# HJakeCunningham/ASVGP

Measured on AMD Instinct MI355X. Metric: Mpoints/s per ELBO+grad step, N=10M 1D Matern-3/2 M=2048, higher is better.
Workload: dtype f64

## Files before the change

### asvgp_amd/_lib.py

```python
import ctypes
import os

import torch

HERE = os.path.dirname(os.path.abspath(__file__))
LIB_PATH = os.path.join(HERE, "libasvgp_hip.so")

_c = ctypes
_P, _I, _L, _D, _Z = _c.c_void_p, _c.c_int, _c.c_int64, _c.c_double, _c.c_size_t

SIGNATURES = {
    "asvgp_version": (_I, []),
    "asvgp_last_error_string": (_c.c_char_p, []),
    "asvgp_status_name": (_c.c_char_p, [_I]),
    "asvgp_phi_workspace_bytes": (_Z, [_L, _I, _L]),
    "asvgp_create": (_I, [_c.POINTER(_P)]),
    "asvgp_destroy": (_I, [_P]),
    "asvgp_phi_accumulate_1d": (_I, [_P, _P, _P, _L, _L, _P, _L, _D, _I, _L, _P, _P, _Z, _P]),
    "asvgp_phi_weighted_workspace_bytes": (_Z, [_L, _I, _L]),
    "asvgp_phi_accumulate_1d_weighted": (_I, [_P, _P, _P, _P, _L, _L, _P, _L, _D, _I, _L, _P, _P, _P, _Z, _P]),
    "asvgp_set_weight_sums": (_I, [_P, _D, _D, _D]),
    "asvgp_phi_accumulate_kron2d_weighted": (_I, [_P, _P, _P, _L, _P, _L, _D, _L, _P, _L, _D, _L, _I, _P, _P, _P]),
    "asvgp_phi_accumulate_kron2d_sorted_weighted": (_I, [_P, _P, _P, _L, _P, _P, _L, _D, _L, _P, _L, _D, _L, _I, _P, _P, _P]),
    "asvgp_set_phi_algorithm": (_I, [_P, _I]),
    "asvgp_phi_last_algorithm": (_I, [_P]),
    "asvgp_set_phi_input_order": (_I, [_P, _I]),
    "asvgp_phi_last_input_order": (_I, [_P]),
    "asvgp_stream_probe": (_I, [_P, _P, _L, _P, _P]),
    "asvgp_debug_reload_env": (_I, []),
    "asvgp_set_deferred_forward_pass": (_I, [_P, _I]),
    "asvgp_prior_publish": (_I, [_P]),
    "asvgp_host_mantissa_bits": (_I, []),
    "asvgp_prior_interior_kuu_host": (_I, [_P, _I, _L, _I, _P, _P, _c.POINTER(_L), _c.POINTER(_L), _P]),
    "asvgp_result_mirror": (_I, [_P, _I, _c.POINTER(_P)]),
    "asvgp_result_mirror_read": (_I, [_P, _c.c_uint64, _P, _D]),
    "asvgp_elbo_grad_ahead_1d": (_I, [_P, _P, _P, _I, _L, _L, _I, _L, _P, _P, _P, _Z, _P]),
    "asvgp_elbo_publish_theta": (_I, [_P, _D, _D, _D]),
    "asvgp_elbo_grad_host_1d": (_I, [_P, _P, _P, _I, _D, _D, _D, _L, _L, _I, _L, _P, _P, _P, _Z, _P, _P, _D]),
    "asvgp_result_mirror_pending": (_c.c_uint64, [_P]),
    "asvgp_set_phi_workgroups": (_I, [_P, _I]),
    "asvgp_set_phi_deferred_reduce": (_I, [_P, _I]),
    "asvgp_phi_reduce_1d": (_I, [_P, _P]),
    "asvgp_phi_index_1d": (_I, [_P, _L, _P, _L, _D, _P, _P]),
    "asvgp_phi_evaluate_1d": (_I, [_P, _L, _P, _L, _D, _I, _I, _P, _P, _P]),
    "asvgp_matern_coeffs": (_I, [_I, _D, _D, _c.POINTER(_D), _c.POINTER(_D), _c.POINTER(_I)]),
    "asvgp_kuu_assemble": (_I, [_P, _I, _c.POINTER(_D), _c.POINTER(_D), _L, _I, _P, _P, _P]),
    "asvgp_cholesky_band": (_I, [_P, _P, _L, _I, _P, _P]),
    "asvgp_inverse_from_cholesky_band": (_I, [_P, _P, _L, _I, _P]),
    "asvgp_solve_triang_mat": (_I, [_P, _P, _P, _L, _I, _L, _I, _P]),
    "asvgp_product_band_band": (_I, [_P, _P, _P, _L, _I, _I, _I, _I, _I, _I, _P]),
    "asvgp_transpose_band": (_I, [_P, _P, _L, _I, _I, _P]),
    "asvgp_symmetrise_band": (_I, [_P, _P, _L, _I, _P]),
    "asvgp_unpack_banded_matrix_to_dense": (_I, [_P, _P, _L, _I, _I, _P]),
    "asvgp_pack_dense_matrix_to_banded": (_I, [_P, _P, _L, _I, _I, _P]),
    "asvgp_band_trace_sym": (_I, [_P, _P, _L, _I, _P, _P]),
    "asvgp_cholesky_band_vjp": (_I, [_P, _P, _P, _P, _L, _I, _P]),
    "asvgp_inverse_from_cholesky_band_vjp": (_I, [_P, _P, _P, _P, _P, _L, _I, _P]),
    "asvgp_band_outer_product": (_I, [_P, _P, _L, _L, _I, _D, _P, _P]),
    "asvgp_elbo_workspace_bytes": (_Z, [_L, _I, _L]),
    "asvgp_set_band_algorithm": (_I, [_P, _I]),
    "asvgp_prior_plan_1d": (_I, [_P, _P, _I, _L, _I, _c.POINTER(_I)]),
    "asvgp_prior_table_doubles": (_Z, [_P, _I, _L, _I]),
    "asvgp_prior_forward_host": (_I, [_P, _I, _L, _I, _P, _P, _P, _Z, _P]),
    "asvgp_set_prior_forward": (_I, [_P, _I]),
    "asvgp_prior_forward_device": (_I, [_P, _P, _P, _P, _Z, _P]),
    "asvgp_prior_forward_stamps": (_I, [_P, _P, _P, _P, _P]),
    "asvgp_prior_plan_image_host": (_I, [_P, _I, _L, _I, _P, _P, _P, _P]),
    "asvgp_elbo_grad_1d": (_I, [_P, _P, _P, _I, _D, _D, _D, _L, _L, _I, _L, _P, _P, _P, _Z, _P]),
    "asvgp_kuu_inverse_band_1d": (_I, [_P, _P, _I, _D, _D, _L, _I, _P, _P, _P, _P, _P, _P, _P, _Z, _P]),
    "asvgp_elbo_chain_sync": (_I, [_P, _I]),
    "asvgp_elbo_prior_chain_1d": (_I, [_P, _P, _I, _D, _D, _D, _L, _I, _L, _P, _P, _Z, _P]),
    "asvgp_elbo_data_chain_1d": (_I, [_P, _P, _P, _I, _D, _D, _D, _L, _L, _I, _L, _P, _P, _P, _Z, _P]),
    "asvgp_posterior_prepare_1d": (_I, [_P, _P, _P, _I, _D, _D, _D, _L, _I, _L, _P, _P, _P, _P, _Z, _P]),
    "asvgp_posterior_prepare_loo_1d": (_I, [_P, _P, _P, _I, _D, _D, _D, _L, _I, _L, _P, _P, _P, _P, _P, _Z, _P]),
    "asvgp_loo_workspace_bytes": (_Z, [_L, _I, _L]),
    "asvgp_loo_1d": (_I, [_P, _P, _P, _P, _L, _L, _P, _L, _D, _I, _L, _P, _P, _P, _D, _D, _P, _P, _P, _P, _P, _Z, _P]),
    "asvgp_predict_1d": (_I, [_P, _L, _P, _L, _D, _I, _L, _P, _P, _D, _L, _P, _P, _P]),
    "asvgp_predict_1d_h": (_I, [_P, _P, _L, _P, _L, _D, _I, _L, _P, _P, _D, _L, _P, _P, _P]),
    "asvgp_posterior_cov_workspace_bytes": (_Z, [_L, _I, _L]),
    "asvgp_posterior_cov_prepare_1d": (_I, [_P, _P, _P, _I, _D, _D, _D, _L, _I, _L, _P, _P, _P, _P, _P, _Z, _P]),
    "asvgp_predict_cov_1d": (_I, [_P, _P, _L, _P, _L, _P, _L, _D, _I, _L, _P, _I, _D, _D, _P, _L, _P]),
    "asvgp_predict_deriv_1d": (_I, [_P, _P, _L, _P, _L, _D, _I, _L, _P, _P, _I, _D, _D, _L, _P, _P, _P]),
    "asvgp_predict_cov_deriv_1d": (_I, [_P, _P, _L, _P, _L, _P, _L, _D, _I, _L, _P, _I, _D, _D, _I, _I, _P, _L, _P]),
    "asvgp_predict_grad_kron2d": (_I, [_P, _L, _P, _L, _D, _L, _P, _L, _D, _L, _I, _P, _P, _P, _P, _P, _L, _I, _L, _L, _L, _L,
                                       _I, _D, _D, _I, _D, _D, _P, _P, _P]),
    "asvgp_kron_dense_inverse": (_I, [_P, _P, _P, _L, _L, _I, _L, _L, _L, _L, _P, _P]),
    "asvgp_predict_cov_kron2d": (_I, [_P, _P, _L, _P, _L, _P, _L, _D, _L, _P, _L, _D, _L, _I, _P, _P, _P, _I, _D, _D, _I, _D, _D, _P, _L, _P]),
    "asvgp_predict_cov_additive": (_I, [_P, _P, _L, _P, _L, _I, _P, _c.POINTER(_L), _c.POINTER(_D), _c.POINTER(_L), _I,
                                         _c.POINTER(_I), _c.POINTER(_D), _c.POINTER(_D), _P, _P, _L, _P]),
    "asvgp_predict_components_additive": (_I, [_P, _P, _L, _I, _P, _c.POINTER(_L), _c.POINTER(_D), _c.POINTER(_L), _I, _c.POINTER(_I),
                                                _c.POINTER(_D), _c.POINTER(_D), _I, _P, _P, _P, _P, _P]),
    "asvgp_profile_enable": (_I, [_P, _I]),
    "asvgp_profile_read": (_I, [_P, _c.POINTER(_D), _c.POINTER(_L)]),
    "asvgp_kron_stats_doubles": (_Z, [_L, _L, _I]),
    "asvgp_phi_accumulate_kron2d": (_I, [_P, _P, _L, _P, _L, _D, _L, _P, _L, _D, _L, _I, _P, _P]),
    "asvgp_kron_evaluate_2d": (_I, [_P, _L, _P, _L, _D, _P, _L, _D, _L, _I, _P, _P, _P]),
    "asvgp_kron_assemble": (_I, [_P, _P, _P, _P, _P, _I, _L, _L, _D, _P, _P, _P]),
    "asvgp_blockband_cholesky": (_I, [_P, _L, _L, _P, _P, _P, _P]),
    "asvgp_blockband_backsolve": (_I, [_P, _L, _L, _P, _P]),
    "asvgp_predict_kron2d": (_I, [_P, _L, _P, _L, _D, _L, _P, _L, _D, _L, _I, _P, _P, _P, _P, _P, _P]),
    "asvgp_kron_cell_index": (_I, [_P, _L, _P, _L, _D, _P, _L, _D, _P, _P]),
    "asvgp_phi_accumulate_kron2d_sorted": (_I, [_P, _P, _L, _P, _P, _L, _D, _L, _P, _L, _D, _L, _I, _P, _P]),
    "asvgp_phi_accumulate_kron2d_sorted_f32": (_I, [_P, _P, _L, _P, _P, _L, _D, _L, _P, _L, _D, _L, _I, _P, _P]),
    "asvgp_blockband_to_blocks": (_I, [_P, _L, _L, _L, _P, _P, _P]),
    "asvgp_kron_grad_terms": (_I, [_P, _P, _L, _P, _P, _P, _P, _P, _P, _P, _P, _P, _P, _I, _L, _L, _P, _P]),
    "asvgp_predict_kron2d_var": (_I, [_P, _L, _P, _L, _D, _P, _L, _D, _L, _I, _P, _P, _L, _P, _P]),
    "asvgp_kron_assemble_twisted": (_I, [_P, _P, _P, _P, _P, _I, _L, _L, _D, _L, _L, _L, _L, _L, _P, _P, _P, _P]),
    "asvgp_kron_grad_terms_twisted": (_I, [_P, _P, _L, _L, _L, _L, _L, _P, _P, _P, _P, _P, _P, _P, _P, _P, _P, _I, _L, _L, _P, _P]),
    "asvgp_predict_kron2d_var_twisted": (_I, [_P, _L, _P, _L, _D, _P, _L, _D, _L, _L, _I, _P, _P, _L, _L, _L, _L, _L, _P, _P]),
    "asvgp_phi_cross_workspace_bytes": (_Z, [_L, _L]),
    "asvgp_phi_cross_2d": (_I, [_P, _P, _L, _P, _L, _D, _L, _P, _L, _D, _L, _I, _P, _P, _Z, _P]),
}


class AsvgpError(RuntimeError):
    pass


_lib = None


def get_lib():
    global _lib
    if _lib is not None:
        return _lib
    if not os.path.exists(LIB_PATH):
        raise AsvgpError("HIP extension %s is missing: run `python -m asvgp_amd.build` (hipcc, gfx950). "
                         "asvgp_amd has no CPU fallback." % LIB_PATH)
    lib = ctypes.CDLL(LIB_PATH)
    for name, (res, args) in SIGNATURES.items():
        fn = getattr(lib, name, None)
        if fn is None:
            raise AsvgpError("libasvgp_hip.so does not export %s" % name)
        fn.restype = res
        fn.argtypes = args
    _lib = lib
    return lib


def check(status, what=""):
    if status != 0:
        lib = get_lib()
        raise AsvgpError("%s failed: %s (%s)" % (what or "asvgp call", lib.asvgp_status_name(status).decode(),
                                                  lib.asvgp_last_error_string().decode()))


class Handle:
    _defaults = {"band": 0, "phi": 0, "prior_forward": 0, "phi_order": 0}
    _live = None

    def __init__(self):
        import weakref
        lib = get_lib()
        h = _P()
        check(lib.asvgp_create(ctypes.byref(h)), "asvgp_create")
        self.ptr = h
        self._lib = lib
        self.band_algorithm = 0
        if Handle._live is None:
            Handle._live = weakref.WeakSet()
        Handle._live.add(self)
        if Handle._defaults["band"]:
            self.set_band_algorithm(Handle._defaults["band"])
        if Handle._defaults["phi"]:
            self.set_phi_algorithm(Handle._defaults["phi"])
        if Handle._defaults["prior_forward"]:
            self.set_prior_forward(Handle._defaults["prior_forward"])
        if Handle._defaults["phi_order"]:
            self.set_phi_input_order(Handle._defaults["phi_order"])

    def set_prior_forward(self, mode):
        check(self._lib.asvgp_set_prior_forward(self.ptr, int(mode)), "set_prior_forward")

    def prior_forward_device(self, coef, dcoef, n_doubles):
        import numpy as np
        coef = np.ascontiguousarray(coef, dtype=np.float64)
        dcoef = np.ascontiguousarray(dcoef, dtype=np.float64)
        tab = np.zeros(int(n_doubles), dtype=np.float64)
        check(self._lib.asvgp_prior_forward_device(self.ptr, coef.ctypes.data, dcoef.ctypes.data, tab.ctypes.data, tab.size, stream_ptr()),
              "prior_forward_device")
        return tab

    def set_band_algorithm(self, algo):
        check(self._lib.asvgp_set_band_algorithm(self.ptr, int(algo)), "set_band_algorithm")
        self.band_algorithm = int(algo)

    def set_phi_algorithm(self, algo):
        check(self._lib.asvgp_set_phi_algorithm(self.ptr, int(algo)), "set_phi_algorithm")

    def set_weight_sums(self, n_pos, sum_w, sum_log_w):
        if n_pos is None:
            n_pos, sum_w, sum_log_w = -1.0, 0.0, 0.0
        check(self._lib.asvgp_set_weight_sums(self.ptr, float(n_pos), float(sum_w), float(sum_log_w)), "set_weight_sums")

    def phi_last_algorithm(self):
        return int(self._lib.asvgp_phi_last_algorithm(self.ptr))

    def set_phi_input_order(self, order):
        check(self._lib.asvgp_set_phi_input_order(self.ptr, int(order)), "set_phi_input_order")

    def phi_last_input_order(self):
        return int(self._lib.asvgp_phi_last_input_order(self.ptr))

    def result_mirror(self, enable=True):
        import numpy as np
        ptr = _P()
        check(self._lib.asvgp_result_mirror(self.ptr, int(bool(enable)), ctypes.byref(ptr)), "result_mirror")
        if not enable or not ptr.value:
            self._mirror = None
            return None
        self._mirror = np.ctypeslib.as_array(ctypes.cast(ptr, ctypes.POINTER(_D)), shape=(16,))
        return self._mirror

    def set_deferred_forward_pass(self, on):
        check(self._lib.asvgp_set_deferred_forward_pass(self.ptr, int(on)), "set_deferred_forward_pass")

    def publish_forward(self):
        self._lib.asvgp_prior_publish(self.ptr)

    def result_mirror_pending(self):
        return int(self._lib.asvgp_result_mirror_pending(self.ptr))

    def set_phi_workgroups(self, n):
        check(self._lib.asvgp_set_phi_workgroups(self.ptr, int(n)), "set_phi_workgroups")

    deferred = False

    def set_phi_deferred_reduce(self, on):
        check(self._lib.asvgp_set_phi_deferred_reduce(self.ptr, int(on)), "set_phi_deferred_reduce")
        self.deferred = bool(on)

    def chain_sync(self, on):
        check(self._lib.asvgp_elbo_chain_sync(self.ptr, int(on)), "elbo_chain_sync")

    def prior_plan(self, static_stack_host, n_terms, M, k):
        ok = _I(0)
        ptr = None if static_stack_host is None else static_stack_host.ctypes.data
        check(self._lib.asvgp_prior_plan_1d(self.ptr, ptr, int(n_terms), int(M), int(k), ctypes.byref(ok)), "prior_plan_1d")
        return bool(ok.value)

    def close(self):
        if getattr(self, "ptr", None) is not None and self.ptr:
            try:
                self._lib.asvgp_destroy(self.ptr)
            except Exception:
                pass
            self.ptr = None
            self._mirror = None

    def __del__(self):
        self.close()


def set_default_algorithms(band=None, phi=None, prior_forward=None, phi_order=None):
    if prior_forward is not None:
        Handle._defaults["prior_forward"] = int(prior_forward)
        for h in list(Handle._live or ()):
            h.set_prior_forward(prior_forward)
    if phi_order is not None:
        Handle._defaults["phi_order"] = int(phi_order)
        for h in list(Handle._live or ()):
            h.set_phi_input_order(phi_order)
    if band is not None:
        Handle._defaults["band"] = int(band)
    if phi is not None:
        Handle._defaults["phi"] = int(phi)
    for h in list(Handle._live or ()):
        if band is not None:
            h.set_band_algorithm(band)
        if phi is not None:
            h.set_phi_algorithm(phi)


_stream_override = None


def set_stream(stream=None):
    global _stream_override
    _stream_override = None if stream is None else ctypes.c_void_p(stream.cuda_stream)


def stream_ptr():
    if _stream_override is not None:
        return _stream_override
    return ctypes.c_void_p(torch.cuda.current_stream().cuda_stream)


def require_cuda(*tensors):
    for t in tensors:
        if not t.is_cuda:
            raise AsvgpError("asvgp_amd operates on ROCm device tensors only (got a %s tensor); there is no CPU path"
                             % t.device)


def f64c(t):
    if t.dtype != torch.float64:
        t = t.to(torch.float64)
    return t.contiguous()
```

### asvgp_amd/csrc/bcr_mfma.hpp

```cpp
#pragma once
#include "bcr.hpp"
#include "prior_plan.hpp"

namespace asvgp {

constexpr int BM_THREADS = 1024;
constexpr int BM_B = 4;
constexpr int BM_GAT = 0, BM_GBT = 16, BM_DINV = 32, BM_SD = 48, BM_CAT = 64, BM_CBT = 80, BM_W = 96, BM_DG = 100, BM_REC = 104;

__host__ __device__ inline size_t bcr_mfma_ws_doubles(long nb) { return (size_t)nb * BM_REC + 64; }
__host__ __device__ inline size_t bcr_mfma_lds_doubles(long nb) {
  return (size_t)((nb + 1) / 2 + 1) * 32 + (size_t)nb * 4 + 96 + (size_t)(BM_THREADS / 64) * 4 * 40 + (size_t)(nb / 8 + 2) * 52;
}

__device__ __forceinline__ double bm_mfma(double a, double b, double c) { return __builtin_amdgcn_mfma_f64_4x4x4f64(a, b, c, 0, 0, 0); }

__device__ __forceinline__ double bm_chol_linv(const double (&d)[10], int hi, int lo, double& dprod, int& badj) {
  double l00, i0, l10, l20, l30, l11, i1, l21, l31, l22, i2, l32, l33, i3;
  Num<double>::sqrt_inv(d[0], l00, i0);
  badj = !(d[0] > 0.0) ? 1 : 0;
  l10 = d[1] * i0; l20 = d[3] * i0; l30 = d[6] * i0;
  double s = fma(-l10, l10, d[2]);
  badj = (!(s > 0.0) && !badj) ? 2 : badj;
  Num<double>::sqrt_inv(s, l11, i1);
  l21 = fma(-l20, l10, d[4]) * i1;
  l31 = fma(-l30, l10, d[7]) * i1;
  s = fma(-l21, l21, fma(-l20, l20, d[5]));
  badj = (!(s > 0.0) && !badj) ? 3 : badj;
  Num<double>::sqrt_inv(s, l22, i2);
  l32 = fma(-l31, l21, fma(-l30, l20, d[8])) * i2;
  s = fma(-l32, l32, fma(-l31, l31, fma(-l30, l30, d[9])));
  badj = (!(s > 0.0) && !badj) ? 4 : badj;
  Num<double>::sqrt_inv(s, l33, i3);
  dprod = (l00 * l11) * (l22 * l33);
  const double z0 = (lo == 0) ? i0 : 0.0;
  const double z1 = fma(-l10, z0, (lo == 1) ? 1.0 : 0.0) * i1;
  const double z2 = fma(-l21, z1, fma(-l20, z0, (lo == 2) ? 1.0 : 0.0)) * i2;
  const double z3 = fma(-l32, z2, fma(-l31, z1, fma(-l30, z0, (lo == 3) ? 1.0 : 0.0))) * i3;
  return hi == 0 ? z0 : (hi == 1 ? z1 : (hi == 2 ? z2 : z3));
}

template <typename Src> __device__ __forceinline__ auto bm_src_load(const Src& A, int dd, long col, long M, int) -> decltype(A.load_dc(dd, col, M)) {
  return A.load_dc(dd, col, M);
}
template <typename Src> __device__ __forceinline__ double bm_src_load(const Src& A, int dd, long col, long M, long) {
  return A.load((long)dd * M + col, true);
}
struct BmLog {
  double m; int e;
  __device__ __forceinline__ void mul(double p) {
    m *= p;
    const int hi = __double2hiint(m);
    e += ((hi >> 20) & 0x7ff) - 1023;
    m = __hiloint2double((hi & 0x800fffff) | 0x3ff00000, __double2loint(m));
  }
};

__device__ __forceinline__ unsigned long long bm_wave_xor(unsigned long long x) {
#pragma unroll
  for (int off = 32; off > 0; off >>= 1) x ^= (unsigned long long)__shfl_xor((long long)x, off, 64);
  return x;
}
__device__ __forceinline__ void bm_msg_send(double* box, int n, double v, unsigned long long tag, int lane) {
  unsigned long long* b = reinterpret_cast<unsigned long long*>(box);
  const unsigned long long w = lane < n ? (unsigned long long)__double_as_longlong(v) : 0ull;
  const unsigned long long x = bm_wave_xor(w) ^ tag;
  if (lane < n) __hip_atomic_store(b + lane, w, __ATOMIC_RELAXED, __HIP_MEMORY_SCOPE_AGENT);
  if (lane == n) __hip_atomic_store(b + n, x, __ATOMIC_RELAXED, __HIP_MEMORY_SCOPE_AGENT);
}
__device__ __forceinline__ bool bm_msg_recv(const double* box, int n, double& v, unsigned long long tag, int lane, long spin_limit) {
  const unsigned long long* b = reinterpret_cast<const unsigned long long*>(box);
  for (long spins = 0; spins <= spin_limit; ++spins) {
    const unsigned long long w = lane <= n ? __hip_atomic_load(b + lane, __ATOMIC_RELAXED, __HIP_MEMORY_SCOPE_AGENT) : 0ull;
    const unsigned long long x = bm_wave_xor(lane < n ? w : 0ull) ^ tag;
    const unsigned long long chk = (unsigned long long)__shfl((long long)w, n, 64);
    if (x == chk) { v = __longlong_as_double((long long)w); return true; }
    __builtin_amdgcn_s_sleep(1);
  }
  return false;
}

struct BmSplit {
  int half = -1;
  double* xchg = nullptr;
  long spin_limit = 0;
  int* gave_up = nullptr;
  unsigned long long tag = 0;
};
constexpr int BM_XCHG = 96;

template <typename Src>
__device__ __attribute__((always_inline)) void bcr_mfma_solve(Src A, const double* rhs, int M, double* ws, double* lds, double* Sband, double* x,
                                                              double* logdet, int* info, int rhs_stride = 1, double* stamps = nullptr,
                                                              BmSplit sp = BmSplit{}) {
  constexpr int B = BM_B;
  const int tid = threadIdx.x;
  const int lane = tid & 63, wv = __builtin_amdgcn_readfirstlane(tid >> 6);
  const int r = lane >> 4, q = (lane >> 2) & 3, c = lane & 3;
  const int e = r * 4 + c, et = c * 4 + r;
  const int hi = r > c ? r : c, lo = r > c ? c : r;
  const int nb = (M + B - 1) / B;
  const int nslot = (nb + 1) / 2;
  double* Dl = lds;
  double* El = lds + (size_t)(nslot + 1) * 16;
  double* xs = El + (size_t)(nslot + 1) * 16;
  double* red = xs + (size_t)nb * B;
  double* slab = red + 96 + (size_t)(wv * 4 + q) * 40;
  double* Fl = red + 96 + (size_t)(BM_THREADS / 64) * 4 * 40;
  double* Sl = lds;
  int levels = 0;
  while ((1 << levels) < nb) ++levels;
  const bool split = sp.half >= 0;
  const int top = levels - 1, ht = 1 << (top > 0 ? top : 0);
  double s_other = 0.0;
  int bad_other = 0x7fffffff;
  auto level_share = [&](int l, int ne, int& m0, int& ne_h) {
    m0 = 0; ne_h = ne;
    if (!split) return;
    if (l < top) {
      const int mL = ht >> (l + 1);
      if (sp.half == 0) ne_h = ne < mL ? ne : mL;
      else { m0 = mL; ne_h = ne > mL ? ne - mL : 0; }
    } else {
      ne_h = sp.half == 0 ? ne : 0;
    }
  };
  int bad = 0;
  BmLog ld{1.0, 0};
  unsigned long long t_prev = stamps ? __builtin_amdgcn_s_memtime() : 0ull;
  int nst = 0;
  auto stamp = [&]() {
    if (stamps && tid == 0) { const unsigned long long t = __builtin_amdgcn_s_memtime(); stamps[nst++] = (double)(t - t_prev); t_prev = t; }
  };
  auto rec = [&](int node) -> double* { return ws + (size_t)node * BM_REC; };
  auto bandD = [&](int n, int rr, int cc) -> double {
    const int col = n * B + cc, row = n * B + rr;
    const bool pad = row >= M;
    const double v = bm_src_load(A, rr - cc, pad ? 0 : col, (long)M, 0);
    return pad ? ((rr == cc) ? 1.0 : 0.0) : v;
  };
  auto bandE = [&](int n, int rr, int cc) -> double {
    if (rr > cc) return 0.0;
    const int col = n * B + cc, row = (n + 1) * B + rr;
    const bool pad = row >= M;
    const double v = bm_src_load(A, B + rr - cc, pad ? 0 : col, (long)M, 0);
    return pad ? 0.0 : v;
  };
  if ((nb & 1) && tid < 16 && !(split && sp.half == 0)) {
    const int rr = tid >> 2, cc = tid & 3;
    Dl[(size_t)((nb - 1) >> 1) * 16 + tid] = bandD(nb - 1, rr > cc ? rr : cc, rr > cc ? cc : rr);
  }
  if (split && sp.half == 0 && tid < 16) Dl[(size_t)(ht >> 1) * 16 + tid] = 0.0;
  for (int row = tid; row < nb * B; row += BM_THREADS) {
    const bool sep_left = split && sp.half == 0 && row >= ht * B && row < (ht + 1) * B;
    xs[row] = (row < M && !sep_left) ? rhs[(long)row * rhs_stride] : 0.0;
  }
  __syncthreads();
  stamp();

  constexpr int RMAXR = 4;
  for (int l = 0; l < levels; ++l) {
    const int h = 1 << l;
    const int ne = (nb > h) ? (nb - h + 2 * h - 1) / (2 * h) : 0;
    int m0, ne_h;
    level_share(l, ne, m0, ne_h);
    if (split && l == top) {
      if (sp.half == 1) {
        if (wv == 0) {
          const double v = lane < 16 ? Dl[(size_t)(ht >> 1) * 16 + lane] : (lane < 20 ? xs[ht * B + lane - 16] : 0.0);
          bm_msg_send(sp.xchg, 20, v, sp.tag | 1ull, lane);
        }
        const double mine = (r == 0 && c == 0) ? (log(ld.m) + (double)ld.e * 0.6931471805599453094) : 0.0;
        const double tot = wave_sum_dpp(mine);
        int bm = bad ? bad : 0x7fffffff;
#pragma unroll
        for (int off = 32; off > 0; off >>= 1) { const int o = __shfl_xor(bm, off, 64); bm = o < bm ? o : bm; }
        int* sbad = reinterpret_cast<int*>(red + 32);
        if (lane == 0) { red[wv] = tot; sbad[wv] = bm; }
        __syncthreads();
        if (wv == 0) {
          double sv = 0.0;
          int bmin = 0x7fffffff;
          for (int w2 = 0; w2 < BM_THREADS / 64; ++w2) { sv += red[w2]; bmin = sbad[w2] < bmin ? sbad[w2] : bmin; }
          bm_msg_send(sp.xchg + 24, 2, lane == 0 ? sv : (double)bmin, sp.tag | 2ull, lane);
        }
      } else {
        if (wv == 0) {
          double v = 0.0;
          if (!bm_msg_recv(sp.xchg, 20, v, sp.tag | 1ull, lane, sp.spin_limit)) { if (lane == 0) *sp.gave_up = 1; }
          else {
            if (lane < 16) Dl[(size_t)(ht >> 1) * 16 + lane] += v;
            else if (lane < 20) xs[ht * B + lane - 16] += v;
          }
        }
        __syncthreads();
        if (*sp.gave_up) return;
      }
      stamp();
    }
    double updb[RMAXR], ybu[RMAXR];
    int qv = q, ev = e;
    asm volatile("" : "+v"(qv), "+v"(ev));
    double sl[2][3];
    auto slab_loads = [&](int rd0) __attribute__((always_inline)) {
#pragma unroll
      for (int u = 0; u < 2; ++u) {
#pragma unroll
        for (int t3 = 0; t3 < 3; ++t3) {
          sl[u][t3] = 0.0;
          int m = (rd0 + u) * 64 + wv * 4 + qv;
          m = m0 + (m < ne_h ? m : ne_h - 1);
          const int kk = ev + 16 * t3, dd = kk >> 3, col = m * 2 * B + (kk & 7);
          const bool in = kk < 40 && col + dd < M;
          const double v = bm_src_load(A, in ? dd : 0, in ? col : 0, (long)M, 0);
          sl[u][t3] = in ? v : ((dd == 0) ? 1.0 : 0.0);
        }
      }
    };
#pragma unroll
    for (int rd = 0; rd < RMAXR; ++rd) {
      __builtin_amdgcn_sched_barrier(0);
      if (l == 0 && (rd & 1) == 0) slab_loads(rd);
      updb[rd] = 0.0; ybu[rd] = 0.0;
      if (rd * 64 + wv * 4 >= ne_h) continue;
      const int ml = rd * 64 + wv * 4 + q;
      const bool act = ml < ne_h;
      const int i = h + (m0 + (act ? ml : ne_h - 1)) * 2 * h, a = i - h, b = i + h;
      const bool hasb = b < nb;
      const int bsafe = hasb ? b : a;
      double d[10];
      double ea, eb, da;
      if (l == 0) {
#pragma unroll
        for (int t3 = 0; t3 < 3; ++t3) if (e + 16 * t3 < 40) slab[e + 16 * t3] = sl[rd & 1][t3];
        int kk = 0;
#pragma unroll
        for (int rr = 0; rr < 4; ++rr)
#pragma unroll
          for (int cc = 0; cc <= rr; ++cc) d[kk++] = slab[(rr - cc) * 8 + 4 + cc];
        ea = slab[(4 + lo - hi) * 8 + hi];
        ea = (r <= c) ? ea : 0.0;
        eb = slab[(4 + lo - hi) * 8 + 4 + hi];
        eb = (hasb && c <= r) ? eb : 0.0;
        da = slab[(hi - lo) * 8 + lo];
      } else {
        const double* Di = Dl + (size_t)(i >> 1) * 16;
        int kk = 0;
#pragma unroll
        for (int rr = 0; rr < 4; ++rr)
#pragma unroll
          for (int cc = 0; cc <= rr; ++cc) d[kk++] = Di[rr * 4 + cc];
        ea = El[(size_t)(a >> 1) * 16 + e];
        eb = El[(size_t)(i >> 1) * 16 + et];
        eb = hasb ? eb : 0.0;
        da = Dl[(size_t)(a >> 1) * 16 + e];
      }
      double yv = xs[i * B + r], ya = xs[a * B + r];
      yv = (c == 0) ? yv : 0.0;
      ya = (c == 0) ? ya : 0.0;
      (void)bsafe;
      double dprod;
      int badj;
      const double t = bm_chol_linv(d, hi, lo, dprod, badj);
      if (act && badj && !bad) bad = i * B + badj;
      const double linv = (r >= c) ? t : 0.0;
      const double linvT = (c >= r) ? t : 0.0;
      if (act) ld.mul(dprod);
      const double ua = bm_mfma(linvT, ea, 0.0);
      const double ub = bm_mfma(linvT, eb, 0.0);
      const double zz = bm_mfma(linvT, yv, 0.0);
      const double nua = -ua, nub = -ub;
      const double da_new = bm_mfma(nua, ua, da);
      const double e_new = bm_mfma(nub, ua, 0.0);
      const double ya_new = bm_mfma(nua, zz, ya);
      updb[rd] = bm_mfma(ub, ub, 0.0);
      ybu[rd] = bm_mfma(ub, zz, 0.0);
      updb[rd] = act ? updb[rd] : 0.0;
      ybu[rd] = act ? ybu[rd] : 0.0;
      const double gat = bm_mfma(ua, linv, 0.0);
      const double gbt = bm_mfma(ub, linv, 0.0);
      const double dinv = bm_mfma(linv, linv, 0.0);
      const double w = bm_mfma(linv, zz, 0.0);
      if (act) {
        if (l >= 3) {
          double* R = Fl + (size_t)(i >> 3) * 52;
          R[e] = gat; R[16 + e] = gbt; R[32 + e] = dinv;
          if (c == 0) R[48 + r] = w;
        } else {
          double* R = rec(i);
          R[BM_GAT + e] = gat; R[BM_GBT + e] = gbt; R[BM_DINV + e] = dinv;
          if (c == 0) R[BM_W + r] = w;
        }
        Dl[(size_t)(a >> 1) * 16 + e] = da_new;
        El[(size_t)(a >> 1) * 16 + e] = e_new;
        if (c == 0) xs[a * B + r] = ya_new;
      }
    }
    bcr_lds_barrier();
#pragma unroll
    for (int rd = 0; rd < RMAXR; ++rd) {
      if (rd * 64 + wv * 4 >= ne_h) continue;
      const int ml = rd * 64 + wv * 4 + q;
      const int i = h + (m0 + ml) * 2 * h, b = i + h;
      if (ml < ne_h && b < nb) {
        Dl[(size_t)(b >> 1) * 16 + e] -= updb[rd];
        if (c == 0) xs[b * B + r] -= ybu[rd];
      }
    }
    bcr_lds_barrier();
    stamp();
  }
  if (wv == 0 && !(split && sp.half == 1)) {
    const bool act = q == 0;
    double d[10];
    int kk = 0;
#pragma unroll
    for (int rr = 0; rr < 4; ++rr)
#pragma unroll
      for (int cc = 0; cc <= rr; ++cc) { const double v = Dl[rr * 4 + cc]; d[kk++] = act ? v : ((rr == cc) ? 1.0 : 0.0); }
    const double yv = (act && c == 0) ? xs[r] : 0.0;
    double dprod;
    int badj;
    const double t = bm_chol_linv(d, hi, lo, dprod, badj);
    if (act && badj && !bad) bad = badj;
    const double linv = (r >= c) ? t : 0.0, linvT = (c >= r) ? t : 0.0;
    if (act) ld.mul(dprod);
    const double s00 = bm_mfma(linv, linv, 0.0);
    const double zz = bm_mfma(linvT, yv, 0.0);
    const double x0 = bm_mfma(linv, zz, 0.0);
    if (act) {
      rec(0)[BM_SD + e] = s00;
      Sl[e] = s00;
      if (r >= c && r < M) Sband[(long)(r - c) * M + c] = s00;
      if (c == 0) xs[r] = x0;
    }
  }
  __syncthreads();
  stamp();
  unsigned long long lw = 0ull;
  for (int l = levels - 1; l >= 0; --l) {
    const int h = 1 << l;
    const int ne = (nb > h) ? (nb - h + 2 * h - 1) / (2 * h) : 0;
    int m0, ne_h;
    level_share(l, ne, m0, ne_h);
    if (split && sp.half == 0 && wv == BM_THREADS / 64 - 1) {
      if (l == top - 1 && lane <= 2)
        lw = __hip_atomic_load(reinterpret_cast<const unsigned long long*>(sp.xchg + 24) + lane, __ATOMIC_RELAXED, __HIP_MEMORY_SCOPE_AGENT);
      if (l == 2) {
        const unsigned long long x = bm_wave_xor(lane < 2 ? lw : 0ull) ^ (sp.tag | 2ull);
        const unsigned long long chk = (unsigned long long)__shfl((long long)lw, 2, 64);
        double v = __longlong_as_double((long long)lw);
        bool ok = x == chk;
        if (!ok) ok = bm_msg_recv(sp.xchg + 24, 2, v, sp.tag | 2ull, lane, sp.spin_limit);
        if (!ok) { if (lane == 0) *sp.gave_up = 1; }
        else if (lane < 2) red[48 + lane] = v;
      }
    }
#pragma unroll
    for (int rd = 0; rd < RMAXR; ++rd) {
      __builtin_amdgcn_sched_barrier(0);
      if (rd * 64 + wv * 4 >= ne_h) continue;
      const int ml = rd * 64 + wv * 4 + q;
      const bool act = ml < ne_h;
      const int i = h + (m0 + (act ? ml : ne_h - 1)) * 2 * h, a = i - h, b = i + h;
      const bool hasb = b < nb;
      const int bs = hasb ? b : a;
      const bool e_is_a = ((a / (2 * h)) & 1) != 0;
      double gat, gbt, dinv, w, saa, sbb, sba, sab;
      if (l >= 3) {
        const double* R = Fl + (size_t)(i >> 3) * 52;
        gat = R[e]; gbt = R[16 + e]; dinv = R[32 + e]; w = R[48 + r];
      } else {
        const double* R = rec(i);
        gat = R[BM_GAT + e]; gbt = R[BM_GBT + e]; dinv = R[BM_DINV + e]; w = R[BM_W + r];
      }
      if (l >= 1) {
        const double* Ra = Sl + (size_t)(a >> 2) * 48;
        const double* Rb = Sl + (size_t)(bs >> 2) * 48;
        saa = Ra[e];
        sbb = Rb[e];
        sba = e_is_a ? Ra[32 + e] : Rb[16 + et];
        sab = e_is_a ? Ra[32 + et] : Rb[16 + e];
      } else {
        const double* Ra = rec(a);
        const double* Rb = rec(bs);
        saa = Ra[BM_SD + e];
        sbb = Rb[BM_SD + e];
        sba = e_is_a ? Ra[BM_CBT + e] : Rb[BM_CAT + et];
        sab = e_is_a ? Ra[BM_CBT + et] : Rb[BM_CAT + e];
      }
      sbb = hasb ? sbb : 0.0; sba = hasb ? sba : 0.0; sab = hasb ? sab : 0.0;
      double xa = xs[a * B + r], xb = xs[bs * B + r];
      xa = (c == 0) ? xa : 0.0;
      xb = (hasb && c == 0) ? xb : 0.0;
      w = (c == 0) ? w : 0.0;
      double ncat = bm_mfma(saa, gat, 0.0);
      ncat = bm_mfma(sba, gbt, ncat);
      double ncbt = bm_mfma(sab, gat, 0.0);
      ncbt = bm_mfma(sbb, gbt, ncbt);
      double sii = bm_mfma(ncat, gat, dinv);
      sii = bm_mfma(ncbt, gbt, sii);
      double gx = bm_mfma(gat, xa, 0.0);
      gx = bm_mfma(gbt, xb, gx);
      if (act) {
        if (c == 0) xs[i * B + r] = w - gx;
        if (l >= 2) {
          double* Rw = Sl + (size_t)(i >> 2) * 48;
          Rw[e] = sii; Rw[16 + e] = -ncat; Rw[32 + e] = -ncbt;
        }
        if (l > 0) {
          double* Rw = rec(i);
          Rw[BM_SD + e] = sii; Rw[BM_CAT + e] = -ncat; Rw[BM_CBT + e] = -ncbt;
        }
        if (r >= c && i * B + r < M) Sband[(long)(r - c) * M + i * B + c] = sii;
        if (l == 0) {
          if (c <= r && i * B + c < M) Sband[(long)(B + c - r) * M + a * B + r] = -ncat;
          if (hasb && r <= c && b * B + r < M) Sband[(long)(B + r - c) * M + i * B + c] = -ncbt;
        }
      }
    }
    if (l == 1) __syncthreads(); else bcr_lds_barrier();
    if (split && l == top) {
      double* Rs = Sl + (size_t)(ht >> 2) * 48;
      if (sp.half == 0) {
        if (wv == 0) bm_msg_send(sp.xchg + 32, 52, lane < 48 ? Rs[lane < 48 ? lane : 0] : (lane < 52 ? xs[ht * B + lane - 48] : 0.0), sp.tag | 3ull, lane);
      } else {
        if (wv == 0) {
          double v = 0.0;
          if (!bm_msg_recv(sp.xchg + 32, 52, v, sp.tag | 3ull, lane, sp.spin_limit)) { if (lane == 0) *sp.gave_up = 1; }
          else if (lane < 48) {
            Rs[lane] = v;
            rec(ht)[BM_SD + lane] = v;
            if (lane < 16) {
              const int rr = lane >> 2, cc = lane & 3;
              if (rr >= cc && ht * B + rr < M) Sband[(long)(rr - cc) * M + ht * B + cc] = v;
            }
          } else if (lane < 52) {
            xs[ht * B + lane - 48] = v;
          }
        }
        __syncthreads();
        if (*sp.gave_up) return;
      }
    }
    stamp();
  }
  if (!(split && sp.half == 0))
    for (int col = M - B + tid; col < M; col += BM_THREADS)
      if (col >= 0)
#pragma unroll
        for (int dd = 1; dd <= B; ++dd)
          if (col + dd >= M) Sband[(long)dd * M + col] = 0.0;
  {
    const int row0 = (split && sp.half == 1) ? (ht + 1) * B : 0, row1 = (split && sp.half == 0) ? (ht + 1) * B : M;
    for (int row = row0 + tid; row < row1 && row < M; row += BM_THREADS) x[(long)row * rhs_stride] = xs[row];
  }
  if (!(split && sp.half == 1)) {
    const double mine = (r == 0 && c == 0) ? (log(ld.m) + (double)ld.e * 0.6931471805599453094) : 0.0;
    const double tot = wave_sum_dpp(mine);
    int bm = bad ? bad : 0x7fffffff;
#pragma unroll
    for (int off = 32; off > 0; off >>= 1) { const int o = __shfl_xor(bm, off, 64); bm = o < bm ? o : bm; }
    int* sbad = reinterpret_cast<int*>(red + 32);
    if (lane == 0) { red[wv] = tot; sbad[wv] = bm; }
    __syncthreads();
    if (split && tid == 0) { s_other = red[48]; bad_other = (int)red[49]; }
    if (tid == 0) {
      double s = 0.0;
      int bmin = 0x7fffffff;
      for (int w2 = 0; w2 < BM_THREADS / 64; ++w2) { s += red[w2]; bmin = sbad[w2] < bmin ? sbad[w2] : bmin; }
      s += s_other;
      bmin = bad_other < bmin ? bad_other : bmin;
      __hip_atomic_store(logdet + 0, 2.0 * s, __ATOMIC_RELAXED, __HIP_MEMORY_SCOPE_AGENT);
      __hip_atomic_store(logdet + 1, 0.0, __ATOMIC_RELAXED, __HIP_MEMORY_SCOPE_AGENT);
      __hip_atomic_store(info, (bmin == 0x7fffffff) ? 0 : bmin, __ATOMIC_RELAXED, __HIP_MEMORY_SCOPE_AGENT);
    }
  }
  stamp();
}


__host__ __device__ inline size_t bcr_mfma_pre_ws_doubles(long nb) { return (size_t)nb * 96 + 64; }
__host__ __device__ inline size_t bcr_mfma_pre_lds_doubles(long nb, int n_rec) {
  return PRIOR_TAB_HEADER + (size_t)2 * n_rec * prior_rec_fields(BM_B) + (size_t)(nb / 4 + 2) * 96 + (size_t)(nb + 1) / 2 + 64;
}

struct BmDual { double v, d; };
__device__ __forceinline__ BmDual bm_dmfma(BmDual x, BmDual y, BmDual c) {
  BmDual r;
  r.v = bm_mfma(x.v, y.v, c.v);
  r.d = bm_mfma(x.d, y.v, c.d);
  r.d = bm_mfma(x.v, y.d, r.d);
  return r;
}

__device__ __attribute__((always_inline)) void bcr_mfma_backward_pre(const double* __restrict__ tab, int n_rec, const int* __restrict__ node_rec, int M,
                                                                      double* ws, double* lds, double* Sv, double* Sd, double* logdet, int* info,
                                                                      unsigned long long* done_flag, unsigned long long seq,
                                                                      const unsigned long long* ready_flag = nullptr, long spin_limit = 0, int* gave_up = nullptr) {
  constexpr int B = BM_B, W = prior_rec_fields(B);
  const int tid = threadIdx.x;
  if (ready_flag) {
    if (tid == 0) {
      long spins = 0;
      while (__hip_atomic_load(ready_flag, __ATOMIC_RELAXED, __HIP_MEMORY_SCOPE_SYSTEM) < seq) {
        __builtin_amdgcn_s_sleep(8);
        if (++spins > spin_limit) { *gave_up = 1; break; }
      }
    }
    __syncthreads();
    if (*gave_up) return;
    __builtin_amdgcn_fence(__ATOMIC_ACQUIRE, "");
  }
  const int lane = tid & 63, wv = __builtin_amdgcn_readfirstlane(tid >> 6);
  const int r = lane >> 4, q = (lane >> 2) & 3, c = lane & 3;
  const int e = r * 4 + c, et = c * 4 + r;
  const int nb = (M + B - 1) / B;
  const int n_tab = PRIOR_TAB_HEADER + 2 * n_rec * W;
  double* tl = lds;
  double* Sl = lds + n_tab;
  int* nrl = reinterpret_cast<int*>(Sl + (size_t)(nb / 4 + 2) * 96);
  {
    const double2* src = reinterpret_cast<const double2*>(tab);
    double2* dst = reinterpret_cast<double2*>(tl);
// ... 96 lines not shown
```

### asvgp_amd/csrc/elbo.hip

```cpp
#include <stdlib.h>
#include <time.h>
#include <string.h>

#include "bcr_pre.hpp"
#include "bcr_mfma.hpp"
#include "handle.hpp"

namespace asvgp {


struct Ws {
  double *Kuu, *dK, *P, *LK, *dLK, *LP, *SK, *dSK, *SP, *c, *alpha, *logdets, *fin, *bcrK, *bcrP;
};
static size_t bcr_ws_chain(int planes, int k, bool big) {
  long ns = 1024;
  while ((long)planes * 2 * k * k * ns * 8 + 2 * ns * k * 8 + 1024 > 150 * 1024) ns >>= 1;
  if (big) ns *= 2;
  return (size_t)planes * (7 * k * k + k) * 2 * ns + (big ? (size_t)planes * k * k * ns : 0);
}
static size_t bcr_ws_K(int k, long M) {
  size_t a = bcr_ws_chain(2, k, false), b = bcr_ws_chain(2, k, true), c = bcr_pre_ws_doubles(k, (M + k - 1) / k);
  a = a > b ? a : b;
  return (a > c ? a : c) + 64;
}
// ... 157 lines not shown
template <int K, bool BIG>
__global__ __launch_bounds__(BCR_THREADS) void elbo_bcr_data_kernel(const double* Kuu, const double* A, const double* b, int M,
                                                                    double* wsP, double* SP, double* x, double* logdets,
                                                                    int* info, int do_stamps, double s, int D, int lds_doubles) {
  extern __shared__ double lds[];
  double* st = do_stamps ? logdets + 8 : nullptr;
  bcr_solve<double, K, 1, BandSumP, BIG>(BandSumP{A, Kuu, 1.0 / s}, b, M, wsP, lds, BandOut<double>{SP, nullptr}, x, logdets + 2, info + 1,
                                         st ? st + 24 : nullptr, D);
  more_columns<K, BIG>(b, x, D, M, wsP, lds, lds_doubles);
}

template <int KT>
__device__ __forceinline__ double quad_col(const double* S, long M, long j, const double* x, long D, long d) {
  double xj = x[j * D + d];
  double a = S[j] * xj * xj;
#pragma unroll
  for (int r = 1; r <= KT; ++r) {
    long jr = (j + r < M) ? j + r : M - 1;
    double sv = (j + r < M) ? S[(long)r * M + j] : 0.0;
    a = fma(2.0 * sv * xj, x[jr * D + d], a);
  }
  return a;
}

struct ElboScalars { double v, l, s, N, Nw, cw; };

template <int KT>
__device__ __forceinline__ void elbo_finalize_body(
    int bid, int nblk, double* part_lds, const double* __restrict__ stats, const double* __restrict__ Kuu, const double* __restrict__ dK,
    const double* __restrict__ LK, const double* __restrict__ LP, const double* __restrict__ SK,
    const double* __restrict__ dSK, const double* __restrict__ SP, const double* __restrict__ c,
    const double* __restrict__ alpha, const double* __restrict__ logdets, long M, long D, ElboScalars th,
    double alpha_scale, double* __restrict__ gacc, unsigned* __restrict__ ticket, unsigned* __restrict__ rearm, double* __restrict__ out) {
  constexpr int k = KT;
  const double* A = stats;
  const double* b = stats + (long)(k + 1) * M;
  const double yy = stats[(long)(k + 1) * M + M * D];
  enum { LOGK, LOGP, TRKA, DTRKA, SKDK, SPDK, SKK, SPK, SPA, CC, AKA, ADKA, AAA, BA, NACC };
  double acc[NACC];
#pragma unroll
  for (int i = 0; i < NACC; ++i) acc[i] = 0.0;
  const long chunk = (M + nblk - 1) / nblk;
  const long j_end = ((long)(bid + 1) * chunk < M) ? (long)(bid + 1) * chunk : M;
  for (long j = (long)bid * chunk + threadIdx.x; j < j_end; j += blockDim.x) {
    if (!logdets) {
      double lk = LK[j], lp = LP[j];
      acc[LOGK] += log(lk * lk);
      acc[LOGP] += log(lp * lp);
    }
#pragma unroll
    for (int r = 0; r <= k; ++r) {
      long o = (long)r * M + j;
      double w = (r == 0) ? 1.0 : 2.0;
      double sk = SK[o], sp = SP[o], a = A[o], kk = Kuu[o], dk = dK[o];
      acc[TRKA] = fma(w * sk, a, acc[TRKA]);
      acc[DTRKA] = fma(w * dSK[o], a, acc[DTRKA]);
      acc[SKDK] = fma(w * sk, dk, acc[SKDK]);
      acc[SPDK] = fma(w * sp, dk, acc[SPDK]);
      acc[SKK] = fma(w * sk, kk, acc[SKK]);
      acc[SPK] = fma(w * sp, kk, acc[SPK]);
      acc[SPA] = fma(w * sp, a, acc[SPA]);
    }
    for (long d = 0; d < D; ++d) {
      if (!logdets) {
        double cv = c[j * D + d];
        acc[CC] = fma(cv, cv, acc[CC]);
      }
      acc[AKA] += quad_col<KT>(Kuu, M, j, alpha, D, d);
      acc[ADKA] += quad_col<KT>(dK, M, j, alpha, D, d);
      acc[AAA] += quad_col<KT>(A, M, j, alpha, D, d);
      acc[BA] = fma(b[j * D + d], alpha[j * D + d], acc[BA]);
    }
  }
  double (*part)[NACC] = reinterpret_cast<double (*)[NACC]>(part_lds);
  const int lane = threadIdx.x & 63, wv = threadIdx.x >> 6, nw = blockDim.x >> 6;
#pragma unroll
  for (int i = 0; i < NACC; ++i) {
    double v = wave_sum_dpp(acc[i]);
    if (lane == 0) part[wv][i] = v;
  }
  __syncthreads();
  double tot[NACC];
  if (threadIdx.x < 64) {
#pragma unroll
    for (int i = 0; i < NACC; ++i) tot[i] = wave_sum_dpp(lane < nw ? part[lane][i] : 0.0);
  }
  int* is_last_p = reinterpret_cast<int*>(part_lds + 16 * NACC);
#define is_last (*is_last_p)
  if (threadIdx.x == 0) {
#pragma unroll
    for (int i = 0; i < NACC; ++i)
      if (tot[i] != 0.0) __hip_atomic_fetch_add(gacc + i, tot[i], __ATOMIC_RELAXED, __HIP_MEMORY_SCOPE_AGENT);
    asm volatile("s_waitcnt vmcnt(0)" ::: "memory");
    unsigned t = __hip_atomic_fetch_add(ticket, 1u, __ATOMIC_RELAXED, __HIP_MEMORY_SCOPE_AGENT);
    is_last = (t == (unsigned)nblk - 1);
  }
  __syncthreads();
  if (!is_last) return;
  if (threadIdx.x == 0) {
#pragma unroll
    for (int i = 0; i < NACC; ++i) tot[i] = __hip_atomic_load(gacc + i, __ATOMIC_RELAXED, __HIP_MEMORY_SCOPE_AGENT);
#pragma unroll
    for (int i = 0; i < NACC; ++i) __hip_atomic_store(gacc + i, 0.0, __ATOMIC_RELAXED, __HIP_MEMORY_SCOPE_AGENT);
    __hip_atomic_store(ticket, 0u, __ATOMIC_RELAXED, __HIP_MEMORY_SCOPE_AGENT);
    if (rearm) __hip_atomic_store(rearm, 0u, __ATOMIC_RELAXED, __HIP_MEMORY_SCOPE_AGENT);
    const double v = th.v, s = th.s, N = th.N, Nw = th.Nw, Dd = (double)D;
    tot[AKA] *= alpha_scale * alpha_scale; tot[ADKA] *= alpha_scale * alpha_scale; tot[AAA] *= alpha_scale * alpha_scale;
    tot[BA] *= alpha_scale;
    if (logdets) {
      tot[LOGK] = logdets[0];
      tot[LOGP] = logdets[2];
      tot[CC] = tot[BA] / s;
    }
    const double two_pi = 6.283185307179586476925286766559;
    double elbo = -0.5 * N * Dd * log(two_pi * s);
    elbo -= 0.5 * Dd * tot[LOGP];
    elbo += 0.5 * Dd * tot[LOGK];
    elbo -= 0.5 * yy / s;
    elbo += 0.5 * tot[CC];
    elbo -= 0.5 * Nw * v / s;
    elbo += 0.5 * tot[TRKA] / s;
    if (th.cw != 0.0) elbo += th.cw;
    double d_l = 0.5 * (Dd * tot[SKDK] - Dd * tot[SPDK] - tot[ADKA] + tot[DTRKA] / s);
    double d_v = 0.5 * (-Dd * tot[SKK] / v + Dd * tot[SPK] / v + tot[AKA] / v + tot[TRKA] / (v * s)) - 0.5 * Nw / s;
    double s2 = s * s;
    double d_s = -0.5 * N * Dd / s + 0.5 * Dd * tot[SPA] / s2 + 0.5 * yy / s2 + 0.5 * tot[AAA] / s2 - tot[BA] / s2 +
                 0.5 * Nw * v / s2 - 0.5 * tot[TRKA] / s2;
    out[0] = elbo; out[1] = d_v; out[2] = d_l; out[3] = d_s;
    out[4] = tot[LOGK]; out[5] = tot[LOGP]; out[6] = tot[TRKA]; out[7] = tot[CC];
  }
#undef is_last
}

constexpr int FIN_LDS_DOUBLES = 16 * 14 + 2;

template <int KT>
__global__ __launch_bounds__(256) void elbo_finalize_kernel(
    const double* __restrict__ stats, const double* __restrict__ Kuu, const double* __restrict__ dK,
    const double* __restrict__ LK, const double* __restrict__ LP, const double* __restrict__ SK,
    const double* __restrict__ dSK, const double* __restrict__ SP, const double* __restrict__ c,
    const double* __restrict__ alpha, const double* __restrict__ logdets, long M, int k_rt, long D, ElboScalars th,
    double alpha_scale, double* __restrict__ gacc, unsigned* __restrict__ ticket, double* __restrict__ out) {
  __shared__ double part[FIN_LDS_DOUBLES];
  (void)k_rt;
  elbo_finalize_body<KT>((int)blockIdx.x, (int)gridDim.x, part, stats, Kuu, dK, LK, LP, SK, dSK, SP, c, alpha, logdets, M, D, th, alpha_scale,
                         gacc, ticket, nullptr, out);
}

struct FusedFin {
  const double* stats; ElboScalars th; double alpha_scale; double* gacc; unsigned* ticket; unsigned* arrived; unsigned* assembled; double* out;
  long D; int n_helpers; int finalize; int debug_no_assembly; int debug_stamps;
  double* mirror; unsigned long long mirror_seq;
  int split; double* xchg;
};
constexpr int FIN_GACC_PR = 21;
__device__ __forceinline__ void assemble_band_slice(const double* __restrict__ S, const double* __restrict__ coef, const double* __restrict__ dcoef, int n_terms,
                                                    long E, long e, double* __restrict__ Kuu, double* __restrict__ dK) {
#pragma clang fp contract(off)
  double sv[ASVGP_MAX_KUU_TERMS];
#pragma unroll
  for (int t = 0; t < ASVGP_MAX_KUU_TERMS; ++t) sv[t] = (t < n_terms) ? S[(long)t * E + e] : 0.0;
  double acc = coef[0] * sv[0], dacc = dcoef[0] * sv[0];
#pragma unroll
  for (int t = 1; t < ASVGP_MAX_KUU_TERMS; ++t)
    if (t < n_terms) { acc = acc + coef[t] * sv[t]; dacc = dacc + dcoef[t] * sv[t]; }
  Kuu[e] = acc;
  if (dK) dK[e] = dacc;
}
template <int K, bool BIG>
__global__ __launch_bounds__(BCR_THREADS) void elbo_chains_kernel(const double* S_static, KuuCoefs2 cf, double* Kuu, double* dK, const double* A, const double* b, int M,
                                                                  double* wsP, double* SP, double* x, double* logdets, int* info,
                                                                  double s, const double* tab, int n_rec, const int* node_rec,
                                                                  double* wsK, double* SK, double* dSK,
                                                                  unsigned long long* done_flag, unsigned long long seq, int D, int lds_doubles, FusedFin fin) {
  extern __shared__ double lds[];
  const long E = (long)(K + 1) * M;
  __shared__ int gave_up;
  if (threadIdx.x == 0) gave_up = 0;
  __syncthreads();
  if (blockIdx.x == 0) {
    if (threadIdx.x == 0) {
      long spins = 0;
      while (__hip_atomic_load(fin.assembled, __ATOMIC_RELAXED, __HIP_MEMORY_SCOPE_AGENT) < (unsigned)fin.n_helpers) {
        __builtin_amdgcn_s_sleep(2);
        if (++spins > (1L << 25)) { gave_up = 1; break; }
      }
      if (!gave_up) __hip_atomic_store(fin.assembled, 0u, __ATOMIC_RELAXED, __HIP_MEMORY_SCOPE_AGENT);
    }
    __syncthreads();
    if (gave_up) { if (threadIdx.x == 0) atomicExch(info + 1, -1); return; }
    __builtin_amdgcn_fence(__ATOMIC_ACQUIRE, "agent");
    bcr_solve<double, K, 1, BandSumP, BIG>(BandSumP{A, Kuu, 1.0 / s}, b, M, wsP, lds, BandOut<double>{SP, nullptr}, x, logdets + 2, info + 1, nullptr, D);
    more_columns<K, BIG>(b, x, D, M, wsP, lds, lds_doubles);
  } else if (blockIdx.x == 1) {
    bcr_backward_pre<K>(tab, n_rec, node_rec, M, wsK, lds, BandOut<Dual>{SK, dSK}, logdets, info, done_flag, seq);
  } else {
    for (long e = (long)(blockIdx.x - 2) * blockDim.x + threadIdx.x; e < E; e += (long)fin.n_helpers * blockDim.x)
      assemble_band_slice(S_static, cf.c, cf.dc, cf.n, E, e, Kuu, dK);
    __syncthreads();
    if (threadIdx.x == 0) {
      __threadfence();
      __hip_atomic_fetch_add(fin.assembled, 1u, __ATOMIC_RELEASE, __HIP_MEMORY_SCOPE_AGENT);
    }
  }
  if (!fin.finalize) return;
  if (blockIdx.x < 2) {
    __syncthreads();
    if (threadIdx.x == 0) {
      __threadfence();
      __hip_atomic_fetch_add(fin.arrived, 1u, __ATOMIC_RELEASE, __HIP_MEMORY_SCOPE_AGENT);
    }
    return;
  }
  if (threadIdx.x == 0) {
    long spins = 0;
    while (__hip_atomic_load(fin.arrived, __ATOMIC_RELAXED, __HIP_MEMORY_SCOPE_AGENT) < 2u) {
      __builtin_amdgcn_s_sleep(8);
      if (++spins > (1L << 25)) { gave_up = 1; break; }
    }
  }
  __syncthreads();
  if (gave_up) { if (threadIdx.x == 0) atomicExch(info + 1, -1); return; }
  __builtin_amdgcn_fence(__ATOMIC_ACQUIRE, "agent");
  elbo_finalize_body<K>((int)blockIdx.x - 2, fin.n_helpers, lds, fin.stats, Kuu, dK, nullptr, nullptr, SK, dSK, SP, nullptr, x, logdets, (long)M, fin.D,
                        fin.th, fin.alpha_scale, fin.gacc, fin.ticket, fin.arrived, fin.out);
}

template <int K>
__global__ __launch_bounds__(BM_THREADS) void elbo_chains_mfma_kernel(KuuInterior ki, const double* S_static, KuuCoefs2 cf, double* Kuu, double* dK, const double* A, const double* b, int M,
                                                                      double* wsP, double* SP, double* x, double* logdets, int* info,
                                                                      double s, const double* tab, int n_rec, const int* node_rec,
                                                                      double* wsK, double* SK, double* dSK,
                                                                      unsigned long long* done_flag, unsigned long long seq,
                                                                      const unsigned long long* ready_flag, long spin_limit, FusedFin fin, const ThetaBox* box) {
  extern __shared__ double lds[];
  static_assert(K == BM_B, "matrix-core chains: bandwidth 4");
  const long E = (long)(K + 1) * M;
  const unsigned long long t_start = fin.debug_stamps ? __builtin_amdgcn_s_memrealtime() : 0ull;
  auto rstamp = [&](int slot) {
    if (fin.debug_stamps && threadIdx.x == 0 && blockIdx.x <= 2)
      logdets[(slot < 4 ? 8 + 4 * (int)blockIdx.x : 24) + slot] = (slot == 0) ? (double)(t_start & 0xffffffffull) : (double)((__builtin_amdgcn_s_memrealtime() - t_start) & 0xffffffffull);
  };
  rstamp(0);
  __shared__ int gave_up, kuu_ok;
  __shared__ double kuu_pref[4];
  if (threadIdx.x == 0) { gave_up = 0; kuu_ok = 0; }
  __syncthreads();
  double s_v = s, asc_v = fin.alpha_scale;
  ElboScalars th_v = fin.th;
  if (box) {
    if (threadIdx.x == 0) {
      long spins = 0;
      for (;;) {
        const unsigned long long got = __hip_atomic_load(&box->seq, __ATOMIC_RELAXED, __HIP_MEMORY_SCOPE_SYSTEM);
        if (got == seq) break;
        if (got == ~0ull || ++spins > spin_limit) { gave_up = 1; break; }
        __builtin_amdgcn_s_sleep(2);
      }
    }
    __syncthreads();
    if (gave_up) { if (threadIdx.x == 0) atomicExch(info + 1, -1); return; }
    s_v = box->s; asc_v = box->alpha_scale;
    th_v.v = box->v; th_v.l = box->l; th_v.s = box->s; th_v.N = box->N; th_v.Nw = box->Nw; th_v.cw = box->cw;
  }
  const double* stats = fin.stats;
  enum { LOGK, LOGP, TRKA, DTRKA, SKDK, SPDK, SKK, SPK, SPA, CC, AKA, ADKA, AAA, BA, NACC };
  double acc[NACC];
#pragma unroll
  for (int i = 0; i < NACC; ++i) acc[i] = 0.0;
  const bool isP = blockIdx.x == 0 || (fin.split && blockIdx.x == 2);
  const bool isPR = fin.split && blockIdx.x == 2;
  __shared__ double kdl[16];
  __shared__ double bnd[2 * PRIOR_BND_DIAGS * PRIOR_BND], dkb[2 * 5 * KI_DKB];
  {
    if (isP) rstamp(1);
    if (threadIdx.x == 0) {
      if (box) {
#pragma unroll
        for (int i = 0; i < 5; ++i) { kdl[i] = box->k[i]; kdl[8 + i] = box->dk[i]; }
      } else {
        kdl[0] = ki.k[0]; kdl[1] = ki.k[1]; kdl[2] = ki.k[2]; kdl[3] = ki.k[3]; kdl[4] = ki.k[4];
        kdl[8] = ki.dk[0]; kdl[9] = ki.dk[1]; kdl[10] = ki.dk[2]; kdl[11] = ki.dk[3]; kdl[12] = ki.dk[4];
      }
    }
    {
      const double* bnd_g = box ? box->bnd : reinterpret_cast<const double*>((const char*)__builtin_amdgcn_kernarg_segment_ptr() + offsetof(KuuInterior, bnd));
      const double* dkb_g = box ? box->dkb : reinterpret_cast<const double*>((const char*)__builtin_amdgcn_kernarg_segment_ptr() + offsetof(KuuInterior, dkb));
      if (threadIdx.x < 2 * PRIOR_BND_DIAGS * PRIOR_BND) bnd[threadIdx.x] = bnd_g[threadIdx.x];
      else if (threadIdx.x < 2 * PRIOR_BND_DIAGS * PRIOR_BND + 2 * 5 * KI_DKB) dkb[threadIdx.x - 2 * PRIOR_BND_DIAGS * PRIOR_BND] = dkb_g[threadIdx.x - 2 * PRIOR_BND_DIAGS * PRIOR_BND];
    }
    __syncthreads();
  }
  if (isP) {
    BmSplit bsp;
    if (fin.split) { bsp.half = isPR ? 1 : 0; bsp.xchg = fin.xchg; bsp.spin_limit = spin_limit; bsp.gave_up = &gave_up; bsp.tag = seq << 8; }
    bcr_mfma_solve<BandSumToep>(BandSumToep{A, 1.0 / s_v, (lds_cdouble_ptr)kdl, (lds_cdouble_ptr)bnd, ki.lo, ki.hi}, b, M, wsP, lds, SP, x, logdets + 2, info + 1, 1,
                                fin.debug_stamps ? (isPR ? fin.xchg + 128 : logdets + 32) : (double*)nullptr, bsp);
    rstamp(3);
    __syncthreads();
    if (gave_up) { if (threadIdx.x == 0) atomicExch(info + 1, -1); return; }
    rstamp(4);
    if (fin.finalize) {
      const double* xs_l = lds + (size_t)2 * ((((M + K - 1) / K) + 1) / 2 + 1) * 16;
      static_assert(BM_THREADS == 1024, "two columns per thread");
      int nbl = (M + K - 1) / K, lv = 0;
      while ((1 << lv) < nbl) ++lv;
      const long jsep = (long)(1 << (lv > 0 ? lv - 1 : 0)) * K;
      const long j0 = isPR ? jsep : 0, j1 = (fin.split && !isPR) ? jsep : (long)M;
      unsigned long long kw = 0ull;
      const bool kuu_reader = !isPR && (threadIdx.x >> 6) == 1;
      if (kuu_reader && (threadIdx.x & 63) <= 4)
        kw = __hip_atomic_load(reinterpret_cast<const unsigned long long*>(fin.gacc + 8) + (threadIdx.x & 63), __ATOMIC_RELAXED, __HIP_MEMORY_SCOPE_AGENT);
      double sp[2][K + 1], av[2][K + 1], bj[2];
#pragma unroll
      for (int cI = 0; cI < 2; ++cI) {
        const long j = j0 + threadIdx.x + cI * BM_THREADS, jc = j < j1 ? j : j1 - 1;
#pragma unroll
        for (int r = 0; r <= K; ++r) { sp[cI][r] = SP[(long)r * M + jc]; av[cI][r] = stats[(long)r * M + jc]; }
        bj[cI] = stats[(long)(K + 1) * M + jc];
      }
#pragma unroll
      for (int cI = 0; cI < 2; ++cI) {
        const long j = j0 + threadIdx.x + cI * BM_THREADS;
        if (j >= j1) continue;
        const bool left = j < ki.lo, right = j >= ki.hi;
        const double xj = xs_l[j];
#pragma unroll
        for (int r = 0; r <= K; ++r) {
          const long o = (long)r * M + j;
          const double w2 = (r == 0) ? 1.0 : 2.0;
          double kv = kdl[r], dkv = kdl[8 + r];
          if (left || right) {
            kv = bnd[left ? (long)r * PRIOR_BND + j : (long)(PRIOR_BND_DIAGS + r) * PRIOR_BND + (j - ki.hi)];
            if (ki.dk_tab) {
              dkv = dkb[left ? (long)r * KI_DKB + j : (long)(5 + r) * KI_DKB + (j - ki.hi)];
            } else {
              dkv = 0.0;
              for (int t = 0; t < cf.n; ++t) dkv = fma(box ? box->dc[t] : cf.dc[t], S_static[(long)t * E + o], dkv);
            }
          }
          const double xx = (j + r < M) ? w2 * xj * xs_l[j + r] : 0.0;
          acc[SPDK] = fma(w2 * sp[cI][r], dkv, acc[SPDK]);
          acc[SPK] = fma(w2 * sp[cI][r], kv, acc[SPK]);
          acc[SPA] = fma(w2 * sp[cI][r], av[cI][r], acc[SPA]);
          acc[AKA] = fma(kv, xx, acc[AKA]);
          acc[ADKA] = fma(dkv, xx, acc[ADKA]);
          acc[AAA] = fma(av[cI][r], xx, acc[AAA]);
        }
        acc[BA] = fma(bj[cI], xj, acc[BA]);
      }
      if (kuu_reader) {
        const int ln = threadIdx.x & 63;
        const unsigned long long x = bm_wave_xor(ln < 4 ? kw : 0ull) ^ ((seq << 8) | 4ull);
        const unsigned long long chk = (unsigned long long)__shfl((long long)kw, 4, 64);
        if (x == chk) { if (ln < 4) kuu_pref[ln] = __longlong_as_double((long long)kw); if (ln == 0) kuu_ok = 1; }
      }
    }
  } else {
    if (fin.debug_no_assembly) {
      if (threadIdx.x == 0) { for (long sp_ = 0; sp_ < spin_limit; ++sp_) __builtin_amdgcn_s_sleep(8); atomicExch(info + 1, -1); }
      return;
    }
    bcr_mfma_backward_pre(tab, n_rec, node_rec, M, wsK, lds, SK, dSK, logdets, info, done_flag, seq, ready_flag,
                          spin_limit < (1L << 20) ? spin_limit : (1L << 20), &gave_up);
    if (gave_up) { if (threadIdx.x == 0) atomicExch(info + 1, -1); return; }
    rstamp(1);
    if (fin.finalize) {
      __syncthreads();
      double sk[2][K + 1], dsk[2][K + 1], av[2][K + 1];
#pragma unroll
      for (int cI = 0; cI < 2; ++cI) {
        const long j = (long)threadIdx.x + cI * BM_THREADS, jc = j < M ? j : M - 1;
#pragma unroll
        for (int r = 0; r <= K; ++r) { sk[cI][r] = SK[(long)r * M + jc]; dsk[cI][r] = dSK[(long)r * M + jc]; av[cI][r] = stats[(long)r * M + jc]; }
      }
#pragma unroll
      for (int cI = 0; cI < 2; ++cI) {
        const long j = (long)threadIdx.x + cI * BM_THREADS;
        if (j >= M) continue;
        const bool left = j < ki.lo, right = j >= ki.hi;
#pragma unroll
        for (int r = 0; r <= K; ++r) {
          const long o = (long)r * M + j;
          const double w2 = (r == 0) ? 1.0 : 2.0;
          double kv = kdl[r], dkv = kdl[8 + r];
          if (left || right) {
            kv = bnd[left ? (long)r * PRIOR_BND + j : (long)(PRIOR_BND_DIAGS + r) * PRIOR_BND + (j - ki.hi)];
            if (ki.dk_tab) {
              dkv = dkb[left ? (long)r * KI_DKB + j : (long)(5 + r) * KI_DKB + (j - ki.hi)];
            } else {
              dkv = 0.0;
              for (int t = 0; t < cf.n; ++t) dkv = fma(box ? box->dc[t] : cf.dc[t], S_static[(long)t * E + o], dkv);
            }
          }
          acc[TRKA] = fma(w2 * sk[cI][r], av[cI][r], acc[TRKA]);
          acc[DTRKA] = fma(w2 * dsk[cI][r], av[cI][r], acc[DTRKA]);
          acc[SKDK] = fma(w2 * sk[cI][r], dkv, acc[SKDK]);
          acc[SKK] = fma(w2 * sk[cI][r], kv, acc[SKK]);
        }
      }
    }
  }
  if (!fin.finalize) { rstamp(2); return; }
  if (isP) rstamp(5);
  double* part0 = lds;
  const int lane = threadIdx.x & 63;
  double mine[8];
  mine[0] = isP ? acc[SPDK] : acc[TRKA];
  mine[1] = isP ? acc[SPK] : acc[DTRKA];
  mine[2] = isP ? acc[SPA] : acc[SKDK];
  mine[3] = isP ? acc[AKA] : acc[SKK];
  mine[4] = acc[ADKA]; mine[5] = acc[AAA]; mine[6] = acc[BA]; mine[7] = 0.0;
  const int nmine = isP ? 7 : 4;
  __syncthreads();
  const bool b0 = (lane & 1) != 0, b1 = (lane & 2) != 0, b2 = (lane & 4) != 0;
  double s4[4], s2[2];
#pragma unroll
  for (int i = 0; i < 4; ++i) { const double keep = b0 ? mine[4 + i] : mine[i], send = b0 ? mine[i] : mine[4 + i]; s4[i] = keep + dpp_move_f64<0xB1>(send); }
#pragma unroll
  for (int i = 0; i < 2; ++i) { const double keep = b1 ? s4[2 + i] : s4[i], send = b1 ? s4[i] : s4[2 + i]; s2[i] = keep + dpp_move_f64<0x4E>(send); }
  double s1 = (b2 ? s2[1] : s2[0]) + dpp_xor4_f64(b2 ? s2[0] : s2[1], b2);
  s1 += dpp_move_f64<0x128>(s1); s1 += __shfl_xor(s1, 16, 64); s1 += __shfl_xor(s1, 32, 64);
  const int wv = threadIdx.x >> 6;
  if (lane < 8) part0[wv * 8 + lane] = s1;
  __syncthreads();
  if (threadIdx.x >= 64) return;
  double t2 = part0[(2 * (lane >> 3)) * 8 + (lane & 7)] + part0[(2 * (lane >> 3) + 1) * 8 + (lane & 7)];
  t2 += __shfl_xor(t2, 8, 64); t2 += __shfl_xor(t2, 16, 64); t2 += __shfl_xor(t2, 32, 64);
  double red[7];
  red[0] = __shfl(t2, 0, 64); red[1] = __shfl(t2, 4, 64); red[2] = __shfl(t2, 2, 64); red[3] = __shfl(t2, 6, 64);
  red[4] = __shfl(t2, 1, 64); red[5] = __shfl(t2, 5, 64); red[6] = __shfl(t2, 3, 64);
  (void)nmine;
  double tot[NACC];
#pragma unroll
  for (int i = 0; i < NACC; ++i) tot[i] = 0.0;
  if (isP && threadIdx.x == 0) rstamp(6);
  const unsigned long long mtag = seq << 8;
  double* box_kuu = fin.gacc + 8;
  double* box_pr = fin.gacc + FIN_GACC_PR;
  if (!isP || isPR) {
    double v = red[0];
#pragma unroll
    for (int i = 1; i < 7; ++i) v = (lane == i) ? red[i] : v;
    bm_msg_send(isPR ? box_pr : box_kuu, nmine, v, mtag | (isPR ? 5ull : 4ull), lane);
    if (threadIdx.x == 0) rstamp(2);
    return;
  }
  double kuu_v = 0.0, pr_v = 0.0;
// ... 5 lines not shown
    if (!ok) { if (lane == 0) atomicExch(info + 1, -1); return; }
  }
  {
    const int pidx[7] = {SPDK, SPK, SPA, AKA, ADKA, AAA, BA};
#pragma unroll
    for (int i = 0; i < 7; ++i) tot[pidx[i]] = red[i] + (fin.split ? __shfl(pr_v, i, 64) : 0.0);
  }
  tot[TRKA] = __shfl(kuu_v, 0, 64); tot[DTRKA] = __shfl(kuu_v, 1, 64); tot[SKDK] = __shfl(kuu_v, 2, 64); tot[SKK] = __shfl(kuu_v, 3, 64);
  if (threadIdx.x != 0) return;
#pragma unroll
  for (int i = 0; i < 14; ++i) __hip_atomic_store(fin.gacc + i, 0.0, __ATOMIC_RELAXED, __HIP_MEMORY_SCOPE_AGENT);
  {
    const double v = th_v.v, sn = th_v.s, N = th_v.N, Nw = th_v.Nw;
    const double yy = stats[(long)(K + 1) * M + M];
    const double asc = asc_v;
    tot[AKA] *= asc * asc; tot[ADKA] *= asc * asc; tot[AAA] *= asc * asc; tot[BA] *= asc;
    tot[LOGK] = __hip_atomic_load(logdets + 0, __ATOMIC_RELAXED, __HIP_MEMORY_SCOPE_AGENT);
    tot[LOGP] = __hip_atomic_load(logdets + 2, __ATOMIC_RELAXED, __HIP_MEMORY_SCOPE_AGENT);
    tot[CC] = tot[BA] / sn;
    const double two_pi = 6.283185307179586476925286766559;
    double elbo = -0.5 * N * log(two_pi * sn);
    elbo -= 0.5 * tot[LOGP];
    elbo += 0.5 * tot[LOGK];
    elbo -= 0.5 * yy / sn;
    elbo += 0.5 * tot[CC];
    elbo -= 0.5 * Nw * v / sn;
    elbo += 0.5 * tot[TRKA] / sn;
    if (th_v.cw != 0.0) elbo += th_v.cw;
    const double d_l = 0.5 * (tot[SKDK] - tot[SPDK] - tot[ADKA] + tot[DTRKA] / sn);
    const double d_v = 0.5 * (-tot[SKK] / v + tot[SPK] / v + tot[AKA] / v + tot[TRKA] / (v * sn)) - 0.5 * Nw / sn;
    const double s2 = sn * sn;
    const double d_s = -0.5 * N / sn + 0.5 * tot[SPA] / s2 + 0.5 * yy / s2 + 0.5 * tot[AAA] / s2 - tot[BA] / s2 + 0.5 * Nw * v / s2 - 0.5 * tot[TRKA] / s2;
    double* out = fin.out;
    out[0] = elbo; out[1] = d_v; out[2] = d_l; out[3] = d_s;
    out[4] = tot[LOGK]; out[5] = tot[LOGP]; out[6] = tot[TRKA]; out[7] = tot[CC];
    if (fin.mirror) {
      double* m = fin.mirror;
      const double mv[10] = {elbo, d_v, d_l, d_s, tot[LOGK], tot[LOGP], tot[TRKA], tot[CC],
                             (double)__hip_atomic_load(info, __ATOMIC_RELAXED, __HIP_MEMORY_SCOPE_AGENT),
                             (double)__hip_atomic_load(info + 1, __ATOMIC_RELAXED, __HIP_MEMORY_SCOPE_AGENT)};
      double sum = (double)fin.mirror_seq;
#pragma unroll
      for (int i = 0; i < 10; ++i) { __hip_atomic_store(m + i, mv[i], __ATOMIC_RELAXED, __HIP_MEMORY_SCOPE_SYSTEM); sum += mv[i]; }
      __hip_atomic_store(m + 11, sum, __ATOMIC_RELAXED, __HIP_MEMORY_SCOPE_SYSTEM);
      __hip_atomic_store(m + 10, (double)fin.mirror_seq, __ATOMIC_RELAXED, __HIP_MEMORY_SCOPE_SYSTEM);
    }
  }
  rstamp(2);
}

static __global__ void scale_sub_kernel(const double* __restrict__ a, const double* __restrict__ b, double* __restrict__ o,
                                 long n) {
  long i = (long)blockIdx.x * blockDim.x + threadIdx.x;
  if (i < n) o[i] = a[i] - b[i];
}
static __global__ void scale_kernel(double* __restrict__ x, double f, long n) {
  long i = (long)blockIdx.x * blockDim.x + threadIdx.x;
  if (i < n) x[i] = x[i] * f;
}

template <int K, bool TANGENT>
static int run_chains(Handle* h, const double* stats, const double* S, int kind, double v, double l, double s, long M, long D,
                      Ws w, int* info, hipStream_t st, bool& use_bcr, int part = 0, bool scale_alpha = true, FusedFin* fin = nullptr) {
  double t_enter = 0.0;
  if (debug_env().host_times) { timespec ts; clock_gettime(CLOCK_MONOTONIC, &ts); t_enter = ts.tv_sec * 1e6 + ts.tv_nsec * 1e-3; }
  KuuCoefs2 cf;
  for (int t = 0; t < ASVGP_MAX_KUU_TERMS; ++t) cf.c[t] = cf.dc[t] = 0.0;
  int rc = asvgp_matern_coeffs(kind, v, l, cf.c, cf.dc, &cf.n);
  if (rc) return rc;
  const long E = (long)(K + 1) * M;
  const double* A = stats;
  const double* b = stats ? stats + E : nullptr;
  const long nb = (M + K - 1) / K;
  const int algo = h->band_algo;
  const bool have_plan = h->plan && prior_plan_M(h->plan) == M && prior_plan_k(h->plan) == K && prior_plan_terms(h->plan) == cf.n;
  if ((algo == 3 || algo == 4) && !have_plan) { set_error("band algorithms 3 and 4 need asvgp_prior_plan_1d for this (M, k, kernel)"); return ASVGP_ERR_BAD_ARG; }
  size_t ldsK = sizeof(double) * (TANGENT ? bcr_lds_doubles<Dual, K, 0>(nb) : bcr_lds_doubles<double, K, 0>(nb));
  size_t ldsP = sizeof(double) * bcr_lds_doubles<double, K, 1>(nb);
  bool planned = have_plan && (algo == 0 || algo == 3 || algo == 4);
  size_t lds_bytes = planned ? ldsP : (ldsK > ldsP ? ldsK : ldsP);
  bool fits = lds_bytes <= 160 * 1024 - 256;
  bool big = false;
  constexpr bool HAS_BIG = (K <= 5);
  if (HAS_BIG && !fits) {
    size_t bK = sizeof(double) * (TANGENT ? bcr_lds_doubles<Dual, K, 0, true>(nb) : bcr_lds_doubles<double, K, 0, true>(nb));
    size_t bP = sizeof(double) * bcr_lds_doubles<double, K, 1, true>(nb);
    size_t bb = planned ? bP : (bK > bP ? bK : bP);
    if (bb <= 160 * 1024 - 256) { big = true; fits = true; lds_bytes = bb; }
  }
  use_bcr = (algo == 2 || algo == 3 || algo == 4 || (algo == 0 && fits));
  planned = planned && use_bcr;
  if (part != 0 && (!use_bcr || planned)) {
    if (part == 1) return ASVGP_OK;
    part = 0;
  }
  if (planned) {
    const int n_rec = prior_plan_nrec(h->plan);
    bool use_mfma = false;
    KuuInterior ki;
    if constexpr (K == BM_B) {
      use_mfma = (algo == 0 || algo == 4) && D == 1 && nb <= 512 && TANGENT && fin != nullptr &&
                 sizeof(double) * bcr_mfma_lds_doubles(nb) <= 160 * 1024 && sizeof(double) * bcr_mfma_pre_lds_doubles(nb, n_rec) <= 160 * 1024;
      if (use_mfma) {
        prior_plan_interior_kuu(h->plan, cf.c, ki.k, &ki.lo, &ki.hi, ki.bnd);
        use_mfma = ki.hi > ki.lo;
        if (use_mfma) {
          double bnd2[2 * PRIOR_BND_DIAGS * PRIOR_BND];
          long lo2 = 0, hi2 = 0;
          prior_plan_interior_kuu(h->plan, cf.dc, ki.dk, &lo2, &hi2, bnd2);
          ki.dk_tab = (ki.lo <= KI_DKB && M - ki.hi <= KI_DKB) ? 1 : 0;
          for (int sd = 0; sd < 2; ++sd)
            for (int d = 0; d <= K; ++d)
              for (int cI = 0; cI < KI_DKB; ++cI)
                ki.dkb[(sd * 5 + d) * KI_DKB + cI] = bnd2[(size_t)(sd * PRIOR_BND_DIAGS + d) * PRIOR_BND + cI];
        }
      }
    }
    if (algo == 4 && !use_mfma) {
      set_error("band algorithm 4 (matrix-core chains) needs k = 4, D = 1, M <= 2048, Toeplitz static bands and the ELBO + gradient entry point");
      return ASVGP_ERR_UNSUPPORTED;
    }
    if (h->ahead_req && !use_mfma) { set_error("launch-ahead exists for the matrix-core launch only (k = 4, D = 1, M <= 2048, planned prior chain)"); return ASVGP_ERR_UNSUPPORTED; }
    if (!use_mfma && !fits) { set_error("BCR needs %zu B of LDS", lds_bytes); return ASVGP_ERR_LDS_CAPACITY; }
    unsigned long long seq = 0;
    int slot = 0;
    double t_acq0 = 0.0, t_acq1 = 0.0;
    if (debug_env().host_times) { timespec ts; clock_gettime(CLOCK_MONOTONIC, &ts); t_acq0 = ts.tv_sec * 1e6 + ts.tv_nsec * 1e-3; }
    double* tab = handle_table_acquire(h, &seq, &slot);
    if (debug_env().host_times) { timespec ts; clock_gettime(CLOCK_MONOTONIC, &ts); t_acq1 = ts.tv_sec * 1e6 + ts.tv_nsec * 1e-3; }
    const bool gpu_fwd = h->prior_forward_gpu;
    const double* tab_k = h->tab_dev + (size_t)slot * h->slot_doubles;
    const unsigned long long* dd_ready = nullptr;
    if (gpu_fwd) {
      double* t = nullptr;
      rc = handle_prior_dd_forward(h, cf.c, cf.dc, slot, st, &t, nullptr, use_mfma ? seq : 0ull, use_mfma ? &dd_ready : nullptr);
      if (rc) return rc;
      tab_k = t;
    }
    size_t lds_pre = sizeof(double) * bcr_pre_lds_doubles(K, n_rec);
    if (lds_pre > lds_bytes) lds_bytes = lds_pre;
    FusedFin ff{};
    if (fin) { ff = *fin; ff.finalize = 1; fin->finalize = -1; }
    ff.n_helpers = (int)((M + 255) / 256 < 6 ? (M + 255) / 256 : 6);
    ff.split = 0; ff.xchg = nullptr;
    ff.assembled = reinterpret_cast<unsigned*>(w.fin + 20);
    ff.debug_no_assembly = debug_env().no_assembly;
    ff.debug_stamps = debug_env().chain_stamps;
    const long spin_limit = debug_env().spin_limit;
    if constexpr (K == BM_B) {
      if (use_mfma) {
        size_t lb = sizeof(double) * bcr_mfma_lds_doubles(nb), lk = sizeof(double) * bcr_mfma_pre_lds_doubles(nb, n_rec);
        if (lk > lb) lb = lk;
        if (sizeof(double) * FIN_LDS_DOUBLES > lb) lb = sizeof(double) * FIN_LDS_DOUBLES;
        auto kern = elbo_chains_mfma_kernel<K>;
        static size_t lds_granted[16] = {0};
        size_t& granted = lds_granted[h->device & 15];
        if (lb > granted) {
          hipError_t e = hipFuncSetAttribute(reinterpret_cast<const void*>(kern), hipFuncAttributeMaxDynamicSharedMemorySize, (int)lb);
          if (e != hipSuccess) { set_error("hipFuncSetAttribute: %s", hipGetErrorString(e)); return ASVGP_ERR_LDS_CAPACITY; }
          granted = lb;
        }
        if (h->mirror_dev) { ff.mirror = h->mirror_dev; ff.mirror_seq = ++h->mirror_seq; h->mirror_pending = ff.mirror_seq; }
        if (nb >= 128 && !debug_env().no_split) {
          ff.split = 1;
          ff.xchg = w.LP;
        }
        ff.n_helpers = 0;
        const bool plan_first = debug_env().plan_first != 0;
        const bool host_times = debug_env().host_times != 0;
        auto now_us = []() { timespec ts; clock_gettime(CLOCK_MONOTONIC, &ts); return ts.tv_sec * 1e6 + ts.tv_nsec * 1e-3; };
        const double t0 = host_times ? now_us() : 0.0;
        if (plan_first && !gpu_fwd) (void)prior_plan_eval(h->plan, cf.c, cf.dc, tab);
        const ThetaBox* box_k = nullptr;
        if (h->ahead_req) {
          if (gpu_fwd || plan_first) { set_error("launch-ahead needs the host forward pass (asvgp_set_prior_forward(h, 0))"); return ASVGP_ERR_UNSUPPORTED; }
          static_assert(sizeof(ThetaBox) <= BOX_BYTES, "theta box");
          if (!h->box_host) {
            if (hipHostMalloc(&h->box_host, BOX_BYTES * TAB_SLOTS, hipHostMallocMapped | hipHostMallocPortable | hipHostMallocCoherent) != hipSuccess ||
                hipHostGetDevicePointer(&h->box_dev, h->box_host, 0) != hipSuccess) {
              if (h->box_host) { (void)hipHostFree(h->box_host); h->box_host = nullptr; }
              set_error("launch-ahead: pinned allocation failed: %s", hipGetErrorString(hipGetLastError()));
              return ASVGP_ERR_HIP;
            }
            memset(h->box_host, 0, BOX_BYTES * TAB_SLOTS);
          }
          ThetaBox* bh = reinterpret_cast<ThetaBox*>(static_cast<char*>(h->box_host) + (size_t)slot * BOX_BYTES);
          __atomic_store_n(&bh->seq, 0ull, __ATOMIC_RELEASE);
          box_k = reinterpret_cast<const ThetaBox*>(static_cast<const char*>(h->box_dev) + (size_t)slot * BOX_BYTES);
        }
        const bool to_worker = !plan_first && !gpu_fwd && h->fwd_worker && !h->ahead_req;
        if (to_worker) {
          for (int t = 0; t < ASVGP_MAX_KUU_TERMS; ++t) { h->fwd.coef[t] = cf.c[t]; h->fwd.dcoef[t] = cf.dc[t]; }
          h->fwd.tab = tab; h->fwd.slot = slot; h->fwd.seq = seq;
          handle_post_forward(h);
        }
        hipLaunchKernelGGL(kern, dim3(2 + ff.split + ff.n_helpers), dim3(BM_THREADS), lb, st, ki, S, cf, w.Kuu, w.dK, A, b, (int)M, w.bcrP, w.SP, w.alpha, w.logdets, info, s,
                           tab_k, n_rec, h->node_rec_dev, w.bcrK, w.SK, w.dSK, h->done_dev + slot, seq,
                           gpu_fwd ? dd_ready : (plan_first ? (const unsigned long long*)nullptr : h->ready_dev + slot), spin_limit, ff, box_k);
        if (h->ahead_req) {
          h->ahead = Handle::PendingAhead{true, slot, seq, tab, kind, ff.th.N, ff.th.Nw, ff.th.cw};
          return check_launch("elbo chains (matrix cores, launched ahead of theta)");
        }
        if (gpu_fwd) return check_launch("elbo chains (matrix cores, forward pass on the GPU)");
        if (to_worker) return check_launch("elbo chains (matrix cores, forward pass on the worker thread)");
        const double t1 = host_times ? now_us() : 0.0;
        if (!plan_first && h->defer_forward) {
          h->fwd.valid = true;
          for (int t = 0; t < ASVGP_MAX_KUU_TERMS; ++t) { h->fwd.coef[t] = cf.c[t]; h->fwd.dcoef[t] = cf.dc[t]; }
          h->fwd.tab = tab; h->fwd.slot = slot; h->fwd.seq = seq;
          return check_launch("elbo chains (matrix cores, forward pass deferred)");
        }
        if (!plan_first) (void)prior_plan_eval(h->plan, cf.c, cf.dc, tab);
        if (host_times) {
          static double acc_launch = 0.0, acc_plan = 0.0, acc_pre = 0.0, acc_acq = 0.0, acc_a = 0.0;
          acc_acq += t_acq1 - t_acq0; acc_a += t_acq0 - t_enter;
          static long calls = 0;
          const double t2 = now_us();
          acc_pre += t0 - t_enter; acc_launch += t1 - t0; acc_plan += t2 - t1;
          if (++calls % 200 == 0) {
            fprintf(stderr, "[entry -> acquire %.1f us, table acquire %.1f us] ", acc_a / 200, acc_acq / 200);
            acc_a = acc_acq = 0.0;
            fprintf(stderr, "[asvgp host times, mean of 200 calls] entry -> launch call %.1f us | launch call (%s) %.1f us | %s %.1f us\n", acc_pre / 200,
                    plan_first ? "forward pass + hipLaunchKernel" : "hipLaunchKernel", acc_launch / 200, plan_first ? "-" : "forward pass", acc_plan / 200);
            acc_launch = acc_plan = acc_pre = 0.0;
          }
        }
        __atomic_store_n(h->ready_host + slot, seq, __ATOMIC_RELEASE);
      }
    }
    if (!use_mfma) {
    if (!gpu_fwd) {
      (void)prior_plan_eval(h->plan, cf.c, cf.dc, tab);
      __atomic_store_n(h->ready_host + slot, seq, __ATOMIC_RELEASE);
    }
    auto kern = big ? elbo_chains_kernel<K, HAS_BIG> : elbo_chains_kernel<K, false>;
    hipError_t e = hipFuncSetAttribute(reinterpret_cast<const void*>(kern), hipFuncAttributeMaxDynamicSharedMemorySize, (int)lds_bytes);
    if (e != hipSuccess) { set_error("hipFuncSetAttribute: %s", hipGetErrorString(e)); return ASVGP_ERR_LDS_CAPACITY; }
    hipLaunchKernelGGL(kern, dim3(2 + ff.n_helpers), dim3(BCR_THREADS), lds_bytes, st, S, cf, w.Kuu, TANGENT ? w.dK : (double*)nullptr, A, b,
                       (int)M, w.bcrP, w.SP, w.alpha, w.logdets, info, s,
                       tab_k, n_rec, h->node_rec_dev, w.bcrK, w.SK, w.dSK,
                       h->done_dev + slot, seq, (int)D, (int)(lds_bytes / sizeof(double)), ff);
    }
    if (scale_alpha) {
      long n = M * D;
      hipLaunchKernelGGL(scale_kernel, dim3((unsigned)((n + 255) / 256)), dim3(256), 0, st, w.alpha, 1.0 / s, n);
    }
    return check_launch("elbo chains (planned prior)");
  }
  const bool pfly = (part == 2) && use_bcr;
  if (!pfly)
    hipLaunchKernelGGL(elbo_prepare_kernel, dim3((unsigned)((E + 255) / 256)), dim3(256), 0, st, S, cf, E, A, s,
                       part == 2 ? w.LK : w.Kuu, part == 2 ? (double*)nullptr : w.dK, part == 1 ? (double*)nullptr : w.P);
  if (h->sync_on && part == 1) (void)hipEventRecord(h->evK, st);
  if (h->sync_on && part == 2) (void)hipStreamWaitEvent(st, h->evK, 0);
  if (use_bcr) {
    if (!fits) { set_error("BCR forced but needs %zu B of LDS", lds_bytes); return ASVGP_ERR_LDS_CAPACITY; }
    hipError_t e = hipFuncSetAttribute(big ? reinterpret_cast<const void*>(elbo_bcr_kernel<K, TANGENT, HAS_BIG>) : reinterpret_cast<const void*>(elbo_bcr_kernel<K, TANGENT, false>), hipFuncAttributeMaxDynamicSharedMemorySize, (int)lds_bytes);
    if (e != hipSuccess) { set_error("hipFuncSetAttribute: %s", hipGetErrorString(e)); return ASVGP_ERR_LDS_CAPACITY; }
    if (part == 1 && TANGENT) {
      if constexpr (TANGENT) {
        auto kern = big ? elbo_bcr_prior_kernel<K, HAS_BIG> : elbo_bcr_prior_kernel<K, false>;
        e = hipFuncSetAttribute(reinterpret_cast<const void*>(kern), hipFuncAttributeMaxDynamicSharedMemorySize, (int)lds_bytes);
        if (e != hipSuccess) { set_error("hipFuncSetAttribute: %s", hipGetErrorString(e)); return ASVGP_ERR_LDS_CAPACITY; }
        hipLaunchKernelGGL(kern, dim3(1), dim3(BCR_THREADS), lds_bytes, st, w.Kuu, w.dK, (int)M, w.bcrK, w.SK, w.dSK, w.logdets, info,
                           debug_env().bcr_stamps);
      }
    } else if (pfly) {
      auto kern = big ? elbo_bcr_data_kernel<K, HAS_BIG> : elbo_bcr_data_kernel<K, false>;
      e = hipFuncSetAttribute(reinterpret_cast<const void*>(kern), hipFuncAttributeMaxDynamicSharedMemorySize, (int)lds_bytes);
      if (e != hipSuccess) { set_error("hipFuncSetAttribute: %s", hipGetErrorString(e)); return ASVGP_ERR_LDS_CAPACITY; }
      hipLaunchKernelGGL(kern, dim3(1), dim3(BCR_THREADS), lds_bytes, st, w.Kuu, A, b, (int)M, w.bcrP, w.SP, w.alpha, w.logdets, info,
                         debug_env().bcr_stamps, s, (int)D, (int)(lds_bytes / sizeof(double)));
    } else {
      auto kern = big ? elbo_bcr_kernel<K, TANGENT, HAS_BIG> : elbo_bcr_kernel<K, TANGENT, false>;
      hipLaunchKernelGGL(kern, dim3(part == 0 ? 2 : 1), dim3(BCR_THREADS), lds_bytes, st, w.Kuu, w.dK,
                         w.P, b, (int)M, w.bcrK, w.bcrP, w.SK, w.dSK, w.SP, w.alpha, w.logdets, info,
                         debug_env().bcr_stamps, part == 2 ? 1 : 0, (int)D, (int)(lds_bytes / sizeof(double)));
    }
    if (part == 1) {
      if (h->sync_on) (void)hipEventRecord(h->evP, st);
      return check_launch("elbo prior chain");
    }
  } else if (D == 1) {
    hipLaunchKernelGGL((elbo_factor_kernel<K, TANGENT, true>), dim3(2), dim3(64), 0, st, w.Kuu, w.dK, w.P, w.LK, w.dLK,
                       w.LP, b, w.c, (int)M, info);
    hipLaunchKernelGGL((elbo_inverse_kernel<K, TANGENT, true>), dim3(2), dim3(64), 0, st, w.LK, w.dLK, w.LP, w.SK,
                       w.dSK, w.SP, w.c, w.alpha, (int)M);
  } else {
    hipLaunchKernelGGL((elbo_factor_kernel<K, TANGENT, false>), dim3(2), dim3(64), 0, st, w.Kuu, w.dK, w.P, w.LK,
                       w.dLK, w.LP, b, w.c, (int)M, info);
    hipLaunchKernelGGL(elbo_trsv_kernel<K>, dim3((unsigned)D), dim3(64), 0, st, w.LP, (int)M, b, w.c, D, 0, 1.0);
    hipLaunchKernelGGL((elbo_inverse_kernel<K, TANGENT, false>), dim3(2), dim3(64), 0, st, w.LK, w.dLK, w.LP, w.SK,
                       w.dSK, w.SP, w.c, w.alpha, (int)M);
    hipLaunchKernelGGL(elbo_trsv_kernel<K>, dim3((unsigned)D), dim3(64), 0, st, w.LP, (int)M, w.c, w.alpha, D, 1, 1.0);
  }
  long n = M * D;
  if (!use_bcr) hipLaunchKernelGGL(scale_kernel, dim3((unsigned)((n + 255) / 256)), dim3(256), 0, st, w.c, 1.0 / s, n);
  if (!use_bcr || scale_alpha)
    hipLaunchKernelGGL(scale_kernel, dim3((unsigned)((n + 255) / 256)), dim3(256), 0, st, w.alpha, 1.0 / s, n);
  return check_launch("elbo chains");
}

template <int K>
int ElboLauncher<K>::run(Handle* h, const double* stats, const double* S, int kind, double v, double l, double s, long N, long M, long D,
                         double* out, int* info, void* ws, hipStream_t st, int part) {
  {
    Ws w = carve(ws, M, K, D);
    bool bcr = false;
    h->mirror_pending = 0;
    ElboScalars th{v, l, s, (double)N, (double)N, 0.0};
    if (h->w_set) { th.N = h->w_npos; th.Nw = h->w_sum; th.cw = 0.5 * (double)D * h->w_sumlog; }
    const int fin_blocks = (int)((M + 255) / 256 < 64 ? (M + 255) / 256 : 64);
    static_assert(BCR_THREADS == 256, "the fused finalize shares the chain kernel's workgroup size");
    FusedFin ff{stats, th, 1.0 / s, w.fin, reinterpret_cast<unsigned*>(w.fin + 16), reinterpret_cast<unsigned*>(w.fin + 18), nullptr, out, D, 0, 0};
    int rc = run_chains<K, true>(h, stats, S, kind, v, l, s, M, D, w, info, st, bcr, part, false, part == 1 ? nullptr : &ff);
    if (rc || (part == 1)) return rc;
    if (ff.finalize < 0) return check_launch("elbo_grad_1d (fused)");
    if (h->sync_on && part == 2 && bcr && h->evP) (void)hipStreamWaitEvent(st, h->evP, 0);
    hipLaunchKernelGGL(elbo_finalize_kernel<K>, dim3(fin_blocks), dim3(256), 0, st, stats, w.Kuu, w.dK, w.LK, w.LP, w.SK,
                       w.dSK, w.SP, w.c, w.alpha, bcr ? w.logdets : (const double*)nullptr, M, K, D, th,
                       bcr ? 1.0 / s : 1.0, w.fin, reinterpret_cast<unsigned*>(w.fin + 16), out);
    return check_launch("elbo_grad_1d");
  }
}
template <int K>
int PostLauncher<K>::run(Handle* h, const double* stats, const double* S, int kind, double v, double l, double s, long M, long D,
                         double* alpha, double* W, int* info, void* ws, hipStream_t st, double* Pinv) {
  {
    Ws w = carve(ws, M, K, D);
    bool bcr = false;
    int rc = run_chains<K, false>(h, stats, S, kind, v, l, s, M, D, w, info, st, bcr);
    if (rc) return rc;
    long E = (long)(K + 1) * M;
    hipLaunchKernelGGL(scale_sub_kernel, dim3((unsigned)((E + 255) / 256)), dim3(256), 0, st, w.SP, w.SK, W, E);
    hipError_t e = hipMemcpyAsync(alpha, w.alpha, sizeof(double) * M * D, hipMemcpyDeviceToDevice, st);
    if (e == hipSuccess && Pinv) e = hipMemcpyAsync(Pinv, w.SP, sizeof(double) * E, hipMemcpyDeviceToDevice, st);
    if (e != hipSuccess) { set_error("hipMemcpyAsync: %s", hipGetErrorString(e)); return ASVGP_ERR_HIP; }
    return check_launch(Pinv ? "posterior_prepare_loo_1d" : "posterior_prepare_1d");
  }
}

#if !defined(ASVGP_ELBO_PART) || ASVGP_ELBO_PART == 2
static __global__ void cov_recip_kernel(const double* __restrict__ LK, const double* __restrict__ LP, long M, double* __restrict__ rK,
                                        double* __restrict__ rP, const int* __restrict__ finfo, int* __restrict__ info) {
  const long j = (long)blockIdx.x * blockDim.x + threadIdx.x;
  if (j < M) { rK[j] = 1.0 / LK[j]; rP[j] = 1.0 / LP[j]; }
  if (j < 2 && info[j] == 0 && finfo[j] != 0) info[j] = finfo[j];
}

// ... 73 lines not shown
template <int K>
int PostCovLauncher<K>::run(Handle* h, const double* stats, const double* S, int kind, double v, double l, double s, long M, long D,
                            double* alpha, double* W, double* Wd, int* info, void* ws, hipStream_t st) {
  int rc = PostLauncher<K>::run(h, stats, S, kind, v, l, s, M, D, alpha, W, info, ws, st);
  if (rc) return rc;
  const Ws w = carve(ws, M, K, D);
  const long E = (long)(K + 1) * M;
  double* c = static_cast<double*>(ws) + ws_doubles(M, K, D);
  double *Kb = c, *Pb = c + E, *LKb = c + 2 * E, *LPb = c + 3 * E, *rK = c + 4 * E, *rP = rK + M;
  int* finfo = reinterpret_cast<int*>(rP + M);
  KuuCoefs2 cf;
  for (int t = 0; t < ASVGP_MAX_KUU_TERMS; ++t) cf.c[t] = cf.dc[t] = 0.0;
  rc = asvgp_matern_coeffs(kind, v, l, cf.c, cf.dc, &cf.n);
  if (rc) return rc;
  hipLaunchKernelGGL(elbo_prepare_kernel, dim3((unsigned)((E + 255) / 256)), dim3(256), 0, st, S, cf, E, stats, s, Kb, (double*)nullptr, Pb);
  rc = asvgp_cholesky_band(Kb, LKb, M, K, finfo, st);
  if (rc) return rc;
  rc = asvgp_cholesky_band(Pb, LPb, M, K, finfo + 1, st);
  if (rc) return rc;
  hipLaunchKernelGGL(cov_recip_kernel, dim3((unsigned)((M + 255) / 256)), dim3(256), 0, st, LKb, LPb, M, rK, rP, finfo, info);
  hipLaunchKernelGGL(cov_rows_kernel<K>, dim3((unsigned)((M + COV_CH - 1) / COV_CH)), dim3(COV_CH), 0, st, LKb, LPb, rK, rP, w.SK, w.SP, W,
                     (int)M, Wd);
  const unsigned nt = (unsigned)((M + 63) / 64);
  hipLaunchKernelGGL(cov_mirror_kernel, dim3(nt, nt), dim3(256), 0, st, Wd, (int)M);
  return check_launch("posterior_cov_prepare_1d");
}
#endif


template <int K>
__global__ __launch_bounds__(BCR_THREADS) void kuu_inverse_pre_kernel(const double* tab, int n_rec, const int* node_rec, int M, double* wsK,
                                                                      double* SK, double* dSK, double* logdet2, int* info,
                                                                      unsigned long long* done_flag, unsigned long long seq) {
  extern __shared__ double lds[];
  bcr_backward_pre<K>(tab, n_rec, node_rec, M, wsK, lds, BandOut<Dual>{SK, dSK}, logdet2, info, done_flag, seq);
}
template <int K>
__global__ __launch_bounds__(64) void kuu_inverse_sweep_kernel(const double* Kuu, const double* dK, double* LK, double* dLK, double* SK,
                                                               double* dSK, int M, int* info) {
  cholesky_sweep<Dual, K, false>(BandPtr<Dual>{Kuu, dK}, BandOut<Dual>{LK, dLK}, M, nullptr, nullptr, info);
  __syncthreads();
  takahashi_sweep<Dual, K, false>(BandPtr<Dual>{LK, dLK}, BandOut<Dual>{SK, dSK}, M, nullptr, nullptr);
}
static __global__ void kuu_logdet_kernel(const double* __restrict__ LK, const double* __restrict__ dLK, long M, double* __restrict__ out) {
  __shared__ double scratch[32];
  double a = 0.0, b = 0.0;
  for (long j = threadIdx.x; j < M; j += blockDim.x) { const double l = LK[j]; a += log(l * l); b += 2.0 * dLK[j] / l; }
  a = block_sum(a, scratch);
  b = block_sum(b, scratch + 16);
  if (threadIdx.x == 0) { out[0] = a; out[1] = b; }
}

template <int K>
int KuuInvLauncher<K>::run(Handle* h, const double* S, int kind, double v, double l, long M, double* Kuu, double* dK, double* SK,
                           double* dSK, double* logdet2, int* info, void* ws, hipStream_t st) {
  KuuCoefs2 cf;
  for (int t = 0; t < ASVGP_MAX_KUU_TERMS; ++t) cf.c[t] = cf.dc[t] = 0.0;
  int rc = asvgp_matern_coeffs(kind, v, l, cf.c, cf.dc, &cf.n);
  if (rc) return rc;
  Ws w = carve(ws, M, K, 1);
  const long E = (long)(K + 1) * M, nb = (M + K - 1) / K;
  hipLaunchKernelGGL(elbo_prepare_kernel, dim3((unsigned)((E + 255) / 256)), dim3(256), 0, st, S, cf, E, (const double*)nullptr, 1.0, Kuu, dK,
                     (double*)nullptr);
  const bool have_plan = h->plan && prior_plan_M(h->plan) == M && prior_plan_k(h->plan) == K && prior_plan_terms(h->plan) == cf.n;
  if (have_plan && h->band_algo != 1 && h->band_algo != 2) {
    unsigned long long seq = 0;
    int slot = 0;
    double* tab = handle_table_acquire(h, &seq, &slot);
    const double* tab_k = h->tab_dev + (size_t)slot * h->slot_doubles;
    if (h->prior_forward_gpu) {
      double* t = nullptr;
      rc = handle_prior_dd_forward(h, cf.c, cf.dc, slot, st, &t);
      if (rc) return rc;
      tab_k = t;
    } else {
      (void)prior_plan_eval(h->plan, cf.c, cf.dc, tab);
    }
    const int n_rec = prior_plan_nrec(h->plan);
    const size_t lds_bytes = sizeof(double) * bcr_pre_lds_doubles(K, n_rec);
    hipError_t e = hipFuncSetAttribute(reinterpret_cast<const void*>(kuu_inverse_pre_kernel<K>), hipFuncAttributeMaxDynamicSharedMemorySize, (int)lds_bytes);
    if (e != hipSuccess) { set_error("hipFuncSetAttribute: %s", hipGetErrorString(e)); return ASVGP_ERR_LDS_CAPACITY; }
    hipLaunchKernelGGL(kuu_inverse_pre_kernel<K>, dim3(1), dim3(BCR_THREADS), lds_bytes, st, tab_k, n_rec,
                       h->node_rec_dev, (int)M, w.bcrK, SK, dSK, logdet2, info, h->done_dev + slot, seq);
    return check_launch("kuu_inverse_band_1d (planned)");
  }
  const size_t ldsK = sizeof(double) * bcr_lds_doubles<Dual, K, 0>(nb);
  if (ldsK <= 160 * 1024 - 256 && h->band_algo != 1) {
    auto kern = elbo_bcr_prior_kernel<K, false>;
    hipError_t e = hipFuncSetAttribute(reinterpret_cast<const void*>(kern), hipFuncAttributeMaxDynamicSharedMemorySize, (int)ldsK);
    if (e != hipSuccess) { set_error("hipFuncSetAttribute: %s", hipGetErrorString(e)); return ASVGP_ERR_LDS_CAPACITY; }
    hipLaunchKernelGGL(kern, dim3(1), dim3(BCR_THREADS), ldsK, st, Kuu, dK, (int)M, w.bcrK, SK, dSK, logdet2, info, 0);
    return check_launch("kuu_inverse_band_1d (BCR)");
  }
  hipLaunchKernelGGL(kuu_inverse_sweep_kernel<K>, dim3(1), dim3(64), 0, st, Kuu, dK, w.LK, w.dLK, SK, dSK, (int)M, info);
  hipLaunchKernelGGL(kuu_logdet_kernel, dim3(1), dim3(256), 0, st, w.LK, w.dLK, M, logdet2);
  return check_launch("kuu_inverse_band_1d (sweeps)");
}

#if ASVGP_ELBO_ONLY_K == 4 && (!defined(ASVGP_ELBO_PART) || ASVGP_ELBO_PART == 1)
int elbo_publish_theta(Handle* h, double v, double l, double s, bool withdraw) {
  if (!h->ahead.valid) { set_error("publish_theta: no launch is waiting for its theta"); return ASVGP_ERR_BAD_ARG; }
  const Handle::PendingAhead a = h->ahead;
  h->ahead.valid = false;
  ThetaBox* bh = reinterpret_cast<ThetaBox*>(static_cast<char*>(h->box_host) + (size_t)a.slot * BOX_BYTES);
  if (withdraw || !h->plan) {
    __atomic_store_n(&bh->seq, ~0ull, __ATOMIC_RELEASE);
    __atomic_store_n(h->ready_host + a.slot, a.seq, __ATOMIC_RELEASE);
    return ASVGP_OK;
  }
  KuuCoefs2 cf;
  for (int t = 0; t < ASVGP_MAX_KUU_TERMS; ++t) cf.c[t] = cf.dc[t] = 0.0;
  const int rc = asvgp_matern_coeffs(a.kind, v, l, cf.c, cf.dc, &cf.n);
  if (rc) { __atomic_store_n(&bh->seq, ~0ull, __ATOMIC_RELEASE); return rc; }
  constexpr int K = 4;
  long lo = 0, hi = 0, lo2 = 0, hi2 = 0;
  double bnd2[2 * PRIOR_BND_DIAGS * PRIOR_BND];
  for (int i = 0; i < 8; ++i) { bh->k[i] = 0.0; bh->dk[i] = 0.0; }
  prior_plan_interior_kuu(h->plan, cf.c, bh->k, &lo, &hi, bh->bnd);
  prior_plan_interior_kuu(h->plan, cf.dc, bh->dk, &lo2, &hi2, bnd2);
  for (int sd = 0; sd < 2; ++sd)
    for (int d = 0; d <= K; ++d)
      for (int cI = 0; cI < KI_DKB; ++cI)
        bh->dkb[(sd * 5 + d) * KI_DKB + cI] = bnd2[(size_t)(sd * PRIOR_BND_DIAGS + d) * PRIOR_BND + cI];
  for (int t = 0; t < ASVGP_MAX_KUU_TERMS; ++t) bh->dc[t] = cf.dc[t];
  bh->s = s; bh->alpha_scale = 1.0 / s; bh->v = v; bh->l = l; bh->N = a.N; bh->Nw = a.Nw; bh->cw = a.cw;
  __atomic_store_n(&bh->seq, a.seq, __ATOMIC_RELEASE);
  if (h->defer_forward) {
    h->fwd.valid = true;
    for (int t = 0; t < ASVGP_MAX_KUU_TERMS; ++t) { h->fwd.coef[t] = cf.c[t]; h->fwd.dcoef[t] = cf.dc[t]; }
    h->fwd.tab = a.tab; h->fwd.slot = a.slot; h->fwd.seq = a.seq;
    return ASVGP_OK;
  }
  (void)prior_plan_eval(h->plan, cf.c, cf.dc, a.tab);
  __atomic_store_n(h->ready_host + a.slot, a.seq, __ATOMIC_RELEASE);
  return ASVGP_OK;
}
#endif

#if !defined(ASVGP_ELBO_PART) || ASVGP_ELBO_PART == 1
template struct ElboLauncher<ASVGP_ELBO_ONLY_K>;
template struct KuuInvLauncher<ASVGP_ELBO_ONLY_K>;
#endif
#if !defined(ASVGP_ELBO_PART) || ASVGP_ELBO_PART == 2
template struct PostLauncher<ASVGP_ELBO_ONLY_K>;
template struct PostCovLauncher<ASVGP_ELBO_ONLY_K>;
#endif
#endif

}

#ifndef ASVGP_ELBO_ONLY_K
using namespace asvgp;

extern "C" size_t asvgp_elbo_workspace_bytes(int64_t M, int k, int64_t D) {
  if (M < 1 || k < 1 || D < 1) return 0;
  return sizeof(double) * ws_doubles(M, k, D);
}

static int elbo_args_ok(const void* stats, const void* S, const void* out, int64_t M, int k, int64_t D, double v,
                        double l, double s, void* ws, size_t wsb, int* info, const char* who) {
  if (!stats || !S || !out || !info || M < 1 || D < 1 || D > 65535 || !(v > 0.0) || !(l > 0.0) || !(s > 0.0)) {
    set_error("%s: bad argument", who);
    return ASVGP_ERR_BAD_ARG;
  }
  if (k < 1 || k > ASVGP_MAX_ORDER) { set_error("%s: bandwidth %d outside 1..%d", who, k, (int)ASVGP_MAX_ORDER); return ASVGP_ERR_UNSUPPORTED; }
  if (M > 0x3fffffff) { set_error("%s: M too large", who); return ASVGP_ERR_UNSUPPORTED; }
  if (!ws || wsb < asvgp_elbo_workspace_bytes(M, k, D)) { set_error("%s: workspace too small", who); return ASVGP_ERR_WORKSPACE; }
  return ASVGP_OK;
}

extern "C" int asvgp_elbo_grad_1d(asvgp_handle_t handle, const double* stats, const double* static_bands, int kind, double variance,
                                  double lengthscale, double noise_variance, int64_t N, int64_t M, int k, int64_t D,
                                  double* out, int* info, void* workspace, size_t workspace_bytes, asvgp_stream_t stream);
extern "C" int asvgp_result_mirror_read(asvgp_handle_t handle, uint64_t token, double* result10, double timeout_seconds) {
  Handle* h = as_handle(handle);
  if (!result10) { set_error("result_mirror_read: bad argument"); return ASVGP_ERR_BAD_ARG; }
  handle_publish_forward(h);
  if (token == 0 || !h->mirror_host) return 1;
  volatile const double* m = h->mirror_host;
  const double want = (double)token;
  struct timespec t0;
  clock_gettime(CLOCK_MONOTONIC, &t0);
  for (unsigned long spins = 0;; ++spins) {
    if (m[10] == want) {
      double r[12];
      for (int i = 0; i < 12; ++i) r[i] = m[i];
      double sum = want;
      for (int i = 0; i < 10; ++i) sum += r[i];
      if (r[10] == want && (sum == r[11] || r[11] != r[11])) {
        for (int i = 0; i < 10; ++i) result10[i] = r[i];
        return ASVGP_OK;
      }
    }
    __builtin_ia32_pause();
    if ((spins & 1023) == 1023) {
      struct timespec t1;
      clock_gettime(CLOCK_MONOTONIC, &t1);
      if ((double)(t1.tv_sec - t0.tv_sec) + 1e-9 * (double)(t1.tv_nsec - t0.tv_nsec) > timeout_seconds) return 1;
    }
  }
}
extern "C" int asvgp_elbo_grad_ahead_1d(asvgp_handle_t handle, const double* stats, const double* static_bands, int kind, int64_t N, int64_t M,
                                        int k, int64_t D, double* out, int* info, void* workspace, size_t workspace_bytes, asvgp_stream_t stream) {
  Handle* h = as_handle(handle);
  if (h->ahead.valid) { set_error("elbo_grad_ahead_1d: the previous launch still waits for its theta (asvgp_elbo_publish_theta)"); return ASVGP_ERR_BAD_ARG; }
  if (!h->mirror_host) { const double* p = nullptr; const int rcm = asvgp_result_mirror(handle, 1, &p); if (rcm) return rcm; }
  h->ahead_req = true;
  const int rc = asvgp_elbo_grad_1d(handle, stats, static_bands, kind, 1.0, 1.0, 1.0, N, M, k, D, out, info, workspace, workspace_bytes, stream);
  h->ahead_req = false;
  return rc;
}
extern "C" int asvgp_elbo_publish_theta(asvgp_handle_t handle, double variance, double lengthscale, double noise_variance) {
  if (!(variance > 0.0) || !(lengthscale > 0.0) || !(noise_variance > 0.0)) { set_error("elbo_publish_theta: bad argument"); return ASVGP_ERR_BAD_ARG; }
  return elbo_publish_theta(as_handle(handle), variance, lengthscale, noise_variance, false);
}
extern "C" int asvgp_elbo_grad_host_1d(asvgp_handle_t handle, const double* stats, const double* static_bands, int kind, double variance,
                                       double lengthscale, double noise_variance, int64_t N, int64_t M, int k, int64_t D,
                                       double* out, int* info, void* workspace, size_t workspace_bytes, asvgp_stream_t stream,
                                       double* result10, double timeout_seconds) {
  Handle* h = as_handle(handle);
  if (!h->mirror_host) { const double* p = nullptr; const int rcm = asvgp_result_mirror(handle, 1, &p); if (rcm) return rcm; }
  const int rc = asvgp_elbo_grad_1d(handle, stats, static_bands, kind, variance, lengthscale, noise_variance, N, M, k, D, out, info, workspace,
                                    workspace_bytes, stream);
  if (rc) return rc;
  return asvgp_result_mirror_read(handle, h->mirror_pending, result10, timeout_seconds);
}

extern "C" int asvgp_elbo_grad_1d(asvgp_handle_t handle, const double* stats, const double* static_bands, int kind, double variance,
                                  double lengthscale, double noise_variance, int64_t N, int64_t M, int k, int64_t D,
                                  double* out, int* info, void* workspace, size_t workspace_bytes,
                                  asvgp_stream_t stream) {
  int rc = elbo_args_ok(stats, static_bands, out, M, k, D, variance, lengthscale, noise_variance, workspace,
                        workspace_bytes, info, "elbo_grad_1d");
  if (rc) return rc;
  Handle* h = as_handle(handle);
  { const int rcf = handle_flush_phi_reduce(h, stats, as_stream(stream)); if (rcf) return rcf; }
  hipStream_t st = as_stream(stream);
#define ELBO_CASE(KK) case KK: return ElboLauncher<KK>::run(h, stats, static_bands, kind, variance, lengthscale, noise_variance, (long)N, (long)M, (long)D, out, info, workspace, st, 0);
  switch (k) { ELBO_CASE(1) ELBO_CASE(2) ELBO_CASE(3) ELBO_CASE(4) ELBO_CASE(5) ELBO_CASE(6) }
#undef ELBO_CASE
  return ASVGP_ERR_UNSUPPORTED;
}

extern "C" int asvgp_elbo_prior_chain_1d(asvgp_handle_t handle, const double* static_bands, int kind, double variance, double lengthscale,
                                         double noise_variance, int64_t M, int k, int64_t D, int* info, void* workspace,
                                         size_t workspace_bytes, asvgp_stream_t stream) {
  int rc = elbo_args_ok(static_bands, static_bands, static_bands, M, k, D, variance, lengthscale, noise_variance, workspace,
                        workspace_bytes, info, "elbo_prior_chain_1d");
  if (rc) return rc;
  Handle* h = as_handle(handle);
  hipStream_t st = as_stream(stream);
#define ELBO_CASE(KK) case KK: return ElboLauncher<KK>::run(h, nullptr, static_bands, kind, variance, lengthscale, noise_variance, 0, (long)M, (long)D, nullptr, info, workspace, st, 1);
  switch (k) { ELBO_CASE(1) ELBO_CASE(2) ELBO_CASE(3) ELBO_CASE(4) ELBO_CASE(5) ELBO_CASE(6) }
#undef ELBO_CASE
  return ASVGP_ERR_UNSUPPORTED;
}

extern "C" int asvgp_elbo_data_chain_1d(asvgp_handle_t handle, const double* stats, const double* static_bands, int kind, double variance,
                                        double lengthscale, double noise_variance, int64_t N, int64_t M, int k, int64_t D,
                                        double* out, int* info, void* workspace, size_t workspace_bytes,
                                        asvgp_stream_t stream) {
  int rc = elbo_args_ok(stats, static_bands, out, M, k, D, variance, lengthscale, noise_variance, workspace,
                        workspace_bytes, info, "elbo_data_chain_1d");
  if (rc) return rc;
  Handle* h = as_handle(handle);
  { const int rcf = handle_flush_phi_reduce(h, stats, as_stream(stream)); if (rcf) return rcf; }
  hipStream_t st = as_stream(stream);
#define ELBO_CASE(KK) case KK: return ElboLauncher<KK>::run(h, stats, static_bands, kind, variance, lengthscale, noise_variance, (long)N, (long)M, (long)D, out, info, workspace, st, 2);
  switch (k) { ELBO_CASE(1) ELBO_CASE(2) ELBO_CASE(3) ELBO_CASE(4) ELBO_CASE(5) ELBO_CASE(6) }
#undef ELBO_CASE
  return ASVGP_ERR_UNSUPPORTED;
}

extern "C" int asvgp_kuu_inverse_band_1d(asvgp_handle_t handle, const double* static_bands, int kind, double variance, double lengthscale,
                                         int64_t M, int k, double* Kuu, double* dKuu_dl, double* S, double* dS_dl, double* logdet2, int* info,
                                         void* workspace, size_t workspace_bytes, asvgp_stream_t stream) {
  if (!static_bands || !Kuu || !dKuu_dl || !S || !dS_dl || !logdet2 || !info || M < 1 || !(variance > 0.0) || !(lengthscale > 0.0)) {
    set_error("kuu_inverse_band_1d: bad argument");
    return ASVGP_ERR_BAD_ARG;
  }
  if (k < 1 || k > ASVGP_MAX_ORDER) { set_error("kuu_inverse_band_1d: bandwidth %d outside 1..%d", k, (int)ASVGP_MAX_ORDER); return ASVGP_ERR_UNSUPPORTED; }
  if (!workspace || workspace_bytes < asvgp_elbo_workspace_bytes(M, k, 1)) { set_error("kuu_inverse_band_1d: workspace too small"); return ASVGP_ERR_WORKSPACE; }
  Handle* h = as_handle(handle);
  hipStream_t st = as_stream(stream);
#define KINV_CASE(KK) case KK: return KuuInvLauncher<KK>::run(h, static_bands, kind, variance, lengthscale, (long)M, Kuu, dKuu_dl, S, dS_dl, logdet2, info, workspace, st);
  switch (k) { KINV_CASE(1) KINV_CASE(2) KINV_CASE(3) KINV_CASE(4) KINV_CASE(5) KINV_CASE(6) }
#undef KINV_CASE
  return ASVGP_ERR_UNSUPPORTED;
}

extern "C" int asvgp_posterior_prepare_1d(asvgp_handle_t handle, const double* stats, const double* static_bands, int kind, double variance,
                                          double lengthscale, double noise_variance, int64_t M, int k, int64_t D,
                                          double* alpha, double* W, int* info, void* workspace, size_t workspace_bytes,
                                          asvgp_stream_t stream) {
  int rc = elbo_args_ok(stats, static_bands, alpha, M, k, D, variance, lengthscale, noise_variance, workspace,
                        workspace_bytes, info, "posterior_prepare_1d");
  if (rc) return rc;
  if (!W) { set_error("posterior_prepare_1d: bad argument"); return ASVGP_ERR_BAD_ARG; }
  Handle* h = as_handle(handle);
  { const int rcf = handle_flush_phi_reduce(h, stats, as_stream(stream)); if (rcf) return rcf; }
  hipStream_t st = as_stream(stream);
#define POST_CASE(KK) case KK: return PostLauncher<KK>::run(h, stats, static_bands, kind, variance, lengthscale, noise_variance, (long)M, (long)D, alpha, W, info, workspace, st);
  switch (k) { POST_CASE(1) POST_CASE(2) POST_CASE(3) POST_CASE(4) POST_CASE(5) POST_CASE(6) }
#undef POST_CASE
  return ASVGP_ERR_UNSUPPORTED;
}
// ... 46 lines not shown
```

### asvgp_amd/csrc/handle.hip

```cpp
#include <sched.h>
#include <stdlib.h>
#include <string.h>
#include <time.h>

#include <condition_variable>
#include <mutex>
#include <thread>
#include <vector>

#include "handle.hpp"

namespace asvgp {

static DebugEnv g_dbg;
static std::once_flag g_dbg_once;
static void debug_env_load() {
  g_dbg.no_assembly = getenv("ASVGP_DEBUG_NO_ASSEMBLY") ? 1 : 0;
  g_dbg.chain_stamps = getenv("ASVGP_CHAIN_STAMPS") ? 1 : 0;
  g_dbg.spin_limit = getenv("ASVGP_SPIN_LIMIT") ? atol(getenv("ASVGP_SPIN_LIMIT")) : (1L << 25);
  g_dbg.host_times = getenv("ASVGP_HOST_TIMES") ? 1 : 0;
  g_dbg.plan_first = getenv("ASVGP_PLAN_FIRST") ? 1 : 0;
  g_dbg.bcr_stamps = getenv("ASVGP_BCR_STAMPS") ? atoi(getenv("ASVGP_BCR_STAMPS")) : 0;
  g_dbg.no_split = getenv("ASVGP_NO_SPLIT") ? atoi(getenv("ASVGP_NO_SPLIT")) : 0;
}
const DebugEnv& debug_env() {
  std::call_once(g_dbg_once, debug_env_load);
  return g_dbg;
}

static Handle* g_default = nullptr;
static std::mutex g_default_mu;

Handle* as_handle(asvgp_handle_t h) {
  if (h) return reinterpret_cast<Handle*>(h);
  std::lock_guard<std::mutex> lk(g_default_mu);
  if (!g_default) {
    g_default = new Handle;
    (void)hipGetDevice(&g_default->device);
  }
  return g_default;
}

static void handle_quiesce(Handle* h) {
  if (h->ahead.valid) (void)elbo_publish_theta(h, 1.0, 1.0, 1.0, true);
  handle_publish_forward(h);
  bool need_sync = false;
  struct timespec t0;
  clock_gettime(CLOCK_MONOTONIC, &t0);
  auto expired = [&]() { struct timespec t1; clock_gettime(CLOCK_MONOTONIC, &t1); return (t1.tv_sec - t0.tv_sec) > 2; };
  if (h->done_host && h->seq > 0) {
    volatile unsigned long long* flag = h->done_host + (h->seq % TAB_SLOTS);
    while (*flag < h->seq) { sched_yield(); if (expired()) { need_sync = true; break; } }
  }
  if (!need_sync && h->mirror_host && h->mirror_pending) {
    volatile double* m = h->mirror_host + 10;
    while (*m != (double)h->mirror_pending) { sched_yield(); if (expired()) { need_sync = true; break; } }
  }
  if (need_sync) (void)hipDeviceSynchronize();
}

static void plan_release(Handle* h) {
  handle_quiesce(h);
  if (h->plan) { prior_plan_destroy(h->plan); h->plan = nullptr; }
  handle_prior_dd_release(h);
  if (h->node_rec_dev) { (void)hipFree(h->node_rec_dev); h->node_rec_dev = nullptr; }
  if (h->tab_host) { (void)hipHostFree(h->tab_host); h->tab_host = nullptr; h->tab_dev = nullptr; }
  if (h->done_host) { (void)hipHostFree(h->done_host); h->done_host = nullptr; h->done_dev = nullptr; }
  if (h->ready_host) { (void)hipHostFree(h->ready_host); h->ready_host = nullptr; h->ready_dev = nullptr; }
  h->slot_doubles = 0;
}

static void worker_wait_idle(Handle* h) {
  while (__atomic_load_n(&h->wstate, __ATOMIC_ACQUIRE) == 1) sched_yield();
}
struct WorkerPark {
  std::mutex mu;
  std::condition_variable cv;
  int parked = 0;
};
static WorkerPark* park_of(Handle* h) { return static_cast<WorkerPark*>(h->worker_park); }
static void worker_main(Handle* h) {
  long idle = 0;
  WorkerPark* pk = park_of(h);
  for (;;) {
    const int st = __atomic_load_n(&h->wstate, __ATOMIC_ACQUIRE);
    if (st == 2) return;
    if (st == 1) {
      if (h->plan) (void)prior_plan_eval(h->plan, h->fwd.coef, h->fwd.dcoef, h->fwd.tab);
      __atomic_store_n(h->ready_host + h->fwd.slot, h->fwd.seq, __ATOMIC_RELEASE);
      __atomic_store_n(&h->wstate, 0, __ATOMIC_RELEASE);
      idle = 0;
    } else if (++idle > 200000) {
      std::unique_lock<std::mutex> lk(pk->mu);
      pk->parked = 1;
      pk->cv.wait(lk, [&] { return __atomic_load_n(&h->wstate, __ATOMIC_ACQUIRE) != 0; });
      pk->parked = 0;
      idle = 0;
    } else {
      __builtin_ia32_pause();
    }
  }
}
static void worker_signal(Handle* h, int state) {
  WorkerPark* pk = park_of(h);
  __atomic_store_n(&h->wstate, state, __ATOMIC_SEQ_CST);
  bool wake;
  { std::lock_guard<std::mutex> lk(pk->mu); wake = pk->parked != 0; }
  if (wake) pk->cv.notify_one();
}
void handle_post_forward(Handle* h) {
  if (!h->worker) {
    h->worker_park = new WorkerPark;
    h->worker = new std::thread(worker_main, h);
  }
  worker_signal(h, 1);
}
static void worker_stop(Handle* h) {
  if (!h->worker) return;
  worker_wait_idle(h);
  worker_signal(h, 2);
  std::thread* t = static_cast<std::thread*>(h->worker);
  t->join();
  delete t;
  delete park_of(h);
  h->worker_park = nullptr;
  h->worker = nullptr;
  h->wstate = 0;
}

void handle_publish_forward(Handle* h) {
  if (h->worker) worker_wait_idle(h);
  if (!h->fwd.valid) return;
  h->fwd.valid = false;
  if (h->plan) (void)prior_plan_eval(h->plan, h->fwd.coef, h->fwd.dcoef, h->fwd.tab);
  __atomic_store_n(h->ready_host + h->fwd.slot, h->fwd.seq, __ATOMIC_RELEASE);
}

double* handle_table_acquire(Handle* h, unsigned long long* seq_out, int* slot_out) {
  handle_publish_forward(h);
  const unsigned long long seq = ++h->seq;
  const int slot = (int)(seq % TAB_SLOTS);
  if (seq > TAB_SLOTS) {
    const unsigned long long need = seq - TAB_SLOTS;
    volatile unsigned long long* flag = h->done_host + slot;
    struct timespec t0;
    clock_gettime(CLOCK_MONOTONIC, &t0);
    while (*flag < need) {
      sched_yield();
      struct timespec t1;
      clock_gettime(CLOCK_MONOTONIC, &t1);
      if ((t1.tv_sec - t0.tv_sec) > 2) { (void)hipDeviceSynchronize(); break; }
    }
  }
  *seq_out = seq;
  *slot_out = slot;
  return h->tab_host + (size_t)slot * h->slot_doubles;
}

bool handle_mesh_is_linspace(Handle* h, const double* mesh_dev, long n_mesh, hipStream_t st, double* step_out, double* first_out, double* last_out) {
  for (int i = 0; i < h->n_mesh_seen; ++i)
    if (h->mesh_seen[i].ptr == mesh_dev && h->mesh_seen[i].n == n_mesh) {
      *step_out = h->mesh_seen[i].step;
      if (first_out) *first_out = h->mesh_seen[i].first;
      if (last_out) *last_out = h->mesh_seen[i].last;
      return h->mesh_seen[i].regular != 0;
    }
  std::vector<double> m((size_t)n_mesh);
  bool regular = false;
  double step = 0.0, first = 0.0, last = 0.0;
  if (n_mesh >= 2 && hipMemcpyAsync(m.data(), mesh_dev, sizeof(double) * (size_t)n_mesh, hipMemcpyDeviceToHost, st) == hipSuccess &&
      hipStreamSynchronize(st) == hipSuccess) {
    const double m0 = m[0];
    first = m0; last = m[n_mesh - 1];
    step = (m[n_mesh - 1] - m0) / (double)(n_mesh - 1);
    regular = step > 0.0 && step == step;
    for (long i = 0; i < n_mesh - 1 && regular; ++i) {
      volatile double t = (double)i * step;
      regular = (m[i] == t + m0);
    }
  }
  if (h->n_mesh_seen < 8) h->mesh_seen[h->n_mesh_seen++] = Handle::MeshSeen{mesh_dev, n_mesh, regular ? 1 : 0, step, first, last};
  *step_out = step;
  if (first_out) *first_out = first;
  if (last_out) *last_out = last;
  return regular;
}

}

using namespace asvgp;

extern "C" int asvgp_prior_interior_kuu_host(const double* static_bands_host, int n_terms, int64_t M, int k, const double* coef_host,
                                             double* kuu_diag8, int64_t* lo, int64_t* hi, double* bnd256) {
  if (!coef_host || !kuu_diag8 || !lo || !hi || !bnd256) { set_error("prior_interior_kuu_host: bad argument"); return ASVGP_ERR_BAD_ARG; }
  char err[256] = "";
  PriorPlan* p = prior_plan_create(static_bands_host, n_terms, (long)M, k, err, sizeof(err));
  if (!p) { set_error("%s", err); return strstr(err, "bad argument") ? ASVGP_ERR_BAD_ARG : ASVGP_ERR_UNSUPPORTED; }
  long l = 0, h = 0;
  for (int i = 0; i < 8; ++i) kuu_diag8[i] = 0.0;
  for (int i = 0; i < 2 * PRIOR_BND_DIAGS * PRIOR_BND; ++i) bnd256[i] = 0.0;
  prior_plan_interior_kuu(p, coef_host, kuu_diag8, &l, &h, bnd256);
  *lo = l; *hi = h;
  prior_plan_destroy(p);
  return ASVGP_OK;
}

extern "C" int asvgp_host_mantissa_bits(void) { return prior_plan_mantissa_bits(); }

extern "C" int asvgp_debug_reload_env(void) {
  asvgp::debug_env_load();
  return ASVGP_OK;
}

extern "C" int asvgp_create(asvgp_handle_t* out) {
  if (!out) { set_error("asvgp_create: bad argument"); return ASVGP_ERR_BAD_ARG; }
  Handle* h = new Handle;
  if (hipGetDevice(&h->device) != hipSuccess) { delete h; set_error("asvgp_create: no HIP device"); return ASVGP_ERR_HIP; }
  *out = reinterpret_cast<asvgp_handle_t>(h);
  return ASVGP_OK;
}

extern "C" int asvgp_destroy(asvgp_handle_t handle) {
  if (!handle) return ASVGP_OK;
  Handle* h = reinterpret_cast<Handle*>(handle);
  if (h->magic != 0x41535647u) { set_error("asvgp_destroy: not a handle"); return ASVGP_ERR_BAD_ARG; }
  worker_stop(h);
  plan_release(h);
  if (h->mirror_host) (void)hipHostFree(h->mirror_host);
  if (h->evK) (void)hipEventDestroy(h->evK);
  if (h->evP) (void)hipEventDestroy(h->evP);
  if (h->prof_made)
    for (int i = 0; i < PROF_RING; ++i) { (void)hipEventDestroy(h->prof_ev[i][0]); (void)hipEventDestroy(h->prof_ev[i][1]); }
  if (h->order_dev) { (void)hipFree(h->order_dev); h->order_dev = nullptr; }
  if (h->box_host) { (void)hipHostFree(h->box_host); h->box_host = nullptr; h->box_dev = nullptr; }
  h->magic = 0;
  delete h;
  return ASVGP_OK;
}

extern "C" int asvgp_set_phi_algorithm(asvgp_handle_t handle, int algo) {
  if (algo != 0 && algo != 1 && algo != 3 && algo != 5 && algo != 6) {
    set_error("set_phi_algorithm: 0 auto (6 where it applies, else 5, else 3), 1 fp64 LDS-atomic band scatter, 3 fixed-point band scatter, 5 fixed-point centred-moment scatter, 6 tile sort + register moments");
    return ASVGP_ERR_BAD_ARG;
  }
  as_handle(handle)->phi_algo = algo;
  return ASVGP_OK;
}

extern "C" int asvgp_set_phi_input_order(asvgp_handle_t handle, int order) {
  if (order < 0 || order > 2) { set_error("set_phi_input_order: 0 probe once per (x, N), 1 unsorted, 2 time series"); return ASVGP_ERR_BAD_ARG; }
  Handle* h = as_handle(handle);
  h->phi_order = order;
  h->n_order_seen = 0;
  return ASVGP_OK;
}

extern "C" int asvgp_phi_last_input_order(asvgp_handle_t handle) { return as_handle(handle)->phi_last_series ? 2 : 1; }

extern "C" int asvgp_set_phi_workgroups(asvgp_handle_t handle, int n) {
  if (n < 0 || n > 256) { set_error("set_phi_workgroups: 0 (default, one per CU) .. 256"); return ASVGP_ERR_BAD_ARG; }
  as_handle(handle)->phi_blocks = n;
  return ASVGP_OK;
}

extern "C" int asvgp_set_weight_sums(asvgp_handle_t handle, double n_pos, double sum_w, double sum_log_w) {
  Handle* h = as_handle(handle);
  if (n_pos < 0.0) { h->w_set = false; h->w_npos = h->w_sum = h->w_sumlog = 0.0; return ASVGP_OK; }
  if (!(n_pos == n_pos) || n_pos != (double)(long long)n_pos || n_pos > 9.0e15 || !(sum_w >= 0.0) || !(sum_w < 1e300) || !(fabs(sum_log_w) < 1e300)) {
    set_error("set_weight_sums: n_pos must be a whole number of rows (negative: unweighted), sum_w >= 0 and sum_log_w finite");
    return ASVGP_ERR_BAD_ARG;
  }
  h->w_set = true; h->w_npos = n_pos; h->w_sum = sum_w; h->w_sumlog = sum_log_w;
  return ASVGP_OK;
}

extern "C" int asvgp_set_phi_deferred_reduce(asvgp_handle_t handle, int on) {
  Handle* h = as_handle(handle);
  h->phi_defer = on != 0;
  if (!h->phi_defer) h->pend.valid = false;
  return ASVGP_OK;
}

extern "C" int asvgp_set_band_algorithm(asvgp_handle_t handle, int algo) {
  if (algo < 0 || algo > 4) {
    set_error("set_band_algorithm: 0 auto, 1 sequential sweeps, 2 block cyclic reduction on the GPU, 3 block cyclic reduction with the planned (host, long double) prior forward pass, 4 the planned chains on the matrix cores");
    return ASVGP_ERR_BAD_ARG;
  }
  as_handle(handle)->band_algo = algo;
  return ASVGP_OK;
}

extern "C" int asvgp_set_deferred_forward_pass(asvgp_handle_t handle, int on) {
  Handle* h = as_handle(handle);
  if (on < 0 || on > 2) { set_error("set_deferred_forward_pass: 0 inline, 1 the caller publishes (asvgp_prior_publish), 2 the handle's worker thread"); return ASVGP_ERR_BAD_ARG; }
  handle_publish_forward(h);
  if (on != 2) worker_stop(h);
  h->defer_forward = on == 1;
  h->fwd_worker = on == 2;
  return ASVGP_OK;
}

extern "C" int asvgp_prior_publish(asvgp_handle_t handle) {
  handle_publish_forward(as_handle(handle));
  return ASVGP_OK;
}

extern "C" int asvgp_result_mirror(asvgp_handle_t handle, int enable, const double** host_ptr) {
  Handle* h = as_handle(handle);
  if (enable && !h->mirror_host) {
    if (hipHostMalloc(reinterpret_cast<void**>(&h->mirror_host), sizeof(double) * 16, hipHostMallocMapped | hipHostMallocPortable | hipHostMallocCoherent) != hipSuccess ||
        hipHostGetDevicePointer(reinterpret_cast<void**>(&h->mirror_dev), h->mirror_host, 0) != hipSuccess) {
      if (h->mirror_host) { (void)hipHostFree(h->mirror_host); h->mirror_host = nullptr; }
      h->mirror_dev = nullptr;
      set_error("result_mirror: pinned allocation failed: %s", hipGetErrorString(hipGetLastError()));
      return ASVGP_ERR_HIP;
    }
    memset(h->mirror_host, 0, sizeof(double) * 16);
  }
  if (!enable && h->mirror_host) {
    handle_quiesce(h);
    (void)hipHostFree(h->mirror_host);
    h->mirror_host = nullptr; h->mirror_dev = nullptr; h->mirror_pending = 0;
  }
  if (host_ptr) *host_ptr = h->mirror_host;
  return ASVGP_OK;
}

extern "C" uint64_t asvgp_result_mirror_pending(asvgp_handle_t handle) { return as_handle(handle)->mirror_pending; }

extern "C" int asvgp_elbo_chain_sync(asvgp_handle_t handle, int enable) {
  Handle* h = as_handle(handle);
  if (enable && !h->evK) {
    if (hipEventCreateWithFlags(&h->evK, hipEventDisableTiming | hipEventReleaseToDevice) != hipSuccess ||
        hipEventCreateWithFlags(&h->evP, hipEventDisableTiming | hipEventReleaseToDevice) != hipSuccess) {
      set_error("elbo_chain_sync: hipEventCreate failed");
      return ASVGP_ERR_HIP;
    }
  }
  h->sync_on = enable != 0;
  return ASVGP_OK;
}

extern "C" int asvgp_profile_enable(asvgp_handle_t handle, int on) {
  Handle* h = as_handle(handle);
  if (on && !h->prof_made) {
    for (int i = 0; i < PROF_RING; ++i)
      for (int j = 0; j < 2; ++j)
        if (hipEventCreateWithFlags(&h->prof_ev[i][j], hipEventReleaseToDevice) != hipSuccess) { set_error("hipEventCreate failed"); return ASVGP_ERR_HIP; }
    h->prof_made = true;
  }
  h->prof_on = on != 0;
  h->prof_every = on > 1 ? on : 1;
  h->prof_calls = 0;
  h->prof_n = 0;
  return ASVGP_OK;
}

extern "C" int asvgp_profile_read(asvgp_handle_t handle, double* phi_kernel_ms_sum, int64_t* launches) {
  Handle* h = as_handle(handle);
  if (!phi_kernel_ms_sum || !launches) { set_error("profile_read: bad argument"); return ASVGP_ERR_BAD_ARG; }
  double tot = 0.0;
  for (long i = 0; i < h->prof_n; ++i) {
    if (hipEventSynchronize(h->prof_ev[i][1]) != hipSuccess) { set_error("hipEventSynchronize failed"); return ASVGP_ERR_HIP; }
    float ms = 0.f;
    (void)hipEventElapsedTime(&ms, h->prof_ev[i][0], h->prof_ev[i][1]);
    tot += ms;
  }
  *phi_kernel_ms_sum = tot;
  *launches = h->prof_n;
  h->prof_n = 0;
  return ASVGP_OK;
}

extern "C" int asvgp_prior_plan_1d(asvgp_handle_t handle, const double* static_bands_host, int n_terms, int64_t M, int k,
                                   int* planned) {
  Handle* h = as_handle(handle);
  if (planned) *planned = 0;
  plan_release(h);
  if (!static_bands_host) return ASVGP_OK;
  char err[256] = "";
  PriorPlan* p = prior_plan_create(static_bands_host, n_terms, (long)M, k, err, sizeof(err));
  if (!p) {
    if (strstr(err, "bad argument")) { set_error("%s", err); return ASVGP_ERR_BAD_ARG; }
    return ASVGP_OK;
  }
  const int nb = prior_plan_nb(p);
  h->slot_doubles = (prior_plan_table_doubles(p) + 63) / 64 * 64;
  bool ok = hipMalloc(reinterpret_cast<void**>(&h->node_rec_dev), sizeof(int) * (size_t)nb) == hipSuccess &&
            hipMemcpy(h->node_rec_dev, prior_plan_node_rec(p), sizeof(int) * (size_t)nb, hipMemcpyHostToDevice) == hipSuccess &&
            hipHostMalloc(reinterpret_cast<void**>(&h->tab_host), sizeof(double) * h->slot_doubles * TAB_SLOTS, hipHostMallocMapped | hipHostMallocPortable | hipHostMallocCoherent) == hipSuccess &&
            hipHostGetDevicePointer(reinterpret_cast<void**>(&h->tab_dev), h->tab_host, 0) == hipSuccess &&
            hipHostMalloc(reinterpret_cast<void**>(&h->done_host), sizeof(unsigned long long) * TAB_SLOTS, hipHostMallocMapped | hipHostMallocPortable | hipHostMallocCoherent) == hipSuccess &&
            hipHostGetDevicePointer(reinterpret_cast<void**>(&h->done_dev), h->done_host, 0) == hipSuccess &&
            hipHostMalloc(reinterpret_cast<void**>(&h->ready_host), sizeof(unsigned long long) * TAB_SLOTS, hipHostMallocMapped | hipHostMallocPortable | hipHostMallocCoherent) == hipSuccess &&
            hipHostGetDevicePointer(reinterpret_cast<void**>(&h->ready_dev), h->ready_host, 0) == hipSuccess;
  if (!ok) {
    prior_plan_destroy(p);
    plan_release(h);
    set_error("prior_plan_1d: device / pinned allocation failed: %s", hipGetErrorString(hipGetLastError()));
    return ASVGP_ERR_HIP;
  }
  for (int i = 0; i < TAB_SLOTS; ++i) { h->done_host[i] = h->seq; h->ready_host[i] = h->seq; }
  h->plan = p;
  h->plan_terms = n_terms;
  if (planned) *planned = 1;
  return ASVGP_OK;
}

extern "C" size_t asvgp_prior_table_doubles(const double* static_bands_host, int n_terms, int64_t M, int k) {
  char err[256];
  PriorPlan* p = prior_plan_create(static_bands_host, n_terms, (long)M, k, err, sizeof(err));
  if (!p) return 0;
  const size_t n = prior_plan_table_doubles(p);
  prior_plan_destroy(p);
  return n;
}

extern "C" int asvgp_prior_forward_host(const double* static_bands_host, int n_terms, int64_t M, int k, const double* coef_host,
                                        const double* dcoef_dl_host, double* table_host, size_t table_doubles, int* node_rec_host) {
  if (!coef_host || !dcoef_dl_host || !table_host || !node_rec_host) { set_error("prior_forward_host: bad argument"); return ASVGP_ERR_BAD_ARG; }
  char err[256] = "";
  PriorPlan* p = prior_plan_create(static_bands_host, n_terms, (long)M, k, err, sizeof(err));
  if (!p) { set_error("%s", err); return strstr(err, "bad argument") ? ASVGP_ERR_BAD_ARG : ASVGP_ERR_UNSUPPORTED; }
  if (table_doubles < prior_plan_table_doubles(p)) { prior_plan_destroy(p); set_error("prior_forward_host: table too small"); return ASVGP_ERR_WORKSPACE; }
  (void)prior_plan_eval(p, coef_host, dcoef_dl_host, table_host);
  memcpy(node_rec_host, prior_plan_node_rec(p), sizeof(int) * (size_t)prior_plan_nb(p));
  prior_plan_destroy(p);
  return ASVGP_OK;
}

extern "C" int asvgp_prior_plan_image_host(const double* static_bands_host, int n_terms, int64_t M, int k, int* ints, size_t* n_ints,
                                           double* doubles, size_t* n_doubles) {
  if (!n_ints || !n_doubles) { set_error("prior_plan_image_host: bad argument"); return ASVGP_ERR_BAD_ARG; }
  char err[256] = "";
  PriorPlan* p = prior_plan_create(static_bands_host, n_terms, (long)M, k, err, sizeof(err));
  if (!p) { set_error("%s", err); return strstr(err, "bad argument") ? ASVGP_ERR_BAD_ARG : ASVGP_ERR_UNSUPPORTED; }
  const size_t ni = prior_plan_image_ints(p), nd = prior_plan_image_doubles(p);
  int rc = ASVGP_OK;
  if (ints && doubles) {
    if (*n_ints < ni || *n_doubles < nd) { set_error("prior_plan_image_host: buffers too small"); rc = ASVGP_ERR_WORKSPACE; }
    else prior_plan_image(p, ints, doubles);
  }
// ... 5 lines not shown
```

### asvgp_amd/csrc/handle.hpp

```cpp
#pragma once
#include "asvgp_common.hpp"
#include "prior_plan.hpp"

namespace asvgp {

constexpr int PROF_RING = 1024;
constexpr int TAB_SLOTS = 16;

struct Handle {
  unsigned magic = 0x41535647u;
  int device = 0;
  int phi_algo = 0, phi_blocks = 0;
  int phi_last = 0;
  bool phi_defer = false;
  struct PendingReduce { const double* partials; int G, M, K; double* stats; bool valid; const int* ranges; } pend = {nullptr, 0, 0, 0, nullptr, false, nullptr};
  int band_algo = 0;
  bool sync_on = false;
  hipEvent_t evK = nullptr, evP = nullptr;
  bool prof_on = false, prof_made = false;
  int prof_every = 1;
  long prof_calls = 0, prof_n = 0;
  hipEvent_t prof_ev[PROF_RING][2];
  PriorPlan* plan = nullptr;
  int* node_rec_dev = nullptr;
  double* tab_host = nullptr;
  double* tab_dev = nullptr;
  unsigned long long* done_host = nullptr;
  unsigned long long* done_dev = nullptr;
  unsigned long long* ready_host = nullptr;
  unsigned long long* ready_dev = nullptr;
  size_t slot_doubles = 0;
  unsigned long long seq = 0;
  int plan_terms = 0;
  bool defer_forward = false;
  bool fwd_worker = false;
  void* worker = nullptr;
  void* worker_park = nullptr;
  int wstate = 0;
  struct PendingForward { bool valid; double coef[ASVGP_MAX_KUU_TERMS], dcoef[ASVGP_MAX_KUU_TERMS]; double* tab; int slot; unsigned long long seq; } fwd = {false, {0}, {0}, nullptr, 0, 0};
  bool prior_forward_gpu = false;
  int* dd_img_i = nullptr;
  int dd_n_img = 0;
  double* dd_img_d = nullptr;
  double* dd_tab = nullptr;
  hipStream_t dd_stream = nullptr;
  unsigned long long* dd_ready = nullptr;
  double* mirror_host = nullptr;
  double* mirror_dev = nullptr;
  unsigned long long mirror_seq = 0;
  unsigned long long mirror_pending = 0;
  struct MeshSeen { const double* ptr; long n; int regular; double step, first, last; };
  MeshSeen mesh_seen[8];
  int n_mesh_seen = 0;
  int phi_order = 0;
  struct OrderSeen { const double* ptr; long n; int series; };
  OrderSeen order_seen[8];
  int n_order_seen = 0;
  int* order_dev = nullptr;
  int phi_last_series = 0;
  bool ahead_req = false;
  void* box_host = nullptr;
  void* box_dev = nullptr;
  struct PendingAhead { bool valid; int slot; unsigned long long seq; double* tab; int kind; double N, Nw, cw; } ahead = {false, 0, 0, nullptr, 0, 0.0, 0.0, 0.0};
  bool w_set = false;
  double w_npos = 0.0, w_sum = 0.0, w_sumlog = 0.0;
};
constexpr size_t BOX_BYTES = 4096;

struct DebugEnv { int no_assembly; int chain_stamps; long spin_limit; int host_times; int plan_first; int bcr_stamps; int no_split; };
const DebugEnv& debug_env();

Handle* as_handle(asvgp_handle_t h);

bool handle_mesh_is_linspace(Handle* h, const double* mesh_dev, long n_mesh, hipStream_t st, double* step_out, double* first_out, double* last_out);

int handle_flush_phi_reduce(Handle* h, const double* stats, hipStream_t st);

void handle_publish_forward(Handle* h);
void handle_post_forward(Handle* h);

int handle_prior_dd_prepare(Handle* h);
void handle_prior_dd_release(Handle* h);
int handle_prior_dd_forward(Handle* h, const double* coef, const double* dcoef, int slot, hipStream_t st, double** tab_out, unsigned long long* stamps = nullptr,
                            unsigned long long seq = 0, const unsigned long long** ready_out = nullptr);

int elbo_publish_theta(Handle* h, double v, double l, double s, bool withdraw);

double* handle_table_acquire(Handle* h, unsigned long long* seq_out, int* slot_out);

}
```

### include/asvgp_hip.h

```cpp
#ifndef ASVGP_HIP_H
#define ASVGP_HIP_H

#include <stddef.h>
#include <stdint.h>

#ifdef __cplusplus
extern "C" {
#endif

typedef void* asvgp_stream_t;
typedef struct asvgp_handle_s* asvgp_handle_t;

typedef enum {
  ASVGP_OK = 0,
  ASVGP_ERR_BAD_ARG = -1,
  ASVGP_ERR_UNSUPPORTED = -2,
  ASVGP_ERR_LDS_CAPACITY = -3,
  ASVGP_ERR_WORKSPACE = -4,
  ASVGP_ERR_HIP = -5
} asvgp_status;

enum { ASVGP_MATERN12 = 0, ASVGP_MATERN32 = 1, ASVGP_MATERN52 = 2 };
enum { ASVGP_MAX_ORDER = 6, ASVGP_MAX_BANDWIDTH = 8, ASVGP_MAX_KUU_TERMS = 9 };

int asvgp_version(void);
const char* asvgp_last_error_string(void);
const char* asvgp_status_name(int status);

int asvgp_create(asvgp_handle_t* handle_out);
int asvgp_destroy(asvgp_handle_t handle);

size_t asvgp_phi_workspace_bytes(int64_t M, int order, int64_t D);
int asvgp_phi_accumulate_1d(asvgp_handle_t handle, const double* x, const double* y, int64_t N, int64_t D,
                            const double* mesh, int64_t n_mesh, double delta, int order, int64_t M,
                            double* stats, void* workspace, size_t workspace_bytes, asvgp_stream_t stream);

int asvgp_set_phi_algorithm(asvgp_handle_t handle, int algo);
int asvgp_prior_interior_kuu_host(const double* static_bands_host, int n_terms, int64_t M, int k, const double* coef_host,
                                  double* kuu_diag8, int64_t* lo, int64_t* hi, double* bnd256);
int asvgp_host_mantissa_bits(void);
int asvgp_debug_reload_env(void);
int asvgp_set_deferred_forward_pass(asvgp_handle_t handle, int on);
int asvgp_prior_publish(asvgp_handle_t handle);
int asvgp_result_mirror(asvgp_handle_t handle, int enable, const double** host_ptr);
uint64_t asvgp_result_mirror_pending(asvgp_handle_t handle);
int asvgp_result_mirror_read(asvgp_handle_t handle, uint64_t token, double* result10, double timeout_seconds);
int asvgp_elbo_grad_ahead_1d(asvgp_handle_t handle, const double* stats, const double* static_bands, int kind, int64_t N, int64_t M, int k,
                             int64_t D, double* out, int* info, void* workspace, size_t workspace_bytes, asvgp_stream_t stream);
int asvgp_elbo_publish_theta(asvgp_handle_t handle, double variance, double lengthscale, double noise_variance);
int asvgp_elbo_grad_host_1d(asvgp_handle_t handle, const double* stats, const double* static_bands, int kind, double variance,
                            double lengthscale, double noise_variance, int64_t N, int64_t M, int k, int64_t D,
                            double* out, int* info, void* workspace, size_t workspace_bytes, asvgp_stream_t stream,
                            double* result10, double timeout_seconds);
int asvgp_phi_last_algorithm(asvgp_handle_t handle);
int asvgp_set_phi_input_order(asvgp_handle_t handle, int order);
int asvgp_phi_last_input_order(asvgp_handle_t handle);
int asvgp_stream_probe(const double* x, const double* y, int64_t N, double* sink, asvgp_stream_t stream);
int asvgp_set_phi_workgroups(asvgp_handle_t handle, int n);
int asvgp_set_phi_deferred_reduce(asvgp_handle_t handle, int on);
int asvgp_phi_reduce_1d(asvgp_handle_t handle, asvgp_stream_t stream);

size_t asvgp_phi_weighted_workspace_bytes(int64_t M, int order, int64_t D);
int asvgp_phi_accumulate_1d_weighted(asvgp_handle_t handle, const double* x, const double* y, const double* w, int64_t N, int64_t D,
                                     const double* mesh, int64_t n_mesh, double delta, int order, int64_t M, double* stats,
                                     double* wstats, void* workspace, size_t workspace_bytes, asvgp_stream_t stream);
int asvgp_set_weight_sums(asvgp_handle_t handle, double n_pos, double sum_w, double sum_log_w);

int asvgp_phi_index_1d(const double* x, int64_t N, const double* mesh, int64_t n_mesh, double delta,
                       int64_t* idx, asvgp_stream_t stream);

int asvgp_phi_evaluate_1d(const double* x, int64_t N, const double* mesh, int64_t n_mesh, double delta,
                          int order, int deriv, int64_t* rows, double* data, asvgp_stream_t stream);

int asvgp_matern_coeffs(int kind, double variance, double lengthscale, double* coef_host, double* dcoef_dl_host,
                        int* n_terms_host);
int asvgp_kuu_assemble(const double* static_bands, int n_terms, const double* coef_host,
                       const double* dcoef_dl_host, int64_t M, int k, double* Kuu, double* dKuu_dl,
                       asvgp_stream_t stream);

int asvgp_cholesky_band(const double* K, double* L, int64_t M, int k, int* info, asvgp_stream_t stream);
int asvgp_inverse_from_cholesky_band(const double* L, double* S, int64_t M, int k, asvgp_stream_t stream);
int asvgp_solve_triang_mat(const double* L, const double* B, double* X, int64_t M, int k, int64_t D,
                           int transpose_left, asvgp_stream_t stream);
int asvgp_product_band_band(const double* left, const double* right, double* out, int64_t M,
                            int left_lower, int left_upper, int right_lower, int right_upper,
                            int result_lower, int result_upper, asvgp_stream_t stream);
int asvgp_transpose_band(const double* in, double* out, int64_t M, int lower, int upper, asvgp_stream_t stream);
int asvgp_symmetrise_band(const double* in, double* out, int64_t M, int lower, asvgp_stream_t stream);
int asvgp_unpack_banded_matrix_to_dense(const double* band, double* dense, int64_t M, int lower, int upper,
                                        asvgp_stream_t stream);
int asvgp_pack_dense_matrix_to_banded(const double* dense, double* band, int64_t M, int lower, int upper,
                                      asvgp_stream_t stream);
int asvgp_band_trace_sym(const double* S, const double* A, int64_t M, int k, double* out, asvgp_stream_t stream);

int asvgp_cholesky_band_vjp(const double* L, const double* Lbar, double* Kbar, double* work, int64_t M, int k, asvgp_stream_t stream);
int asvgp_inverse_from_cholesky_band_vjp(const double* L, const double* S, const double* Sbar, double* Lbar, double* work, int64_t M,
                                         int k, asvgp_stream_t stream);
int asvgp_band_outer_product(const double* U, const double* V, int64_t M, int64_t D, int k, double sign, double* out, asvgp_stream_t stream);

size_t asvgp_elbo_workspace_bytes(int64_t M, int k, int64_t D);
int asvgp_set_band_algorithm(asvgp_handle_t handle, int algo);
int asvgp_prior_plan_1d(asvgp_handle_t handle, const double* static_bands_host, int n_terms, int64_t M, int k, int* planned);
size_t asvgp_prior_table_doubles(const double* static_bands_host, int n_terms, int64_t M, int k);
int asvgp_prior_forward_host(const double* static_bands_host, int n_terms, int64_t M, int k, const double* coef_host,
                             const double* dcoef_dl_host, double* table_host, size_t table_doubles, int* node_rec_host);
int asvgp_set_prior_forward(asvgp_handle_t handle, int mode);
int asvgp_prior_forward_device(asvgp_handle_t handle, const double* coef_host, const double* dcoef_dl_host, double* table_host,
                               size_t table_doubles, void* stream);
int asvgp_prior_plan_image_host(const double* static_bands_host, int n_terms, int64_t M, int k, int* ints, size_t* n_ints,
                                double* doubles, size_t* n_doubles);
int asvgp_prior_forward_stamps(asvgp_handle_t handle, const double* coef_host, const double* dcoef_dl_host, uint64_t* out64, void* stream);
int asvgp_elbo_grad_1d(asvgp_handle_t handle, const double* stats, const double* static_bands, int kind, double variance,
                       double lengthscale, double noise_variance, int64_t N, int64_t M, int k, int64_t D,
                       double* out, int* info, void* workspace, size_t workspace_bytes, asvgp_stream_t stream);

int asvgp_kuu_inverse_band_1d(asvgp_handle_t handle, const double* static_bands, int kind, double variance, double lengthscale,
                              int64_t M, int k, double* Kuu, double* dKuu_dl, double* S, double* dS_dl, double* logdet2, int* info,
                              void* workspace, size_t workspace_bytes, asvgp_stream_t stream);

int asvgp_elbo_chain_sync(asvgp_handle_t handle, int enable);
int asvgp_elbo_prior_chain_1d(asvgp_handle_t handle, const double* static_bands, int kind, double variance, double lengthscale,
                              double noise_variance, int64_t M, int k, int64_t D, int* info, void* workspace,
                              size_t workspace_bytes, asvgp_stream_t stream);
int asvgp_elbo_data_chain_1d(asvgp_handle_t handle, const double* stats, const double* static_bands, int kind, double variance,
                             double lengthscale, double noise_variance, int64_t N, int64_t M, int k, int64_t D,
                             double* out, int* info, void* workspace, size_t workspace_bytes, asvgp_stream_t stream);

int asvgp_posterior_prepare_1d(asvgp_handle_t handle, const double* stats, const double* static_bands, int kind, double variance,
                               double lengthscale, double noise_variance, int64_t M, int k, int64_t D,
                               double* alpha, double* W, int* info, void* workspace, size_t workspace_bytes,
                               asvgp_stream_t stream);
int asvgp_predict_1d(const double* xnew, int64_t n, const double* mesh, int64_t n_mesh, double delta, int order,
                     int64_t M, const double* alpha, const double* W, double variance, int64_t D, double* mean,
                     double* var, asvgp_stream_t stream);
int asvgp_predict_1d_h(asvgp_handle_t handle, const double* xnew, int64_t n, const double* mesh, int64_t n_mesh, double delta, int order,
                       int64_t M, const double* alpha, const double* W, double variance, int64_t D, double* mean,
                       double* var, asvgp_stream_t stream);

size_t asvgp_posterior_cov_workspace_bytes(int64_t M, int k, int64_t D);
int asvgp_posterior_cov_prepare_1d(asvgp_handle_t handle, const double* stats, const double* static_bands, int kind, double variance,
                                   double lengthscale, double noise_variance, int64_t M, int k, int64_t D,
                                   double* alpha, double* W, double* W_dense, int* info, void* workspace, size_t workspace_bytes,
                                   asvgp_stream_t stream);
int asvgp_predict_cov_1d(asvgp_handle_t handle, const double* x1, int64_t n1, const double* x2, int64_t n2, const double* mesh,
                         int64_t n_mesh, double delta, int order, int64_t M, const double* W_dense, int kind, double variance,
                         double lengthscale, double* cov, int64_t ldc, asvgp_stream_t stream);

int asvgp_predict_deriv_1d(asvgp_handle_t handle, const double* xnew, int64_t n, const double* mesh, int64_t n_mesh, double delta,
                           int order, int64_t M, const double* alpha, const double* W, int kind, double variance, double lengthscale,
                           int64_t D, double* mean, double* var, asvgp_stream_t stream);
int asvgp_predict_cov_deriv_1d(asvgp_handle_t handle, const double* x1, int64_t n1, const double* x2, int64_t n2, const double* mesh,
                               int64_t n_mesh, double delta, int order, int64_t M, const double* W_dense, int kind, double variance,
                               double lengthscale, int p, int q, double* cov, int64_t ldc, asvgp_stream_t stream);

int asvgp_posterior_prepare_loo_1d(asvgp_handle_t handle, const double* stats, const double* static_bands, int kind, double variance,
                                   double lengthscale, double noise_variance, int64_t M, int k, int64_t D,
                                   double* alpha, double* W, double* Pinv_band, int* info, void* workspace, size_t workspace_bytes,
                                   asvgp_stream_t stream);
size_t asvgp_loo_workspace_bytes(int64_t M, int order, int64_t D);
int asvgp_loo_1d(asvgp_handle_t handle, const double* x, const double* y, const double* w, int64_t N, int64_t D, const double* mesh,
                 int64_t n_mesh, double delta, int order, int64_t M, const double* alpha, const double* W, const double* Pinv_band,
                 double variance, double noise_variance, double* mean, double* var, double* logdens, double* scores,
                 void* workspace, size_t workspace_bytes, asvgp_stream_t stream);

size_t asvgp_kron_stats_doubles(int64_t m1, int64_t m2, int k);
int asvgp_phi_accumulate_kron2d(const double* X, const double* y, int64_t N, const double* mesh1, int64_t n_mesh1,
                                double delta1, int64_t m1, const double* mesh2, int64_t n_mesh2, double delta2,
                                int64_t m2, int order, double* stats, asvgp_stream_t stream);
int asvgp_kron_evaluate_2d(const double* X, int64_t N, const double* mesh1, int64_t n_mesh1, double delta1,
                           const double* mesh2, int64_t n_mesh2, double delta2, int64_t m2, int order, int64_t* rows,
                           double* data, asvgp_stream_t stream);
int asvgp_kron_assemble(const double* K1, const double* K2, const double* S1, const double* S2, const double* Ablk, int k,
                        int64_t m1, int64_t m2, double noise_variance, double* Pb, double* trace_out,
                        asvgp_stream_t stream);
int asvgp_blockband_cholesky(double* Pb, int64_t M, int64_t bw, double* rhs, double* logdet, int* info,
                             asvgp_stream_t stream);
int asvgp_blockband_backsolve(const double* Lb, int64_t M, int64_t bw, double* x, asvgp_stream_t stream);
int asvgp_predict_kron2d(const double* Xnew, int64_t n, const double* mesh1, int64_t n_mesh1, double delta1, int64_t m1,
                         const double* mesh2, int64_t n_mesh2, double delta2, int64_t m2, int order, const double* alpha,
                         const double* S1, const double* S2, double* mean, double* qk, asvgp_stream_t stream);

int asvgp_kron_cell_index(const double* X, int64_t N, const double* mesh1, int64_t n_mesh1, double delta1,
                          const double* mesh2, int64_t n_mesh2, double delta2, int* cell, asvgp_stream_t stream);
int asvgp_phi_accumulate_kron2d_sorted(const double* Xs, const double* ys, int64_t N, const int64_t* cell_start,
                                       const double* mesh1, int64_t n_mesh1, double delta1, int64_t m1,
                                       const double* mesh2, int64_t n_mesh2, double delta2, int64_t m2, int order,
                                       double* stats, asvgp_stream_t stream);
int asvgp_phi_accumulate_kron2d_sorted_f32(const float* Xs, const float* ys, int64_t N, const int64_t* cell_start,
                                           const double* mesh1, int64_t n_mesh1, double delta1, int64_t m1,
                                           const double* mesh2, int64_t n_mesh2, double delta2, int64_t m2, int order,
                                           double* stats, asvgp_stream_t stream);
int asvgp_phi_accumulate_kron2d_weighted(const double* X, const double* y, const double* w, int64_t N, const double* mesh1, int64_t n_mesh1,
                                         double delta1, int64_t m1, const double* mesh2, int64_t n_mesh2, double delta2,
                                         int64_t m2, int order, double* stats, double* wstats, asvgp_stream_t stream);
// ... 64 lines not shown
```

Baseline: 118,400.

## Offload level-0 block cyclic reduction of P solve to helper workgroups

Adds extra helper workgroups to the fused ELBO kernel. They compute the first block-cyclic-reduction level of the P band solve in parallel shares and post the results to a global staging area as tagged messages. The main solver waits a bounded time to import these results and falls back to computing level 0 itself if they do not arrive. This spreads the level-0 elimination across more compute units. In exchange it costs extra workgroups, a staging buffer, spin-wait polling and a miss counter.

After: 106,400. 10.1% lower.

```diff
diff --git a/asvgp_amd/_lib.py b/asvgp_amd/_lib.py
--- a/asvgp_amd/_lib.py
+++ b/asvgp_amd/_lib.py
@@ -63,6 +63,9 @@
     "asvgp_prior_table_doubles": (_Z, [_P, _I, _L, _I]),
     "asvgp_prior_forward_host": (_I, [_P, _I, _L, _I, _P, _P, _P, _Z, _P]),
     "asvgp_set_prior_forward": (_I, [_P, _I]),
+    "asvgp_set_p_helpers": (_I, [_P, _I]),
+    "asvgp_p_helper_misses": (_c.c_int64, [_P]),
+    "asvgp_p_helper_shares": (_I, [_L, _I, _c.POINTER(_I), _I]),
     "asvgp_prior_forward_device": (_I, [_P, _P, _P, _P, _Z, _P]),
     "asvgp_prior_forward_stamps": (_I, [_P, _P, _P, _P, _P]),
     "asvgp_prior_plan_image_host": (_I, [_P, _I, _L, _I, _P, _P, _P, _P]),
@@ -181,6 +184,12 @@
               "prior_forward_device")
         return tab
 
+    def set_p_helpers(self, n):
+        check(self._lib.asvgp_set_p_helpers(self.ptr, int(n)), "set_p_helpers")
+
+    def p_helper_misses(self):
+        return int(self._lib.asvgp_p_helper_misses(self.ptr))
+
     def set_band_algorithm(self, algo):
         check(self._lib.asvgp_set_band_algorithm(self.ptr, int(algo)), "set_band_algorithm")
         self.band_algorithm = int(algo)
@@ -250,6 +259,13 @@
 
     def __del__(self):
         self.close()
+
+
+def p_helper_shares(nb, n_helpers):
+    lib = get_lib()
+    buf = (_I * (4 * 64))()
+    n = lib.asvgp_p_helper_shares(int(nb), int(n_helpers), buf, 64)
+    return [tuple(buf[4 * s: 4 * s + 4]) for s in range(min(n, 64))]
 
 
 def set_default_algorithms(band=None, phi=None, prior_forward=None, phi_order=None):
diff --git a/asvgp_amd/csrc/bcr_mfma.hpp b/asvgp_amd/csrc/bcr_mfma.hpp
--- a/asvgp_amd/csrc/bcr_mfma.hpp
+++ b/asvgp_amd/csrc/bcr_mfma.hpp
@@ -86,8 +86,246 @@
   long spin_limit = 0;
   int* gave_up = nullptr;
   unsigned long long tag = 0;
+  int help = 0;
+  double* stage = nullptr;
+  long help_wait = 0;
+  unsigned long long t0 = 0;
+  int* miss = nullptr;
+  unsigned long long* miss_ctr = nullptr;
 };
 constexpr int BM_XCHG = 96;
+
+struct BmShare { int half, m_lo, m_hi, halo; };
+constexpr int BM_SHARE_MAX = 128;
+constexpr int BM_STAGE_BOX = 40;
+__host__ __device__ inline int bm_sep_node(int nb) {
+  int levels = 0;
+  while ((1 << levels) < nb) ++levels;
+  return 1 << (levels > 1 ? levels - 1 : 0);
+}
+__host__ __device__ inline int bm_half_shares(int n, int want) {
+  if (n <= 0) return 0;
+  int k = want < 1 ? 1 : (want > n ? n : want);
+  while (!(k == 1 ? n <= BM_SHARE_MAX : (n + k - 1) / k + 1 <= BM_SHARE_MAX)) ++k;
+  return k;
+}
+__host__ __device__ inline int bm_helper_share(int nb, int H, int s, BmShare* out) {
+  const int ht = bm_sep_node(nb), ne0 = nb / 2;
+  const int nL = ne0 < ht / 2 ? ne0 : ht / 2, nR = ne0 - nL;
+  if (H < 1 || ne0 < 1) return 0;
+  int hL = H, hR = 0;
+  if (nR > 0) {
+    hL = H < 2 ? 1 : (H * nL + ne0 / 2) / ne0;
+    hL = hL < 1 ? 1 : (hL > H - 1 && H >= 2 ? H - 1 : hL);
+    hR = H < 2 ? 1 : H - hL;
+    if (hR > nR) { hR = nR; hL = H - hR; }
+  }
+  const int sL = bm_half_shares(nL, hL), sR = bm_half_shares(nR, hR);
+  if (s >= 0 && s < sL + sR && out) {
+    const int half = s < sL ? 0 : 1, idx = half ? s - sL : s, k = half ? sR : sL, base = half ? nL : 0, n = half ? nR : nL;
+    out->half = half;
+    out->m_lo = base + (int)((long)idx * n / k);
+    out->m_hi = base + (int)((long)(idx + 1) * n / k);
+    out->halo = idx > 0 ? 1 : 0;
+  }
+  return sL + sR;
+}
+__host__ __device__ inline size_t bcr_mfma_stage_doubles(long nb) { return (size_t)((nb + 1) / 2 + 2) * BM_STAGE_BOX; }
+__host__ __device__ inline size_t bcr_mfma_helper_lds_doubles(long nb) {
+  const long rows = ((nb + 1) / 2 < BM_SHARE_MAX ? (nb + 1) / 2 : BM_SHARE_MAX) + 2;
+  return (size_t)(BM_THREADS / 64) * 4 * 40 + (size_t)rows * 60;
+}
+
+struct BmL0Out {
+  double* stage = nullptr;
+  double* upd = nullptr;
+  int halo = 0;
+  const double* rhs = nullptr;
+  int rhs_stride = 1;
+};
+
+template <bool HELPER, typename Src>
+__device__ __attribute__((always_inline)) void bm_level0(const Src& A, int M, int nb, int m0, int ne_h, double* ws, double* Dl, double* El, double* xs,
+                                                         double* slab_base, int& bad, BmLog& ld, BmL0Out ho) {
+  constexpr int B = BM_B;
+  constexpr int NR = HELPER ? BM_SHARE_MAX / 64 : 4;
+  const int tid = threadIdx.x;
+  const int lane = tid & 63, wv = __builtin_amdgcn_readfirstlane(tid >> 6);
+  const int r = lane >> 4, q = (lane >> 2) & 3, c = lane & 3;
+  const int e = r * 4 + c;
+  const int hi = r > c ? r : c, lo = r > c ? c : r;
+  double* slab = slab_base + (size_t)(wv * 4 + q) * 40;
+  double updb[NR], ybu[NR];
+  int qv = q, ev = e;
+  asm volatile("" : "+v"(qv), "+v"(ev));
+  double sl[2][3], yg[2][2];
+  auto slab_loads = [&](int rd0) __attribute__((always_inline)) {
+#pragma unroll
+    for (int u = 0; u < 2; ++u) {
+      int m = (rd0 + u) * 64 + wv * 4 + qv;
+      m = m0 + (m < ne_h ? m : ne_h - 1);
+#pragma unroll
+      for (int t3 = 0; t3 < 3; ++t3) {
+        sl[u][t3] = 0.0;
+        const int kk = ev + 16 * t3, dd = kk >> 3, col = m * 2 * B + (kk & 7);
+        const bool in = kk < 40 && col + dd < M;
+        const double v = bm_src_load(A, in ? dd : 0, in ? col : 0, (long)M, 0);
+        sl[u][t3] = in ? v : ((dd == 0) ? 1.0 : 0.0);
+      }
+      if (HELPER) {
+#pragma unroll
+        for (int t2 = 0; t2 < 2; ++t2) {
+          const int row = (2 * m + t2) * B + (ev >> 2);
+          const double v = ho.rhs[(long)(row < M ? row : M - 1) * ho.rhs_stride];
+          yg[u][t2] = row < M ? v : 0.0;
+        }
+      }
+    }
+  };
+  if (ne_h > 0) {
+#pragma unroll
+    for (int rd = 0; rd < NR; ++rd) {
+      __builtin_amdgcn_sched_barrier(0);
+      if ((rd & 1) == 0 && rd * 64 < ne_h) slab_loads(rd);
+      updb[rd] = 0.0; ybu[rd] = 0.0;
+      if (rd * 64 + wv * 4 >= ne_h) continue;
+      const int ml = rd * 64 + wv * 4 + q;
+      const bool act = ml < ne_h;
+      const int i = 1 + (m0 + (act ? ml : ne_h - 1)) * 2, a = i - 1, b = i + 1;
+      const bool hasb = b < nb;
+      double d[10];
+#pragma unroll
+      for (int t3 = 0; t3 < 3; ++t3) if (e + 16 * t3 < 40) slab[e + 16 * t3] = sl[rd & 1][t3];
+      int kk = 0;
+#pragma unroll
+      for (int rr = 0; rr < 4; ++rr)
+#pragma unroll
+        for (int cc = 0; cc <= rr; ++cc) d[kk++] = slab[(rr - cc) * 8 + 4 + cc];
+      double ea = slab[(4 + lo - hi) * 8 + hi];
+      ea = (r <= c) ? ea : 0.0;
+      double eb = slab[(4 + lo - hi) * 8 + 4 + hi];
+      eb = (hasb && c <= r) ? eb : 0.0;
+      const double da = slab[(hi - lo) * 8 + lo];
+      double yv, ya;
+      if (HELPER) { yv = yg[rd & 1][1]; ya = yg[rd & 1][0]; }
+      else { yv = xs[i * B + r]; ya = xs[a * B + r]; }
+      yv = (c == 0) ? yv : 0.0;
+      ya = (c == 0) ? ya : 0.0;
+      double dprod;
+      int badj;
+      const double t = bm_chol_linv(d, hi, lo, dprod, badj);
+      if (!HELPER && act && badj && !bad) bad = i * B + badj;
+      const double linv = (r >= c) ? t : 0.0;
+      const double linvT = (c >= r) ? t : 0.0;
+      if (!HELPER && act) ld.mul(dprod);
+      const double ua = bm_mfma(linvT, ea, 0.0);
+      const double ub = bm_mfma(linvT, eb, 0.0);
+      const double zz = bm_mfma(linvT, yv, 0.0);
+      const double nua = -ua, nub = -ub;
+      const double da_new = bm_mfma(nua, ua, da);
+      const double e_new = bm_mfma(nub, ua, 0.0);
+      const double ya_new = bm_mfma(nua, zz, ya);
+      updb[rd] = bm_mfma(ub, ub, 0.0);
+      ybu[rd] = bm_mfma(ub, zz, 0.0);
+      updb[rd] = act ? updb[rd] : 0.0;
+      ybu[rd] = act ? ybu[rd] : 0.0;
+      const double gat = bm_mfma(ua, linv, 0.0);
+      const double gbt = bm_mfma(ub, linv, 0.0);
+      const double dinv = bm_mfma(linv, linv, 0.0);
+      const double w = bm_mfma(linv, zz, 0.0);
+      if (act) {
+        double* R = ws + (size_t)i * BM_REC;
+        if (HELPER) {
+          if (ml >= ho.halo) {
+            __hip_atomic_store(R + BM_GAT + e, gat, __ATOMIC_RELAXED, __HIP_MEMORY_SCOPE_AGENT);
+            __hip_atomic_store(R + BM_GBT + e, gbt, __ATOMIC_RELAXED, __HIP_MEMORY_SCOPE_AGENT);
+            __hip_atomic_store(R + BM_DINV + e, dinv, __ATOMIC_RELAXED, __HIP_MEMORY_SCOPE_AGENT);
+            if (c == 0) __hip_atomic_store(R + BM_W + r, w, __ATOMIC_RELAXED, __HIP_MEMORY_SCOPE_AGENT);
+          }
+          double* S = ho.stage + (size_t)ml * 40;
+          double* U = ho.upd + (size_t)ml * 20;
+          S[e] = da_new; S[16 + e] = e_new; U[e] = updb[rd];
+          if (c == 0) { S[32 + r] = ya_new; U[16 + r] = ybu[rd]; }
+          if (e == 0) { S[36] = dprod; S[37] = (double)badj; }
+        } else {
+          R[BM_GAT + e] = gat; R[BM_GBT + e] = gbt; R[BM_DINV + e] = dinv;
+          if (c == 0) R[BM_W + r] = w;
+          Dl[(size_t)(a >> 1) * 16 + e] = da_new;
+          El[(size_t)(a >> 1) * 16 + e] = e_new;
+          if (c == 0) xs[a * B + r] = ya_new;
+        }
+      }
+    }
+  }
+  bcr_lds_barrier();
+  if (HELPER) return;
+#pragma unroll
+  for (int rd = 0; rd < NR; ++rd) {
+    if (rd * 64 + wv * 4 >= ne_h) continue;
+    const int ml = rd * 64 + wv * 4 + q;
+    const int i = 1 + (m0 + ml) * 2, b = i + 1;
+    if (ml < ne_h && b < nb) {
+      Dl[(size_t)(b >> 1) * 16 + e] -= updb[rd];
+      if (c == 0) xs[b * B + r] -= ybu[rd];
+    }
+  }
+  bcr_lds_barrier();
+}
+
+template <typename Src>
+__device__ __attribute__((always_inline)) void bcr_mfma_level0_helper(Src A, const double* rhs, int M, double* ws, double* lds, double* stage_g,
+                                                                       unsigned long long tag, int n_helpers, int k, int rhs_stride = 1,
+                                                                       double* stamp = nullptr) {
+  constexpr int B = BM_B;
+  const int tid = threadIdx.x;
+  const int lane = tid & 63, wv = __builtin_amdgcn_readfirstlane(tid >> 6);
+  const int nb = (M + B - 1) / B, nslot = (nb + 1) / 2, ne0 = nb / 2, ht = bm_sep_node(nb);
+  const int nL = ne0 < ht / 2 ? ne0 : ht / 2;
+  double* slab_base = lds;
+  double* stg = slab_base + (size_t)(BM_THREADS / 64) * 4 * 40;
+  const int rows = (nslot < BM_SHARE_MAX ? nslot : BM_SHARE_MAX) + 2;
+  double* upd = stg + (size_t)rows * 40;
+  BmShare sh{0, 0, 0, 0};
+  const int n_sh = bm_helper_share(nb, n_helpers, -1, nullptr);
+  for (int s = k; s < n_sh; s += n_helpers) {
+    bm_helper_share(nb, n_helpers, s, &sh);
+    const int m_first = sh.m_lo - sh.halo, nloc = sh.m_hi - m_first;
+    if (nloc <= 0 || nloc > BM_SHARE_MAX) continue;
+    int xnode = -1;
+    if (sh.half == 0 && sh.m_hi == nL) xnode = ht < nb ? ht : -1;
+    else if (sh.half == 1 && sh.m_hi == ne0 && (nb & 1)) xnode = nb - 1;
+    const bool xband = sh.half == 1;
+    if (xnode >= 0 && tid < 40) {
+      double v = 0.0;
+      if (tid < 16 && xband) {
+        const int rr = tid >> 2, cc = tid & 3, hi2 = rr > cc ? rr : cc, lo2 = rr > cc ? cc : rr;
+        const int col = xnode * B + lo2, row = xnode * B + hi2;
+        const bool pad = row >= M;
+        const double bv = bm_src_load(A, hi2 - lo2, pad ? 0 : col, (long)M, 0);
+        v = pad ? ((hi2 == lo2) ? 1.0 : 0.0) : bv;
+      } else if (tid >= 32 && tid < 36 && xband) {
+        const int row = xnode * B + tid - 32;
+        v = row < M ? rhs[(long)row * rhs_stride] : 0.0;
+      } else if (tid == 36) {
+        v = 1.0;
+      }
+      stg[(size_t)nloc * 40 + tid] = v;
+    }
+    int bad = 0;
+    BmLog ld{1.0, 0};
+    bm_level0<true>(A, M, nb, m_first, nloc, ws, nullptr, nullptr, nullptr, slab_base, bad, ld, BmL0Out{stg, upd, sh.halo, rhs, rhs_stride});
+    if (stamp && tid == 0 && s == k) stamp[0] = (double)(__builtin_amdgcn_s_memrealtime() & 0xffffffffull);
+    const int nmsg = nloc - sh.halo + (xnode >= 0 ? 1 : 0);
+    for (int u = wv; u < nmsg; u += BM_THREADS / 64) {
+      const int j = sh.halo + u;
+      double v = lane < 38 ? stg[(size_t)j * 40 + lane] : 0.0;
+      if (j >= 1 && (lane < 16 || (lane >= 32 && lane < 36))) v -= upd[(size_t)(j - 1) * 20 + (lane < 16 ? lane : lane - 16)];
+      const int box = j < nloc ? m_first + j : (sh.half == 0 ? nslot : xnode >> 1);
+      bm_msg_send(stage_g + (size_t)box * BM_STAGE_BOX, 38, v, tag, lane);
+    }
+    __syncthreads();
+  }
+}
 
 template <typename Src>
 __device__ __attribute__((always_inline)) void bcr_mfma_solve(Src A, const double* rhs, int M, double* ws, double* lds, double* Sband, double* x,
@@ -105,7 +343,6 @@
   double* El = lds + (size_t)(nslot + 1) * 16;
   double* xs = El + (size_t)(nslot + 1) * 16;
   double* red = xs + (size_t)nb * B;
-  double* slab = red + 96 + (size_t)(wv * 4 + q) * 40;
   double* Fl = red + 96 + (size_t)(BM_THREADS / 64) * 4 * 40;
   double* Sl = lds;
   int levels = 0;
@@ -159,7 +396,76 @@
   stamp();
 
   constexpr int RMAXR = 4;
-  for (int l = 0; l < levels; ++l) {
+  if (levels > 0) {
+    int m0, ne_h;
+    level_share(0, nb / 2, m0, ne_h);
+    double* slab_base = red + 96;
+    bool imported = false;
+    if (split && sp.help) {
+      const bool xtra = sp.half == 0 ? true : ((nb & 1) && ne_h > 0);
+      const int nbox = ne_h + (xtra ? 1 : 0);
+      constexpr int NT = (BM_SHARE_MAX + 1 + BM_THREADS / 64 - 1) / (BM_THREADS / 64);
+      unsigned long long wd[NT];
+      auto box_of = [&](int j) -> int { return j < ne_h ? m0 + j : (sp.half == 0 ? nslot : nb >> 1); };
+      const unsigned long long mtag = sp.tag | 6ull;
+      bool ok = nbox <= NT * (BM_THREADS / 64);
+      while (ok) {
+#pragma unroll
+        for (int t = 0; t < NT; ++t) {
+          wd[t] = 0ull;
+          const int j = wv + t * (BM_THREADS / 64);
+          if (j < nbox && lane <= 38)
+            wd[t] = __hip_atomic_load(reinterpret_cast<const unsigned long long*>(sp.stage + (size_t)box_of(j) * BM_STAGE_BOX) + lane, __ATOMIC_RELAXED, __HIP_MEMORY_SCOPE_AGENT);
+        }
+        bool all = true;
+#pragma unroll
+        for (int t = 0; t < NT; ++t) {
+          if (wv + t * (BM_THREADS / 64) >= nbox) continue;
+          const unsigned long long x = bm_wave_xor(lane < 38 ? wd[t] : 0ull) ^ mtag;
+          const unsigned long long chk = (unsigned long long)__shfl((long long)wd[t], 38, 64);
+          all = all && (x == chk);
+        }
+        if (all) break;
+        if ((long)(__builtin_amdgcn_s_memrealtime() - sp.t0) > sp.help_wait) { ok = false; break; }
+        __builtin_amdgcn_s_sleep(1);
+      }
+      if (!ok && lane == 0) *sp.miss = 1;
+      __syncthreads();
+      imported = *sp.miss == 0;
+      if (imported) {
+        double* dpl = slab_base;
+        double* bjl = slab_base + BM_SHARE_MAX;
+#pragma unroll
+        for (int t = 0; t < NT; ++t) {
+          const int j = wv + t * (BM_THREADS / 64);
+          if (j >= nbox) continue;
+          const int an = j < ne_h ? 2 * (m0 + j) : (sp.half == 0 ? ht : nb - 1);
+          const double v = __longlong_as_double((long long)wd[t]);
+          if (lane < 16) Dl[(size_t)(an >> 1) * 16 + lane] = v;
+          else if (lane < 32) El[(size_t)(an >> 1) * 16 + lane - 16] = v;
+          else if (lane < 36) xs[an * B + lane - 32] = v;
+          else if (lane == 36 && j < ne_h) dpl[j] = v;
+          else if (lane == 37 && j < ne_h) bjl[j] = v;
+        }
+        bcr_lds_barrier();
+#pragma unroll
+        for (int rd = 0; rd < BM_SHARE_MAX / 64; ++rd) {
+          const int ml = rd * 64 + wv * 4 + q;
+          if (ml < ne_h) {
+            const int badj = (int)bjl[ml];
+            if (badj && !bad) bad = (1 + (m0 + ml) * 2) * B + badj;
+            ld.mul(dpl[ml]);
+          }
+        }
+      } else if (tid == 0 && sp.miss_ctr) {
+        const unsigned long long old = __hip_atomic_exchange(sp.miss_ctr + 1, sp.tag, __ATOMIC_RELAXED, __HIP_MEMORY_SCOPE_AGENT);
+        if (old != sp.tag) __hip_atomic_fetch_add(sp.miss_ctr, 1ull, __ATOMIC_RELAXED, __HIP_MEMORY_SCOPE_AGENT);
+      }
+    }
+    if (!imported) bm_level0<false>(A, M, nb, m0, ne_h, ws, Dl, El, xs, slab_base, bad, ld, BmL0Out{});
+    stamp();
+  }
+  for (int l = 1; l < levels; ++l) {
     const int h = 1 << l;
     const int ne = (nb > h) ? (nb - h + 2 * h - 1) / (2 * h) : 0;
     int m0, ne_h;
@@ -199,51 +505,18 @@
       stamp();
     }
     double updb[RMAXR], ybu[RMAXR];
-    int qv = q, ev = e;
-    asm volatile("" : "+v"(qv), "+v"(ev));
-    double sl[2][3];
-    auto slab_loads = [&](int rd0) __attribute__((always_inline)) {
-#pragma unroll
-      for (int u = 0; u < 2; ++u) {
-#pragma unroll
-        for (int t3 = 0; t3 < 3; ++t3) {
-          sl[u][t3] = 0.0;
-          int m = (rd0 + u) * 64 + wv * 4 + qv;
-          m = m0 + (m < ne_h ? m : ne_h - 1);
-          const int kk = ev + 16 * t3, dd = kk >> 3, col = m * 2 * B + (kk & 7);
-          const bool in = kk < 40 && col + dd < M;
-          const double v = bm_src_load(A, in ? dd : 0, in ? col : 0, (long)M, 0);
-          sl[u][t3] = in ? v : ((dd == 0) ? 1.0 : 0.0);
-        }
-      }
-    };
 #pragma unroll
     for (int rd = 0; rd < RMAXR; ++rd) {
       __builtin_amdgcn_sched_barrier(0);
-      if (l == 0 && (rd & 1) == 0) slab_loads(rd);
       updb[rd] = 0.0; ybu[rd] = 0.0;
       if (rd * 64 + wv * 4 >= ne_h) continue;
       const int ml = rd * 64 + wv * 4 + q;
       const bool act = ml < ne_h;
       const int i = h + (m0 + (act ? ml : ne_h - 1)) * 2 * h, a = i - h, b = i + h;
       const bool hasb = b < nb;
-      const int bsafe = hasb ? b : a;
       double d[10];
       double ea, eb, da;
-      if (l == 0) {
-#pragma unroll
-        for (int t3 = 0; t3 < 3; ++t3) if (e + 16 * t3 < 40) slab[e + 16 * t3] = sl[rd & 1][t3];
-        int kk = 0;
-#pragma unroll
-        for (int rr = 0; rr < 4; ++rr)
-#pragma unroll
-          for (int cc = 0; cc <= rr; ++cc) d[kk++] = slab[(rr - cc) * 8 + 4 + cc];
-        ea = slab[(4 + lo - hi) * 8 + hi];
-        ea = (r <= c) ? ea : 0.0;
-        eb = slab[(4 + lo - hi) * 8 + 4 + hi];
-        eb = (hasb && c <= r) ? eb : 0.0;
-        da = slab[(hi - lo) * 8 + lo];
-      } else {
+      {
         const double* Di = Dl + (size_t)(i >> 1) * 16;
         int kk = 0;
 #pragma unroll
@@ -258,7 +531,6 @@
       double yv = xs[i * B + r], ya = xs[a * B + r];
       yv = (c == 0) ? yv : 0.0;
       ya = (c == 0) ? ya : 0.0;
-      (void)bsafe;
       double dprod;
       int badj;
       const double t = bm_chol_linv(d, hi, lo, dprod, badj);
@@ -370,6 +642,12 @@
       if (l >= 3) {
         const double* R = Fl + (size_t)(i >> 3) * 52;
         gat = R[e]; gbt = R[16 + e]; dinv = R[32 + e]; w = R[48 + r];
+      } else if (l == 0 && sp.help) {
+        const double* R = rec(i);
+        gat = __hip_atomic_load(R + BM_GAT + e, __ATOMIC_RELAXED, __HIP_MEMORY_SCOPE_AGENT);
+        gbt = __hip_atomic_load(R + BM_GBT + e, __ATOMIC_RELAXED, __HIP_MEMORY_SCOPE_AGENT);
+        dinv = __hip_atomic_load(R + BM_DINV + e, __ATOMIC_RELAXED, __HIP_MEMORY_SCOPE_AGENT);
+        w = __hip_atomic_load(R + BM_W + r, __ATOMIC_RELAXED, __HIP_MEMORY_SCOPE_AGENT);
       } else {
         const double* R = rec(i);
         gat = R[BM_GAT + e]; gbt = R[BM_GBT + e]; dinv = R[BM_DINV + e]; w = R[BM_W + r];
diff --git a/asvgp_amd/csrc/elbo.hip b/asvgp_amd/csrc/elbo.hip
--- a/asvgp_amd/csrc/elbo.hip
+++ b/asvgp_amd/csrc/elbo.hip
@@ -333,7 +333,11 @@
   long D; int n_helpers; int finalize; int debug_no_assembly; int debug_stamps;
   double* mirror; unsigned long long mirror_seq;
   int split; double* xchg;
+  int p_helpers; double* stage; long help_wait; unsigned long long* miss_ctr; int debug_no_publish;
 };
+constexpr int P_HELPERS_MAX = 13;
+constexpr int P_HELPERS_AUTO = 0;
+constexpr long P_HELPER_WAIT_TICKS = 2000;
 constexpr int FIN_GACC_PR = 21;
 __device__ __forceinline__ void assemble_band_slice(const double* __restrict__ S, const double* __restrict__ coef, const double* __restrict__ dcoef, int n_terms,
                                                     long E, long e, double* __restrict__ Kuu, double* __restrict__ dK) {
@@ -417,15 +421,15 @@
   extern __shared__ double lds[];
   static_assert(K == BM_B, "matrix-core chains: bandwidth 4");
   const long E = (long)(K + 1) * M;
-  const unsigned long long t_start = fin.debug_stamps ? __builtin_amdgcn_s_memrealtime() : 0ull;
+  const unsigned long long t_start = (fin.debug_stamps || fin.p_helpers) ? __builtin_amdgcn_s_memrealtime() : 0ull;
   auto rstamp = [&](int slot) {
     if (fin.debug_stamps && threadIdx.x == 0 && blockIdx.x <= 2)
       logdets[(slot < 4 ? 8 + 4 * (int)blockIdx.x : 24) + slot] = (slot == 0) ? (double)(t_start & 0xffffffffull) : (double)((__builtin_amdgcn_s_memrealtime() - t_start) & 0xffffffffull);
   };
   rstamp(0);
-  __shared__ int gave_up, kuu_ok;
+  __shared__ int gave_up, kuu_ok, help_miss;
   __shared__ double kuu_pref[4];
-  if (threadIdx.x == 0) { gave_up = 0; kuu_ok = 0; }
+  if (threadIdx.x == 0) { gave_up = 0; kuu_ok = 0; help_miss = 0; }
   __syncthreads();
   double s_v = s, asc_v = fin.alpha_scale;
   ElboScalars th_v = fin.th;
@@ -472,9 +476,23 @@
     }
     __syncthreads();
   }
+  if (fin.p_helpers && (int)blockIdx.x >= 2 + fin.split) {
+    if (fin.debug_no_publish) return;
+    const int hk = (int)blockIdx.x - 2 - fin.split;
+    bcr_mfma_level0_helper<BandSumToep>(BandSumToep{A, 1.0 / s_v, (lds_cdouble_ptr)kdl, (lds_cdouble_ptr)bnd, ki.lo, ki.hi}, b, M, wsP, lds, fin.stage,
+                                        (seq << 8) | 6ull, fin.p_helpers, hk, 1, fin.debug_stamps ? fin.xchg + 192 + 3 * hk + 1 : (double*)nullptr);
+    if (fin.debug_stamps && threadIdx.x == 0) {
+      fin.xchg[192 + 3 * hk] = (double)(t_start & 0xffffffffull);
+      fin.xchg[192 + 3 * hk + 2] = (double)(__builtin_amdgcn_s_memrealtime() & 0xffffffffull);
+    }
+    return;
+  }
   if (isP) {
     BmSplit bsp;
     if (fin.split) { bsp.half = isPR ? 1 : 0; bsp.xchg = fin.xchg; bsp.spin_limit = spin_limit; bsp.gave_up = &gave_up; bsp.tag = seq << 8; }
+    if (fin.split && fin.p_helpers) {
+      bsp.help = fin.p_helpers; bsp.stage = fin.stage; bsp.help_wait = fin.help_wait; bsp.t0 = t_start; bsp.miss = &help_miss; bsp.miss_ctr = fin.miss_ctr;
+    }
     bcr_mfma_solve<BandSumToep>(BandSumToep{A, 1.0 / s_v, (lds_cdouble_ptr)kdl, (lds_cdouble_ptr)bnd, ki.lo, ki.hi}, b, M, wsP, lds, SP, x, logdets + 2, info + 1, 1,
                                 fin.debug_stamps ? (isPR ? fin.xchg + 128 : logdets + 32) : (double*)nullptr, bsp);
     rstamp(3);
@@ -786,6 +804,15 @@
         size_t lb = sizeof(double) * bcr_mfma_lds_doubles(nb), lk = sizeof(double) * bcr_mfma_pre_lds_doubles(nb, n_rec);
         if (lk > lb) lb = lk;
         if (sizeof(double) * FIN_LDS_DOUBLES > lb) lb = sizeof(double) * FIN_LDS_DOUBLES;
+        int p_want = 0;
+        if (nb >= 128 && !debug_env().no_split && !h->ahead_req) {
+          p_want = debug_env().p_helpers != -2 ? debug_env().p_helpers : h->p_helpers;
+          if (p_want < 0) p_want = P_HELPERS_AUTO;
+          if (p_want > P_HELPERS_MAX) p_want = P_HELPERS_MAX;
+          if (bcr_mfma_ws_doubles(nb) + bcr_mfma_stage_doubles(nb) > bcr_ws_P(K)) p_want = 0;
+          const size_t lh = sizeof(double) * bcr_mfma_helper_lds_doubles(nb);
+          if (p_want > 0 && lh > lb) lb = lh;
+        }
         auto kern = elbo_chains_mfma_kernel<K>;
         static size_t lds_granted[16] = {0};
         size_t& granted = lds_granted[h->device & 15];
@@ -800,6 +827,24 @@
           ff.xchg = w.LP;
         }
         ff.n_helpers = 0;
+        ff.p_helpers = 0;
+        if (ff.split && !h->ahead_req) {
+          const int want = p_want;
+          if (want > 0) {
+            if (!h->p_miss_dev) {
+              if (hipMalloc(reinterpret_cast<void**>(&h->p_miss_dev), 2 * sizeof(unsigned long long)) != hipSuccess ||
+                  hipMemset(h->p_miss_dev, 0, 2 * sizeof(unsigned long long)) != hipSuccess) {
+                set_error("p helpers: device allocation failed: %s", hipGetErrorString(hipGetLastError()));
+                return ASVGP_ERR_HIP;
+              }
+            }
+            ff.p_helpers = want;
+            ff.stage = w.bcrP + bcr_mfma_ws_doubles(nb);
+            ff.help_wait = debug_env().p_helper_wait > 0 ? debug_env().p_helper_wait : P_HELPER_WAIT_TICKS;
+            ff.miss_ctr = h->p_miss_dev;
+            ff.debug_no_publish = debug_env().no_helper_publish;
+          }
+        }
         const bool plan_first = debug_env().plan_first != 0;
         const bool host_times = debug_env().host_times != 0;
         auto now_us = []() { timespec ts; clock_gettime(CLOCK_MONOTONIC, &ts); return ts.tv_sec * 1e6 + ts.tv_nsec * 1e-3; };
@@ -828,7 +873,7 @@
           h->fwd.tab = tab; h->fwd.slot = slot; h->fwd.seq = seq;
           handle_post_forward(h);
         }
-        hipLaunchKernelGGL(kern, dim3(2 + ff.split + ff.n_helpers), dim3(BM_THREADS), lb, st, ki, S, cf, w.Kuu, w.dK, A, b, (int)M, w.bcrP, w.SP, w.alpha, w.logdets, info, s,
+        hipLaunchKernelGGL(kern, dim3(2 + ff.split + ff.n_helpers + ff.p_helpers), dim3(BM_THREADS), lb, st, ki, S, cf, w.Kuu, w.dK, A, b, (int)M, w.bcrP, w.SP, w.alpha, w.logdets, info, s,
                            tab_k, n_rec, h->node_rec_dev, w.bcrK, w.SK, w.dSK, h->done_dev + slot, seq,
                            gpu_fwd ? dd_ready : (plan_first ? (const unsigned long long*)nullptr : h->ready_dev + slot), spin_limit, ff, box_k);
         if (h->ahead_req) {
@@ -1208,6 +1253,17 @@
 #ifndef ASVGP_ELBO_ONLY_K
 using namespace asvgp;
 
+extern "C" int asvgp_p_helper_shares(int64_t nb, int H, int* out, int cap) {
+  if (nb < 2 || nb > 512 || H < 1 || H > 64) return 0;
+  const int n = bm_helper_share((int)nb, H, -1, nullptr);
+  for (int s = 0; s < n && s < cap && out; ++s) {
+    BmShare sh{0, 0, 0, 0};
+    bm_helper_share((int)nb, H, s, &sh);
+    out[4 * s] = sh.half; out[4 * s + 1] = sh.m_lo; out[4 * s + 2] = sh.m_hi; out[4 * s + 3] = sh.halo;
+  }
+  return n;
+}
+
 extern "C" size_t asvgp_elbo_workspace_bytes(int64_t M, int k, int64_t D) {
   if (M < 1 || k < 1 || D < 1) return 0;
   return sizeof(double) * ws_doubles(M, k, D);
diff --git a/asvgp_amd/csrc/handle.hip b/asvgp_amd/csrc/handle.hip
--- a/asvgp_amd/csrc/handle.hip
+++ b/asvgp_amd/csrc/handle.hip
@@ -1,4 +1,5 @@
 #include <sched.h>
+#include <stdio.h>
 #include <stdlib.h>
 #include <string.h>
 #include <time.h>
@@ -22,6 +23,9 @@
   g_dbg.plan_first = getenv("ASVGP_PLAN_FIRST") ? 1 : 0;
   g_dbg.bcr_stamps = getenv("ASVGP_BCR_STAMPS") ? atoi(getenv("ASVGP_BCR_STAMPS")) : 0;
   g_dbg.no_split = getenv("ASVGP_NO_SPLIT") ? atoi(getenv("ASVGP_NO_SPLIT")) : 0;
+  g_dbg.p_helpers = getenv("ASVGP_P_HELPERS") ? atoi(getenv("ASVGP_P_HELPERS")) : -2;
+  g_dbg.p_helper_wait = getenv("ASVGP_P_HELPER_WAIT") ? atol(getenv("ASVGP_P_HELPER_WAIT")) : 0;
+  g_dbg.no_helper_publish = getenv("ASVGP_DEBUG_NO_HELPER_PUBLISH") ? 1 : 0;
 }
 const DebugEnv& debug_env() {
   std::call_once(g_dbg_once, debug_env_load);
@@ -232,6 +236,14 @@
   if (h->prof_made)
     for (int i = 0; i < PROF_RING; ++i) { (void)hipEventDestroy(h->prof_ev[i][0]); (void)hipEventDestroy(h->prof_ev[i][1]); }
   if (h->order_dev) { (void)hipFree(h->order_dev); h->order_dev = nullptr; }
+  if (h->p_miss_dev) {
+    if (getenv("ASVGP_P_HELPER_REPORT")) {
+      unsigned long long n = 0;
+      if (hipMemcpy(&n, h->p_miss_dev, sizeof(n), hipMemcpyDeviceToHost) == hipSuccess && h->seq > 0)
+        fprintf(stderr, "[asvgp] level-0 helper misses: %llu (table sequence number at teardown: %llu)\n", n, h->seq);
+    }
+    (void)hipFree(h->p_miss_dev); h->p_miss_dev = nullptr;
+  }
   if (h->box_host) { (void)hipHostFree(h->box_host); h->box_host = nullptr; h->box_dev = nullptr; }
   h->magic = 0;
   delete h;
@@ -288,6 +300,20 @@
   }
   as_handle(handle)->band_algo = algo;
   return ASVGP_OK;
+}
+
+extern "C" int asvgp_set_p_helpers(asvgp_handle_t handle, int n) {
+  if (n < -1 || n > 13) { set_error("set_p_helpers: -1 auto, 0 off, 1 .. 13 helper workgroups"); return ASVGP_ERR_BAD_ARG; }
+  as_handle(handle)->p_helpers = n;
+  return ASVGP_OK;
+}
+
+extern "C" int64_t asvgp_p_helper_misses(asvgp_handle_t handle) {
+  Handle* h = as_handle(handle);
+  if (!h->p_miss_dev) return 0;
+  unsigned long long n = 0;
+  if (hipMemcpy(&n, h->p_miss_dev, sizeof(n), hipMemcpyDeviceToHost) != hipSuccess) { set_error("p_helper_misses: %s", hipGetErrorString(hipGetLastError())); return -1; }
+  return (int64_t)n;
 }
 
 extern "C" int asvgp_set_deferred_forward_pass(asvgp_handle_t handle, int on) {
diff --git a/asvgp_amd/csrc/handle.hpp b/asvgp_amd/csrc/handle.hpp
--- a/asvgp_amd/csrc/handle.hpp
+++ b/asvgp_amd/csrc/handle.hpp
@@ -64,10 +64,13 @@
   struct PendingAhead { bool valid; int slot; unsigned long long seq; double* tab; int kind; double N, Nw, cw; } ahead = {false, 0, 0, nullptr, 0, 0.0, 0.0, 0.0};
   bool w_set = false;
   double w_npos = 0.0, w_sum = 0.0, w_sumlog = 0.0;
+  int p_helpers = -1;
+  unsigned long long* p_miss_dev = nullptr;
 };
 constexpr size_t BOX_BYTES = 4096;
 
-struct DebugEnv { int no_assembly; int chain_stamps; long spin_limit; int host_times; int plan_first; int bcr_stamps; int no_split; };
+struct DebugEnv { int no_assembly; int chain_stamps; long spin_limit; int host_times; int plan_first; int bcr_stamps; int no_split;
+                  int p_helpers; long p_helper_wait; int no_helper_publish; };
 const DebugEnv& debug_env();
 
 Handle* as_handle(asvgp_handle_t h);
diff --git a/include/asvgp_hip.h b/include/asvgp_hip.h
--- a/include/asvgp_hip.h
+++ b/include/asvgp_hip.h
@@ -40,6 +40,9 @@
                                   double* kuu_diag8, int64_t* lo, int64_t* hi, double* bnd256);
 int asvgp_host_mantissa_bits(void);
 int asvgp_debug_reload_env(void);
+int asvgp_set_p_helpers(asvgp_handle_t handle, int n);
+int64_t asvgp_p_helper_misses(asvgp_handle_t handle);
+int asvgp_p_helper_shares(int64_t nb, int H, int* out, int cap);
 int asvgp_set_deferred_forward_pass(asvgp_handle_t handle, int on);
 int asvgp_prior_publish(asvgp_handle_t handle);
 int asvgp_result_mirror(asvgp_handle_t handle, int enable, const double** host_ptr);
```
